# succinctlabs/snark-bn254-verifier

Measured on AMD Instinct MI355X. Metric: Groth16 verifies/sec (2 pub-inputs) at batch=2^20, 1/2/4/8 MI355X, higher is better.
Workload: dtype int64

## Files before the change

### snark-bn254-verifier_amd/csrc/bn254_fp.h

```cpp
#pragma once
#include <stdint.h>
#include <utility>
#include "bn254_constants.h"

#if defined(__HIPCC__)
#include <hip/hip_runtime.h>
#if defined(__HIP_DEVICE_COMPILE__)
#define BN_HD __host__ __device__ __forceinline__
#else
#define BN_HD __host__ __device__ inline
#endif
#if defined(BN_INLINE_ALL)
#define BN_HD_NOINLINE __host__ __device__ __forceinline__
#else
#define BN_HD_NOINLINE __host__ __device__ inline __attribute__((noinline))
#endif
#if defined(__HIP_DEVICE_COMPILE__)
#define BN_HD_DEVINLINE __host__ __device__ __forceinline__
#else
#define BN_HD_DEVINLINE __host__ __device__ inline __attribute__((noinline))
#endif
#else
#if defined(BN_TRACK_BOUNDS) || defined(BN_HOST_PLAIN_INLINE)
#define BN_HD inline
#else
#define BN_HD inline __attribute__((always_inline))
#endif
#define BN_HD_NOINLINE inline __attribute__((noinline))
#define BN_HD_DEVINLINE inline __attribute__((noinline))
#endif

#if defined(__HIP_DEVICE_COMPILE__) && !defined(BN_NO_SCHED_FENCE)
#define BN_SCHED_FENCE() __builtin_amdgcn_sched_barrier(0)
#else
#define BN_SCHED_FENCE() do { } while (0)
#endif

#if defined(BN_TRACK_BOUNDS) && !defined(__HIP_DEVICE_COMPILE__)
#include <cmath>
#include <cstdio>
#include <cstdlib>
#include <execinfo.h>
#define BN_TRACKING 1
#else
#define BN_TRACKING 0
#endif

namespace bn254 {

#define BN_HALF (1 << (BN_LB - 1))

struct Fp {
  int32_t v[BN_NL];
#if BN_TRACKING
  double vb;
  double lb;
#endif
};

#if BN_TRACKING
static const long double BN_P_LD = 21888242871839275222246405745257275088696311157297823662689037894645226208583.0L;
inline long double fp_dbg_value(const Fp& a) {
  long double s = 0;
  for (int i = BN_NL - 1; i >= 0; i--) s = s * 536870912.0L + (long double)a.v[i];
  return s;
}
inline void fp_dbg_fail(const char* what, double x) {
  fprintf(stderr, "bn254 bound violation: %s (%g)\n", what, x);
  void* bt[32]; int n = backtrace(bt, 32); backtrace_symbols_fd(bt, n, 2);
  abort();
}
inline void fp_dbg_check(const Fp& a, const char* where) {
  long double val = fabsl(fp_dbg_value(a)) / BN_P_LD;
  if (val > (long double)a.vb * (1 + 1e-12L) + 1e-9L) fp_dbg_fail(where, (double)val);
  if (a.vb > 80.0) fp_dbg_fail("value bound exceeds representable range (|v| < 2^260)", a.vb);
  for (int i = 0; i < BN_NL; i++)
    if (fabs((double)a.v[i]) > a.lb * 536870912.0 + 0.5) fp_dbg_fail("digit bound wrong", (double)a.v[i]);
}
#define BN_SETB(x, VB, LB) do { (x).vb = (VB); (x).lb = (LB); fp_dbg_check((x), __func__); } while (0)
#define BN_VB(x) ((x).vb)
#define BN_LBD(x) ((x).lb)
#else
#define BN_SETB(x, VB, LB) do { } while (0)
#define BN_VB(x) 0.0
#define BN_LBD(x) 0.0
#endif

BN_HD int32_t bn_p_limb(int i) {
  switch (i) {
    case 0: return BN_P0; case 1: return BN_P1; case 2: return BN_P2; case 3: return BN_P3; case 4: return BN_P4;
    case 5: return BN_P5; case 6: return BN_P6; case 7: return BN_P7; default: return BN_P8;
  }
}
BN_HD int32_t bn_sext29(uint32_t x) { return (int32_t)(x << 3) >> 3; }

BN_HD Fp fp_from_limbs(const int32_t* c) {
  Fp r;
#pragma unroll
  for (int i = 0; i < BN_NL; i++) r.v[i] = c[i];
  BN_SETB(r, 1.0, 0.5);
  return r;
}
BN_HD Fp fp_zero() {
  Fp r;
#pragma unroll
  for (int i = 0; i < BN_NL; i++) r.v[i] = 0;
  BN_SETB(r, 0.0, 0.5);
  return r;
}
BN_HD Fp fp_one() { return fp_from_limbs(BN_ONE); }

BN_HD Fp fp_norm(const Fp& a) {
  Fp r;
  int32_t c = 0;
#pragma unroll
  for (int i = 0; i < BN_NL - 1; i++) {
    int32_t t = a.v[i] + c + BN_HALF;
    r.v[i] = (t & (int32_t)BN_MASK) - BN_HALF;
    c = t >> BN_LB;
  }
  r.v[BN_NL - 1] = a.v[BN_NL - 1] + c;
#if BN_TRACKING
  if (a.lb > 3.4) fp_dbg_fail("fp_norm: digit overflow", a.lb);
  BN_SETB(r, a.vb, 0.5);
#endif
  return r;
}

BN_HD Fp fp_add_lazy(const Fp& a, const Fp& b) {
  Fp r;
#pragma unroll
  for (int i = 0; i < BN_NL; i++) r.v[i] = a.v[i] + b.v[i];
  BN_SETB(r, BN_VB(a) + BN_VB(b), BN_LBD(a) + BN_LBD(b));
  return r;
}
BN_HD Fp fp_sub_lazy(const Fp& a, const Fp& b) {
  Fp r;
#pragma unroll
  for (int i = 0; i < BN_NL; i++) r.v[i] = a.v[i] - b.v[i];
  BN_SETB(r, BN_VB(a) + BN_VB(b), BN_LBD(a) + BN_LBD(b));
  return r;
}
BN_HD Fp fp_neg(const Fp& a) {
  Fp r;
#pragma unroll
  for (int i = 0; i < BN_NL; i++) r.v[i] = -a.v[i];
  BN_SETB(r, BN_VB(a), BN_LBD(a) + 1e-9);
  return r;
}
BN_HD Fp fp_add(const Fp& a, const Fp& b) { return fp_norm(fp_add_lazy(a, b)); }
BN_HD Fp fp_sub(const Fp& a, const Fp& b) { return fp_norm(fp_sub_lazy(a, b)); }
BN_HD Fp fp_dbl(const Fp& a) { return fp_add(a, a); }
BN_HD Fp fp_dbl_lazy(const Fp& a) { return fp_add_lazy(a, a); }

BN_HD Fp fp_lincomb(int32_t k1, const Fp& a, int32_t k2, const Fp& b) {
  Fp r;
  int64_t acc = 0;
#pragma unroll
  for (int i = 0; i < BN_NL - 1; i++) {
    acc += (int64_t)k1 * (int64_t)a.v[i] + (int64_t)k2 * (int64_t)b.v[i] + BN_HALF;
    r.v[i] = (int32_t)((uint32_t)acc & BN_MASK) - BN_HALF;
    acc >>= BN_LB;
  }
  acc += (int64_t)k1 * (int64_t)a.v[BN_NL - 1] + (int64_t)k2 * (int64_t)b.v[BN_NL - 1];
  r.v[BN_NL - 1] = (int32_t)acc;
#if BN_TRACKING
  BN_SETB(r, a.vb * (k1 < 0 ? -k1 : k1) + b.vb * (k2 < 0 ? -k2 : k2), 0.5);
#endif
  return r;
}
BN_HD Fp fp_lincomb_reduce(int32_t k1, const Fp& a, int32_t k2, const Fp& b) {
  const int64_t C = 1420063842;
  int64_t top = (int64_t)k1 * (int64_t)a.v[BN_NL - 1] + (int64_t)k2 * (int64_t)b.v[BN_NL - 1];
  int32_t q = (int32_t)((top * C) >> 52);
  Fp r;
  int64_t acc = 0;
#pragma unroll
  for (int i = 0; i < BN_NL - 1; i++) {
    acc += (int64_t)k1 * (int64_t)a.v[i] + (int64_t)k2 * (int64_t)b.v[i] - (int64_t)q * (int64_t)bn_p_limb(i) + BN_HALF;
    r.v[i] = (int32_t)((uint32_t)acc & BN_MASK) - BN_HALF;
    acc >>= BN_LB;
  }
  acc += top - (int64_t)q * (int64_t)bn_p_limb(BN_NL - 1);
  r.v[BN_NL - 1] = (int32_t)acc;
#if BN_TRACKING
  if (a.vb * (k1 < 0 ? -k1 : k1) + b.vb * (k2 < 0 ? -k2 : k2) > 1e5) fp_dbg_fail("fp_lincomb_reduce: out of range", a.vb + b.vb);
  if (a.lb > 1.01 || b.lb > 1.01) fp_dbg_fail("fp_lincomb_reduce: digits too large", a.lb + b.lb);
  BN_SETB(r, 1.0 + 3e-5, 0.5);
#endif
  return r;
}
BN_HD Fp fp_reduce(const Fp& a) { return fp_lincomb_reduce(1, a, 0, a); }

template <int SIGN>
struct DotTerm {
  const Fp& a;
  const Fp& b;
};
BN_HD DotTerm<1> dplus(const Fp& a, const Fp& b) { return DotTerm<1>{a, b}; }
BN_HD DotTerm<-1> dminus(const Fp& a, const Fp& b) { return DotTerm<-1>{a, b}; }
template <int S> BN_HD DotTerm<S> dterm(const Fp& a, const Fp& b) { return DotTerm<S>{a, b}; }

struct DotAcc { int64_t p1, m1, p2, m2; };
template <int SIGN, int K>
BN_HD void dot_col(DotAcc& c, const DotTerm<SIGN>& t) {
  constexpr int LO = K < BN_NL ? 0 : K - (BN_NL - 1);
  constexpr int HI = K < BN_NL ? K : BN_NL - 1;
#pragma unroll
  for (int i = LO; i <= HI; i++) {
    int64_t pr = (int64_t)t.a.v[i] * (int64_t)t.b.v[K - i];
    if (SIGN == 1) c.p1 += pr; else if (SIGN == -1) c.m1 += pr; else if (SIGN == 2) c.p2 += pr; else c.m2 += pr;
  }
}
constexpr int bn_iabs(int x) { return x < 0 ? -x : x; }
template <int K, int... SIGNS>
BN_HD void dot_step(int64_t& acc, int32_t (&m)[BN_NL], Fp& r, const DotTerm<SIGNS>&... terms) {
  constexpr bool has_m1 = ((SIGNS == -1) || ...), has_p2 = ((SIGNS == 2) || ...), has_m2 = ((SIGNS == -2) || ...);
  DotAcc c; c.p1 = acc; c.m1 = 0; c.p2 = 0; c.m2 = 0;
  (dot_col<SIGNS, K>(c, terms), ...);
  acc = c.p1;
  if (has_m1) acc -= c.m1;
  if (has_p2 && has_m2) acc += 2 * (c.p2 - c.m2);
  else if (has_p2) acc += 2 * c.p2;
  else if (has_m2) acc -= 2 * c.m2;
  if constexpr (K < BN_NL) {
#pragma unroll
    for (int i = 0; i < K; i++) acc += (int64_t)m[i] * (int64_t)bn_p_limb(K - i);
    m[K] = bn_sext29((uint32_t)acc * BN_PINV);
    acc += (int64_t)m[K] * (int64_t)bn_p_limb(0);
    acc >>= BN_LB;
  } else {
#pragma unroll
    for (int i = K - (BN_NL - 1); i < BN_NL; i++) acc += (int64_t)m[i] * (int64_t)bn_p_limb(K - i);
    acc += BN_HALF;
    r.v[K - BN_NL] = (int32_t)((uint32_t)acc & BN_MASK) - BN_HALF;
    acc >>= BN_LB;
  }
}
template <int... KS, int... SIGNS>
BN_HD void dot_all(std::integer_sequence<int, KS...>, int64_t& acc, int32_t (&m)[BN_NL], Fp& r, const DotTerm<SIGNS>&... terms) {
  (dot_step<KS, SIGNS...>(acc, m, r, terms...), ...);
}
template <int... SIGNS>
BN_HD Fp fp_dot(const DotTerm<SIGNS>&... terms) {
  BN_SCHED_FENCE();
  int64_t acc = 0;
  int32_t m[BN_NL];
  Fp r;
  dot_all(std::make_integer_sequence<int, 2 * BN_NL - 1>{}, acc, m, r, terms...);
  r.v[BN_NL - 1] = (int32_t)acc;
  BN_SCHED_FENCE();
#if BN_TRACKING
  double cap = ((9.0 * bn_iabs(SIGNS) * terms.a.lb * terms.b.lb) + ...);
  if (cap + 9.0 * 0.25 + 0.01 > 32.0) fp_dbg_fail("fp_dot: accumulator may overflow", cap);
  double s = ((bn_iabs(SIGNS) * terms.a.vb * terms.b.vb) + ...);
  BN_SETB(r, 1.0 + s / 169.0 + 1e-6, 0.5);
#endif
  return r;
}
BN_HD Fp fp_mul(const Fp& a, const Fp& b) { return fp_dot(dplus(a, b)); }
BN_HD Fp fp_sqr(const Fp& a) {
  BN_SCHED_FENCE();
  int64_t acc = 0;
  int32_t m[BN_NL];
  int32_t a2[BN_NL];
  Fp r;
#pragma unroll
  for (int i = 0; i < BN_NL; i++) a2[i] = a.v[i] * 2;
#pragma unroll
  for (int k = 0; k < 2 * BN_NL - 1; k++) {
#pragma unroll
    for (int i = 0; i < BN_NL; i++) {
      int j = k - i;
      if (j >= 0 && j < BN_NL && i < j) acc += (int64_t)a2[i] * (int64_t)a.v[j];
    }
    if ((k & 1) == 0) acc += (int64_t)a.v[k / 2] * (int64_t)a.v[k / 2];
    if (k < BN_NL) {
#pragma unroll
      for (int i = 0; i < k; i++) acc += (int64_t)m[i] * (int64_t)bn_p_limb(k - i);
      m[k] = bn_sext29((uint32_t)acc * BN_PINV);
      acc += (int64_t)m[k] * (int64_t)bn_p_limb(0);
      acc >>= BN_LB;
    } else {
#pragma unroll
      for (int i = k - (BN_NL - 1); i < BN_NL; i++) acc += (int64_t)m[i] * (int64_t)bn_p_limb(k - i);
      acc += BN_HALF;
      r.v[k - BN_NL] = (int32_t)((uint32_t)acc & BN_MASK) - BN_HALF;
      acc >>= BN_LB;
    }
  }
  r.v[BN_NL - 1] = (int32_t)acc;
  BN_SCHED_FENCE();
#if BN_TRACKING
  if (9.0 * a.lb * a.lb + 2.26 > 32.0) fp_dbg_fail("fp_sqr: accumulator may overflow", a.lb);
  BN_SETB(r, 1.0 + a.vb * a.vb / 169.0 + 1e-6, 0.5);
#endif
  return r;
}

BN_HD bool fp_is_negative(const Fp& a) {
  int32_t s = a.v[BN_NL - 1];
#pragma unroll
  for (int i = BN_NL - 2; i >= 0; i--) s = (s != 0) ? s : a.v[i];
  return s < 0;
}
BN_HD Fp fp_select(bool c, const Fp& a, const Fp& b) {
  Fp r;
#pragma unroll
  for (int i = 0; i < BN_NL; i++) r.v[i] = c ? a.v[i] : b.v[i];
#if BN_TRACKING
  BN_SETB(r, a.vb > b.vb ? a.vb : b.vb, a.lb > b.lb ? a.lb : b.lb);
#endif
  return r;
}
BN_HD Fp fp_canon(const Fp& a) {
  Fp r = fp_reduce(fp_norm(a));
  Fp pl = fp_from_limbs(BN_P);
  r = fp_select(fp_is_negative(r), fp_norm(fp_add_lazy(r, pl)), r);
  Fp dn = fp_norm(fp_sub_lazy(r, pl));
  r = fp_select(!fp_is_negative(dn), dn, r);
  BN_SETB(r, 1.0, 0.5);
  return r;
}
BN_HD bool fp_is_zero(const Fp& a) {
  Fp c = fp_canon(a);
  int32_t d = 0;
#pragma unroll
  for (int i = 0; i < BN_NL; i++) d |= c.v[i];
  return d == 0;
}
BN_HD bool fp_eq(const Fp& a, const Fp& b) { return fp_is_zero(fp_sub(a, b)); }

BN_HD Fp fp_from_words_raw(const uint32_t w[8]) {
  Fp r;
#pragma unroll
  for (int i = 0; i < BN_NL; i++) {
    int bit = BN_LB * i, wi = bit >> 5, sh = bit & 31;
    uint64_t lo = w[wi];
    uint64_t hi = (wi + 1 < 8) ? w[wi + 1] : 0;
    r.v[i] = (int32_t)((uint32_t)(((hi << 32) | lo) >> sh) & BN_MASK);
  }
  BN_SETB(r, 5.3, 1.0);
  return fp_norm(r);
}
BN_HD Fp fp_from_words(const uint32_t w[8]) {
  return fp_mul(fp_from_words_raw(w), fp_from_limbs(BN_R2));
}
BN_HD void fp_to_words(uint32_t w[8], const Fp& a) {
  Fp one_plain = fp_zero();
  one_plain.v[0] = 1;
  Fp c = fp_canon(fp_mul(a, one_plain));
  uint32_t u[BN_NL];
  int32_t cy = 0;
#pragma unroll
  for (int i = 0; i < BN_NL; i++) {
    int32_t t = c.v[i] + cy;
    u[i] = (uint32_t)t & BN_MASK;
    cy = t >> BN_LB;
  }
#pragma unroll
  for (int i = 0; i < 8; i++) w[i] = 0;
#pragma unroll
  for (int i = 0; i < BN_NL; i++) {
    int bit = BN_LB * i, wi = bit >> 5, sh = bit & 31;
    uint64_t v = (uint64_t)u[i] << sh;
    if (wi < 8) w[wi] |= (uint32_t)v;
    if (wi + 1 < 8) w[wi + 1] |= (uint32_t)(v >> 32);
  }
}
BN_HD bool words_ge(const uint32_t a[8], const uint32_t b[8]) {
  bool ge = true;
#pragma unroll
  for (int i = 0; i < 8; i++) ge = (a[i] > b[i]) || (a[i] == b[i] && ge);
  return ge;
}
BN_HD void words_from_be(uint32_t w[8], const uint8_t* be32) {
#pragma unroll
  for (int i = 0; i < 8; i++) {
    const uint8_t* p = be32 + 4 * (7 - i);
    w[i] = (uint32_t)p[0] << 24 | (uint32_t)p[1] << 16 | (uint32_t)p[2] << 8 | (uint32_t)p[3];
  }
}
BN_HD void words_to_be(uint8_t* be32, const uint32_t w[8]) {
#pragma unroll
  for (int i = 0; i < 8; i++) {
    uint8_t* p = be32 + 4 * (7 - i);
    p[0] = (uint8_t)(w[i] >> 24); p[1] = (uint8_t)(w[i] >> 16); p[2] = (uint8_t)(w[i] >> 8); p[3] = (uint8_t)w[i];
  }
}

BN_HD_DEVINLINE Fp fp_mul_nl(const Fp& a, const Fp& b) { return fp_mul(a, b); }
BN_HD_DEVINLINE Fp fp_sqr_nl(const Fp& a) { return fp_sqr(a); }
BN_HD Fp fp_pow_bits(const Fp& a, const uint8_t* bits, int nbits) {
  Fp acc = a;
  for (int i = 1; i < nbits; i++) {
    acc = fp_sqr_nl(acc);
    if (bits[i]) acc = fp_mul_nl(acc, a);
  }
  return acc;
}
BN_HD Fp fp_inv_fermat(const Fp& a) { return fp_pow_bits(fp_reduce(fp_norm(a)), BN_EXP_PM2_BITS, BN_EXP_PM2_NBITS); }

BN_HD int bn_clz64(uint64_t x) {
#if defined(__HIP_DEVICE_COMPILE__)
  return __clzll((long long)x);
#else
  return __builtin_clzll(x);
#endif
}
BN_HD void fp_unsigned_digits(int32_t d[BN_NL], const int32_t* balanced) {
  int32_t cy = 0;
#pragma unroll
  for (int i = 0; i < BN_NL; i++) { int32_t t = balanced[i] + cy; d[i] = t & (int32_t)BN_MASK; cy = t >> BN_LB; }
}
BN_HD Fp fp_inv(const Fp& x) {
  const Fp y = fp_canon(x);
  int32_t a[BN_NL], b[BN_NL], u[BN_NL], v[BN_NL];
  fp_unsigned_digits(a, y.v);
  {
    int32_t pl[BN_NL];
#pragma unroll
    for (int i = 0; i < BN_NL; i++) pl[i] = bn_p_limb(i);
    fp_unsigned_digits(b, pl);
  }
  {
    const Fp c = fp_from_limbs(BN_R2);
#pragma unroll
    for (int i = 0; i < BN_NL; i++) { u[i] = c.v[i]; v[i] = 0; }
  }
#pragma unroll 1
  for (int round = 0; round < 18; round++) {
    int32_t ah = 0, am = 0, al = 0, bh = 0, bm = 0, bl = 0, low = 0;
    bool found = false;
#pragma unroll
    for (int i = BN_NL - 1; i >= 2; i--) {
      const bool take = !found && ((a[i] | b[i]) != 0);
      ah = take ? a[i] : ah; am = take ? a[i - 1] : am; al = take ? a[i - 2] : al;
      bh = take ? b[i] : bh; bm = take ? b[i - 1] : bm; bl = take ? b[i - 2] : bl;
// ... 74 lines not shown
```

### snark-bn254-verifier_amd/csrc/bn254_k_g16_load.hip

```cpp
#include <hip/hip_runtime.h>
#include "bn254_launch_ops.h"
#include "bn254_g16_loader.h"
#include "bn254_g16_plan.h"
#include "bn254_codec.h"
#include "bn254_sha256.h"

namespace bn254 {

__global__ void __launch_bounds__(256, 2)
k_g16_classify(const uint8_t* __restrict__ proofs, size_t stride, uint32_t n, uint8_t* __restrict__ status, uint32_t* __restrict__ block_count) {
  __shared__ uint32_t lds[4 * 64 * PREP_LDS_ROW];
  __shared__ uint32_t wave_pending[4];
  const int wave = threadIdx.x >> 6, lane = threadIdx.x & 63;
  const uint32_t first = blockIdx.x * 256u + (uint32_t)wave * 64u;
  uint32_t* wl = lds + wave * 64 * PREP_LDS_ROW;
  const uint32_t i = first + lane;
  const bool live = i < n;
  g16_stage_records(wl, proofs, stride, n, lane, i);
  __syncthreads();
  G1Aff A; G2Aff B;
  int err = g16_parse_a(wl + lane * PREP_LDS_ROW, A);
  err = g16_parse_b(wl + lane * PREP_LDS_ROW, B, err);
  if (live) status[i] = err ? (uint8_t)err : (uint8_t)BN254_ST_PENDING;
  const uint64_t pend = __builtin_amdgcn_ballot_w64(live && err == 0);
  if (lane == 0) wave_pending[wave] = (uint32_t)__builtin_popcountll(pend);
  __syncthreads();
  if (threadIdx.x == 0) block_count[blockIdx.x] = wave_pending[0] + wave_pending[1] + wave_pending[2] + wave_pending[3];
}
__global__ void __launch_bounds__(256)
k_g16_compact_write(const uint8_t* __restrict__ status, uint32_t n, const uint32_t* __restrict__ block_count, uint32_t* __restrict__ slot_proof, uint8_t* __restrict__ slot_status) {
  __shared__ uint32_t s_before[G16_COMPACT_BLOCK], s_total[G16_COMPACT_BLOCK], wave_pending[4];
  const uint32_t t = threadIdx.x, wave = t >> 6, lane = t & 63u;
  uint32_t before, total;
  g16_compact_partial(block_count, gridDim.x, blockIdx.x, t, &before, &total);
  s_before[t] = before; s_total[t] = total;
  const uint32_t i = blockIdx.x * 256u + t;
  const bool pend = i < n && status[i] == BN254_ST_PENDING;
  const uint64_t mask = __builtin_amdgcn_ballot_w64(pend);
  if (lane == 0) wave_pending[wave] = (uint32_t)__builtin_popcountll(mask);
  __syncthreads();
  for (uint32_t d = G16_COMPACT_BLOCK / 2; d > 0; d >>= 1) {
    if (t < d) { s_before[t] += s_before[t + d]; s_total[t] += s_total[t + d]; }
    __syncthreads();
  }
  const uint32_t n_pending = s_total[0];
  uint32_t j = s_before[0] + (uint32_t)__builtin_popcountll(mask & ((1ull << lane) - 1ull));
  for (uint32_t k = 0; k < wave; k++) j += wave_pending[k];
  if (pend && j < n) { slot_proof[j] = i; slot_status[j] = BN254_ST_PENDING; }
  if (i < n && i >= n_pending) { slot_proof[i] = G16_COMPACT_NO_PROOF; slot_status[i] = 0; }
}

__global__ void __launch_bounds__(256, 2)
k_g16_prepare(const uint8_t* __restrict__ proofs, size_t stride, const uint8_t* __restrict__ inputs, int n_public, uint32_t n,
              int32_t* ws, uint8_t* __restrict__ status, const int32_t* __restrict__ msm_tab, const int32_t* __restrict__ k0,
              int inputs_match_key, int wide_msm, const uint32_t* __restrict__ slot_proof, uint8_t* __restrict__ slot_status) {
  __shared__ uint32_t lds[4 * 64 * PREP_LDS_ROW];
  const int wave = threadIdx.x >> 6, lane = threadIdx.x & 63;
  const uint32_t first = blockIdx.x * 256u + (uint32_t)wave * 64u;
  uint32_t* wl = lds + wave * 64 * PREP_LDS_ROW;
  uint32_t pi = first + (uint32_t)lane;
  bool wave_live = true;
  if (slot_proof) {
    const bool slot_live = pi < n && (slot_status[pi] & BN254_ST_PENDING) != 0;
    pi = slot_live ? slot_proof[pi] : G16_COMPACT_NO_PROOF;
    wave_live = __builtin_amdgcn_ballot_w64(slot_live) != 0;
  }
  if (wave_live) g16_stage_records(wl, proofs, stride, n, lane, pi);
  __syncthreads();
  if (!wave_live) return;
  uint8_t* const st_out = slot_proof ? slot_status : status;
  const uint32_t i = first + lane;
  const bool live = pi < n;
  const uint32_t ii = live ? pi : n - 1;
  DevWs w(ws, n, live ? i : DEAD_LANE);
  const uint32_t* my = wl + lane * PREP_LDS_ROW;

  G1Aff A;
  int err = g16_parse_a(my, A);
  w.st(VE_AX, A.x); w.st(VE_AY, A.y);
  G2Aff B;
  err = g16_parse_b(my, B, err);
  vst2(w, VE_B, B.x); vst2(w, VE_B + 2, B.y);

  G1Aff C;
  const int err_c = g16_parse_c(my, C);
  w.st(VE_CX, C.x); w.st(VE_CY, C.y);

  if (wide_msm) {
    if (live) st_out[i] = err ? (uint8_t)err : (uint8_t)(BN254_ST_PENDING | err_c);
    return;
  }
  G1Aff K0; K0.x = uni_ld(k0); K0.y = uni_ld(k0 + BN_NL);
  G1Proj L = g1_from_affine(K0);
  if (inputs_match_key) {
    for (int s = 0; s < n_public; s++) {
      const uint8_t* sp = inputs + ((size_t)ii * (size_t)n_public + s) * 32;
      uint32_t sw[8];
      if ((((uintptr_t)inputs) & 3) == 0) {
#pragma unroll
        for (int k = 0; k < 8; k++) sw[k] = ((const uint32_t*)sp)[k];
      } else {
#pragma unroll
        for (int k = 0; k < 8; k++) sw[k] = (uint32_t)sp[4 * k] | (uint32_t)sp[4 * k + 1] << 8 | (uint32_t)sp[4 * k + 2] << 16 | (uint32_t)sp[4 * k + 3] << 24;
      }
      uint32_t kw[8];
#pragma unroll
      for (int k = 0; k < 8; k++) kw[k] = __builtin_bswap32(sw[7 - k]);
      auto next_digit = [&]() -> uint32_t {
        const uint32_t dg = kw[0] & MSM_FW_ENTRIES;
#pragma unroll
        for (int k = 0; k < 7; k++) kw[k] = (kw[k] >> MSM_FW_BITS) | (kw[k + 1] << (32 - MSM_FW_BITS));
        kw[7] >>= MSM_FW_BITS;
        return dg;
      };
      uint32_t dig = next_digit();
      G1Aff q = msm_entry(msm_tab, (size_t)(s * MSM_FW_WINDOWS) * MSM_FW_ENTRIES + (dig ? dig - 1 : 0));
      for (int j = 0; j < MSM_FW_WINDOWS; j++) {
        uint32_t dn = 0; G1Aff qn = q;
        if (j + 1 < MSM_FW_WINDOWS) { dn = next_digit(); qn = msm_entry(msm_tab, (size_t)(s * MSM_FW_WINDOWS + j + 1) * MSM_FW_ENTRIES + (dn ? dn - 1 : 0)); }
        if (dig != 0) L = g1_add_mixed(L, q);
        dig = dn; q = qn;
      }
    }
  }
  bool l_inf = g1_is_identity(L);
  G1Aff La = g1_to_affine(L);
  La.y = fp_select(l_inf, fp_one(), La.y);
  w.st(VE_LX, La.x); w.st(VE_LY, La.y);
  if (live) st_out[i] = err ? (uint8_t)err : (uint8_t)(BN254_ST_PENDING | (l_inf ? BN254_ST_LINF : 0) | err_c);
}

__global__ void __launch_bounds__(256, 2)
k_g16_check_scalars(const uint8_t* __restrict__ inputs, int n_public, uint32_t n, uint8_t* __restrict__ status) {
  const uint32_t i = blockIdx.x * 256u + threadIdx.x;
  if (i >= n) return;
  bool bad = false;
  for (int s = 0; s < n_public; s++) {
    const uint8_t* sp = inputs + ((size_t)i * (size_t)n_public + s) * 32;
    uint32_t w[8];
    words_from_be(w, sp);
    bad |= words_ge(w, BN_R_WORDS);
  }
  if (bad) status[i] = BN254_ST_NOT_MEMBER;
}

__global__ void __launch_bounds__(256, 2)
k_g16_msm_partial(const uint8_t* __restrict__ inputs, int n_public, uint32_t n, int per, int chunks, const uint8_t* __restrict__ status,
                  const int32_t* __restrict__ msm_tab, int32_t* __restrict__ part) {
  const uint32_t g = blockIdx.x * 256u + threadIdx.x;
  if (g >= n * (uint32_t)chunks) return;
  const uint32_t c = g / n, i = g - c * n;
  G1Proj acc = g1_identity();
  if (status[i] & BN254_ST_PENDING) {
    const int s_end = (int)min((uint32_t)n_public, (c + 1) * (uint32_t)per);
    for (int s = (int)(c * per); s < s_end; s++) {
      const uint8_t* sp = inputs + ((size_t)i * (size_t)n_public + s) * 32;
      uint32_t sw[8];
      if ((((uintptr_t)inputs) & 3) == 0) {
#pragma unroll
        for (int k = 0; k < 8; k++) sw[k] = ((const uint32_t*)sp)[k];
      } else {
#pragma unroll
        for (int k = 0; k < 8; k++) sw[k] = (uint32_t)sp[4 * k] | (uint32_t)sp[4 * k + 1] << 8 | (uint32_t)sp[4 * k + 2] << 16 | (uint32_t)sp[4 * k + 3] << 24;
      }
      for (int j = 0; j < 32; j++) {
        const int wi = 31 - j;
        uint32_t dig = sw[0] & 0xff;
#pragma unroll
        for (int k = 0; k < 7; k++) sw[k] = (sw[k] >> 8) | (sw[k + 1] << 24);
        sw[7] >>= 8;
        if (dig != 0) acc = g1_add_mixed(acc, msm_entry(msm_tab, (size_t)(s * 32 + wi) * 255 + (dig - 1)));
      }
    }
  }
  int32_t* o = part + (size_t)c * 27 * n + i;
#pragma unroll
  for (int l = 0; l < BN_NL; l++) { o[(size_t)l * n] = acc.x.v[l]; o[(size_t)(9 + l) * n] = acc.y.v[l]; o[(size_t)(18 + l) * n] = acc.z.v[l]; }
}
__global__ void __launch_bounds__(256)
k_g16_comb_digits(const uint8_t* __restrict__ inputs, int n_public, uint32_t n, uint16_t* __restrict__ digits) {
  const size_t g = (size_t)blockIdx.x * 256u + threadIdx.x;
  if (g >= (size_t)n * (size_t)n_public) return;
  const uint32_t s = (uint32_t)(g / n), i = (uint32_t)(g - (size_t)s * n);
  const uint8_t* sp = inputs + ((size_t)i * (size_t)n_public + s) * 32;
  uint32_t w[8];
#pragma unroll
  for (int k = 0; k < 8; k++) { const uint8_t* q = sp + 28 - 4 * k; w[k] = (uint32_t)q[0] << 24 | (uint32_t)q[1] << 16 | (uint32_t)q[2] << 8 | (uint32_t)q[3]; }
  for (int col = 0; col < G16_COMB_COLS; col++) {
    const uint32_t idx = g16_comb_digit(w, col);
    digits[((size_t)col * (size_t)n_public + s) * n + i] = (uint16_t)idx;
  }
}
__global__ void __launch_bounds__(256, 2)
k_g16_msm_partial_comb(const uint16_t* __restrict__ digits, int n_public, uint32_t n, int per, int chunks, const uint8_t* __restrict__ status,
                       const int32_t* __restrict__ msm_tab, int32_t* __restrict__ part) {
  const uint32_t g = blockIdx.x * 256u + threadIdx.x;
  if (g >= n * (uint32_t)chunks) return;
  const uint32_t c = g / n, i = g - c * n;
  G1Proj acc = g1_identity();
  if (status[i] & BN254_ST_PENDING) {
    const int s_begin = (int)(c * per), s_end = (int)min((uint32_t)n_public, (c + 1) * (uint32_t)per);
    auto digit_at = [&](int col, int s) -> uint32_t { return digits[((size_t)col * (size_t)n_public + (size_t)s) * n + i]; };
    auto entry_at = [&](int s, uint32_t idx) -> G1Aff { return msm_entry(msm_tab, ((size_t)s << G16_COMB_TEETH) + idx); };
    auto advance = [&](int& col, int& s) { if (++s == s_end) { s = s_begin; col--; } };
    if (s_begin < s_end) {
      int col1 = G16_COMB_COLS - 1, s1 = s_begin;
      uint32_t d_cur = digit_at(col1, s1);
      G1Aff e_cur = entry_at(s1, d_cur);
      int col0 = col1, s0 = s1;
      advance(col1, s1);
      uint32_t d_nxt = col1 >= 0 ? digit_at(col1, s1) : 0u;
      int col2 = col1, s2 = s1;
      if (col2 >= 0) advance(col2, s2);
      while (col0 >= 0) {
        G1Aff e_nxt = e_cur;
        uint32_t d_nn = 0u;
        if (col1 >= 0) e_nxt = entry_at(s1, d_nxt);
        if (col2 >= 0) d_nn = digit_at(col2, s2);
        if (s0 == s_begin && col0 != G16_COMB_COLS - 1) acc = g1_dbl(acc);
        if (d_cur != 0) acc = g1_add_mixed(acc, e_cur);
        col0 = col1; s0 = s1; d_cur = d_nxt; e_cur = e_nxt;
        col1 = col2; s1 = s2; d_nxt = d_nn;
        if (col2 >= 0) advance(col2, s2);
      }
    }
  }
  int32_t* o = part + (size_t)c * 27 * n + i;
#pragma unroll
  for (int l = 0; l < BN_NL; l++) { o[(size_t)l * n] = acc.x.v[l]; o[(size_t)(9 + l) * n] = acc.y.v[l]; o[(size_t)(18 + l) * n] = acc.z.v[l]; }
}
__global__ void __launch_bounds__(256, 2)
k_g16_msm_reduce(const int32_t* __restrict__ part, int chunks, uint32_t n, int32_t* ws, uint8_t* __restrict__ status, const int32_t* __restrict__ k0) {
  VM_KERNEL_PROLOGUE();
  const uint32_t ii = i < n ? i : n - 1;
  G1Aff K0; K0.x = uni_ld(k0); K0.y = uni_ld(k0 + BN_NL);
  G1Proj L = g1_from_affine(K0);
  for (int c = 0; c < chunks; c++) {
    const int32_t* o = part + (size_t)c * 27 * n + ii;
    G1Proj q;
#pragma unroll
    for (int l = 0; l < BN_NL; l++) { q.x.v[l] = o[(size_t)l * n]; q.y.v[l] = o[(size_t)(9 + l) * n]; q.z.v[l] = o[(size_t)(18 + l) * n]; }
    BN_SETB(q.x, 3.0, 0.5); BN_SETB(q.y, 3.0, 0.5); BN_SETB(q.z, 3.0, 0.5);
    L = g1_add(L, q);
  }
  bool l_inf = g1_is_identity(L);
  G1Aff La = g1_to_affine(L);
  La.y = fp_select(l_inf, fp_one(), La.y);
  w.st(VE_LX, La.x); w.st(VE_LY, La.y);
  if (i < n && (st & BN254_ST_PENDING) && l_inf) status[i] = st | BN254_ST_LINF;
}

__global__ void __launch_bounds__(256, 2)
k_g16_msm_reduce8(const int32_t* __restrict__ part, int chunks, uint32_t n, int32_t* ws, uint8_t* __restrict__ status, const int32_t* __restrict__ k0) {
  __shared__ int32_t sums[32 * 8 * 27];
  const uint32_t p = blockIdx.x * 32u + (threadIdx.x >> 3), sub = threadIdx.x & 7u;
  const uint32_t pp = p < n ? p : n - 1;
  G1Proj L = g1_identity();
  for (int c = (int)sub; c < chunks; c += 8) {
    const int32_t* o = part + (size_t)c * 27 * n + pp;
    G1Proj q;
#pragma unroll
    for (int l = 0; l < BN_NL; l++) { q.x.v[l] = o[(size_t)l * n]; q.y.v[l] = o[(size_t)(9 + l) * n]; q.z.v[l] = o[(size_t)(18 + l) * n]; }
    BN_SETB(q.x, 3.0, 0.5); BN_SETB(q.y, 3.0, 0.5); BN_SETB(q.z, 3.0, 0.5);
    L = g1_add(L, q);
  }
  {
    int32_t* o = sums + threadIdx.x * 27;
    const Fp x = fp_reduce(L.x), y = fp_reduce(L.y), z = fp_reduce(L.z);
#pragma unroll
    for (int l = 0; l < BN_NL; l++) { o[l] = x.v[l]; o[9 + l] = y.v[l]; o[18 + l] = z.v[l]; }
  }
  __syncthreads();
  const bool lead = sub == 0 && p < n;
  const uint8_t st = status[pp];
  G1Aff K0; K0.x = uni_ld(k0); K0.y = uni_ld(k0 + BN_NL);
  G1Proj T = g1_from_affine(K0);
  for (int j = 0; j < 8; j++) {
    const int32_t* o = sums + ((threadIdx.x & ~7u) + j) * 27;
    G1Proj q;
#pragma unroll
    for (int l = 0; l < BN_NL; l++) { q.x.v[l] = o[l]; q.y.v[l] = o[9 + l]; q.z.v[l] = o[18 + l]; }
    BN_SETB(q.x, 1.01, 0.5); BN_SETB(q.y, 1.01, 0.5); BN_SETB(q.z, 1.01, 0.5);
    T = g1_add(T, q);
  }
  const bool l_inf = g1_is_identity(T);
  G1Aff La = g1_to_affine(T);
  La.y = fp_select(l_inf, fp_one(), La.y);
  DevWs w(ws, n, lead ? p : DEAD_LANE);
  w.st(VE_LX, La.x); w.st(VE_LY, La.y);
  if (lead && (st & BN254_ST_PENDING) && l_inf) status[p] = st | BN254_ST_LINF;
}

__global__ void k_gather_rows(uint8_t* __restrict__ dst, const uint8_t* __restrict__ src, size_t src_stride, uint32_t row_bytes, const uint32_t* __restrict__ idx, uint32_t m) {
  const size_t t = (size_t)blockIdx.x * 256 + threadIdx.x;
  const uint32_t per = row_bytes / 4;
  if (t >= (size_t)m * per) return;
  const uint32_t k = (uint32_t)(t / per), c = (uint32_t)(t % per);
  const uint8_t* p = src + (size_t)idx[k] * src_stride + 4 * (size_t)c;
  uint32_t v;
  if ((((uintptr_t)src) | src_stride) & 3) v = (uint32_t)p[0] | (uint32_t)p[1] << 8 | (uint32_t)p[2] << 16 | (uint32_t)p[3] << 24;
  else v = *(const uint32_t*)p;
  ((uint32_t*)dst)[t] = v;
}
__global__ void k_scatter_status(uint8_t* __restrict__ status, const uint8_t* __restrict__ fb_status, const uint32_t* __restrict__ idx, uint32_t m) {
  const uint32_t k = blockIdx.x * 256u + threadIdx.x;
  if (k < m) status[idx[k]] = fb_status[k];
}
__global__ void __launch_bounds__(256, 2) k_g16_decompress(const uint8_t* __restrict__ src, size_t stride, uint32_t n, uint8_t* __restrict__ raw, uint8_t* __restrict__ pre) {
  const uint32_t i = blockIdx.x * 256u + threadIdx.x;
  if (i >= n) return;
  const uint8_t* p = src + (size_t)i * stride;
  uint32_t in[32], out[64];
  if (((((uintptr_t)src) | stride) & 15) == 0) {
#pragma unroll
    for (int k = 0; k < 8; k++) { const uint4 v = ((const uint4*)p)[k]; in[4 * k] = v.x; in[4 * k + 1] = v.y; in[4 * k + 2] = v.z; in[4 * k + 3] = v.w; }
  } else {
#pragma unroll
    for (int k = 0; k < 32; k++) in[k] = (uint32_t)p[4 * k] | (uint32_t)p[4 * k + 1] << 8 | (uint32_t)p[4 * k + 2] << 16 | (uint32_t)p[4 * k + 3] << 24;
  }
  const bool ok = g16_decompress_record(in, out);
  uint4* q = (uint4*)(raw + (size_t)i * 256);
#pragma unroll
  for (int k = 0; k < 16; k++) q[k] = make_uint4(out[4 * k], out[4 * k + 1], out[4 * k + 2], out[4 * k + 3]);
  pre[i] = ok ? 0 : 1;
}
__global__ void __launch_bounds__(256) k_g16_status_merge(uint8_t* __restrict__ status, const uint8_t* __restrict__ pre, uint32_t n) {
  const uint32_t i = blockIdx.x * 256u + threadIdx.x;
  if (i < n && pre[i]) status[i] = BN254_ST_MALFORMED;
}
__global__ void __launch_bounds__(256) k_sp1_public_inputs(const uint8_t* __restrict__ vkh, size_t vkh_stride, const uint8_t* __restrict__ pv, uint64_t pv_bytes,
                                                           uint64_t pv_base, const uint64_t* __restrict__ off, uint32_t n, uint8_t* __restrict__ rows,
                                                           uint8_t* __restrict__ pre) {
  const uint32_t i = blockIdx.x * 256u + threadIdx.x;
  const bool lane = i < n;
  uint64_t start = 0, len = 0;
  bool ok = false;
  if (lane) ok = sp1_range(off[i], off[i + 1], pv_base, pv_bytes, &start, &len);
  const uint64_t nb = lane ? sha256_blocks(len) : 0;
  uint32_t h[8];
  sha256_init(h);
  for (uint64_t b = 0; __ballot(b < nb) != 0; b++) sp1_sha256_block(h, pv, pv_bytes, start, len, b);
  if (!lane) return;
  uint32_t v[8], dg[8];
  sp1_load_vkey_hash(vkh + (size_t)i * vkh_stride, v);
  sp1_digest_words(h, dg);
  uint4* q = (uint4*)(rows + (size_t)i * 64);
  q[0] = make_uint4(v[0], v[1], v[2], v[3]); q[1] = make_uint4(v[4], v[5], v[6], v[7]);
  q[2] = make_uint4(dg[0], dg[1], dg[2], dg[3]); q[3] = make_uint4(dg[4], dg[5], dg[6], dg[7]);
  pre[i] = ok ? 0 : 1;
}

}

using namespace bn254;
hipError_t bn254_launch_gather_rows(uint8_t* dst, const uint8_t* src, size_t src_stride, uint32_t row_bytes, const uint32_t* idx, uint32_t m, hipStream_t s) {
  const size_t threads = (size_t)m * (row_bytes / 4);
  if (threads) hipLaunchKernelGGL(k_gather_rows, dim3((unsigned)((threads + 255) / 256)), dim3(256), 0, s, dst, src, src_stride, row_bytes, idx, m);
  return hipGetLastError();
}
hipError_t bn254_launch_scatter_status(uint8_t* status, const uint8_t* fb_status, const uint32_t* idx, uint32_t m, hipStream_t s) {
  if (m) hipLaunchKernelGGL(k_scatter_status, dim3(grid_for(m)), dim3(256), 0, s, status, fb_status, idx, m);
  return hipGetLastError();
}
hipError_t bn254_launch_g16_decompress(const uint8_t* src, size_t stride, uint32_t n, uint8_t* raw, uint8_t* pre, hipStream_t s) {
  if (n) hipLaunchKernelGGL(k_g16_decompress, dim3(grid_for(n)), dim3(256), 0, s, src, stride, n, raw, pre);
  return hipGetLastError();
}
hipError_t bn254_launch_g16_status_merge(uint8_t* status, const uint8_t* pre, uint32_t n, hipStream_t s) {
  if (n) hipLaunchKernelGGL(k_g16_status_merge, dim3(grid_for(n)), dim3(256), 0, s, status, pre, n);
  return hipGetLastError();
}
hipError_t bn254_launch_sp1_public_inputs(const uint8_t* vkh, size_t vkh_stride, const uint8_t* pv, uint64_t pv_bytes, uint64_t pv_base, const uint64_t* off, uint32_t n,
                                          uint8_t* rows, uint8_t* pre, hipStream_t s) {
  if (n) hipLaunchKernelGGL(k_sp1_public_inputs, dim3(grid_for(n)), dim3(256), 0, s, vkh, vkh_stride, pv, pv_bytes, pv_base, off, n, rows, pre);
  return hipGetLastError();
}
```

### snark-bn254-verifier_amd/csrc/bn254_k_probe.hip

```cpp
#include <hip/hip_runtime.h>
#include "bn254_launch_ops.h"

namespace bn254 {

#define VALU_PEAK_ITERS 16384
__global__ void __launch_bounds__(256) k_valu_peak(uint32_t* out, uint32_t seed, int iters) {
  const uint32_t tid = threadIdx.x + blockIdx.x * blockDim.x;
  const uint32_t a = seed * 2654435761u + tid, b = (seed ^ 0x9e3779b9u) + tid * 7u;
  uint64_t acc[16];
#pragma unroll
  for (int i = 0; i < 16; i++) acc[i] = (uint64_t)(a + i) << 7 | (uint32_t)i;
  for (int it = 0; it < iters; it++) {
#pragma unroll
    for (int i = 0; i < 16; i++) asm volatile("v_mad_u64_u32 %0, vcc, %1, %2, %0" : "+v"(acc[i]) : "v"(a), "v"(b) : "vcc");
  }
  uint32_t x = 0;
#pragma unroll
  for (int i = 0; i < 16; i++) x ^= (uint32_t)acc[i] ^ (uint32_t)(acc[i] >> 32);
  out[tid] = x;
}

__device__ __forceinline__ Fp probe_ld_fp(const uint8_t* p) {
  uint32_t w[8];
  words_from_be(w, p);
  return fp_from_words(w);
}
__device__ __forceinline__ void probe_st_fp(uint8_t* p, const Fp& a) {
  uint32_t w[8];
  fp_to_words(w, a);
  words_to_be(p, w);
}
__global__ void __launch_bounds__(256, 2) k_dbg_fp_mul(const uint8_t* a, const uint8_t* b, uint8_t* o, size_t n) {
  size_t i = (size_t)blockIdx.x * 256 + threadIdx.x;
  if (i >= n) return;
  probe_st_fp(o + 32 * i, fp_mul(probe_ld_fp(a + 32 * i), probe_ld_fp(b + 32 * i)));
}
__global__ void __launch_bounds__(256, 2) k_dbg_load(int32_t* ws, uint32_t n, uint8_t* status, int e, const uint8_t* src, int kind) {
  const uint32_t i = blockIdx.x * 256u + threadIdx.x;
  if (i >= n) return;
  DevWs w(ws, n, i);
  if (kind == 0) {
    const int korder[6] = {0, 2, 4, 1, 3, 5};
    const uint8_t* p = src + 384 * (size_t)i;
    for (int t = 0; t < 6; t++) { w.st(e + 2 * korder[t], probe_ld_fp(p + 64 * t)); w.st(e + 2 * korder[t] + 1, probe_ld_fp(p + 64 * t + 32)); }
  } else if (kind == 3) {
    const int korder[6] = {0, 2, 4, 1, 3, 5};
    const int32_t* p = (const int32_t*)src + 12 * BN_NL * (size_t)i;
    for (int t = 0; t < 12; t++) { Fp a; for (int l = 0; l < BN_NL; l++) a.v[l] = p[t * BN_NL + l]; w.st(e + 2 * korder[t >> 1] + (t & 1), a); }
  } else if (kind == 4) {
    w.st(e, probe_ld_fp(src + 64 * (size_t)i)); w.st(e + 1, probe_ld_fp(src + 64 * (size_t)i + 32));
  } else if (kind == 1) {
    w.st(VE_AX, probe_ld_fp(src + 64 * (size_t)i)); w.st(VE_AY, probe_ld_fp(src + 64 * (size_t)i + 32));
  } else {
    const uint8_t* q = src + 128 * (size_t)i;
    w.st(VE_B + 1, probe_ld_fp(q)); w.st(VE_B, probe_ld_fp(q + 32)); w.st(VE_B + 3, probe_ld_fp(q + 64)); w.st(VE_B + 2, probe_ld_fp(q + 96));
  }
  status[i] = BN254_ST_PENDING;
}
__global__ void __launch_bounds__(256, 2) k_dbg_store(int32_t* ws, uint32_t n, int e, uint8_t* dst) {
  const uint32_t i = blockIdx.x * 256u + threadIdx.x;
  if (i >= n) return;
  DevWs w(ws, n, i);
  const int korder[6] = {0, 2, 4, 1, 3, 5};
  uint8_t* p = dst + 384 * (size_t)i;
  for (int t = 0; t < 6; t++) { probe_st_fp(p + 64 * t, w.ld(e + 2 * korder[t])); probe_st_fp(p + 64 * t + 32, w.ld(e + 2 * korder[t] + 1)); }
}
__global__ void __launch_bounds__(256, 2) k_dbg_store_raw(int32_t* ws, uint32_t n, int e, int32_t* dst) {
  const uint32_t i = blockIdx.x * 256u + threadIdx.x;
  if (i >= n) return;
  DevWs w(ws, n, i);
  const int korder[6] = {0, 2, 4, 1, 3, 5};
  int32_t* p = dst + 12 * BN_NL * (size_t)i;
  for (int t = 0; t < 12; t++) { const Fp a = w.ld(e + 2 * korder[t >> 1] + (t & 1)); for (int l = 0; l < BN_NL; l++) p[t * BN_NL + l] = a.v[l]; }
}
__global__ void __launch_bounds__(256, 2) k_dbg_g2_subgroup(const uint8_t* g2, uint8_t* o, size_t n) {
  size_t i = (size_t)blockIdx.x * 256 + threadIdx.x;
  if (i >= n) return;
  G2Aff q; q.x.c1 = probe_ld_fp(g2 + 128 * i); q.x.c0 = probe_ld_fp(g2 + 128 * i + 32);
  q.y.c1 = probe_ld_fp(g2 + 128 * i + 64); q.y.c0 = probe_ld_fp(g2 + 128 * i + 96);
  o[i] = (g2_on_curve(q) && g2_in_subgroup(q)) ? 1 : 0;
}
__global__ void __launch_bounds__(256, 2) k_dbg_g2_ate(int32_t* ws, uint32_t n, const uint8_t* __restrict__ status, uint8_t* o) {
  VM_KERNEL_PROLOGUE();
  bool ok = vm_g2_ate_check(w, VE_T, VE_B);
  if (i < n) o[i] = ok ? 1 : 0;
}

}

using namespace bn254;
double bn254_measure_valu_peak(int reps) {
  hipDeviceProp_t p;
  int dev = 0;
  if (hipGetDevice(&dev) != hipSuccess || hipGetDeviceProperties(&p, dev) != hipSuccess) return 0.0;
  const int grid = p.multiProcessorCount * 4;
  uint32_t* out = nullptr;
  if (hipMalloc((void**)&out, (size_t)grid * 256 * 4) != hipSuccess) return 0.0;
  hipEvent_t e0, e1;
  (void)hipEventCreate(&e0); (void)hipEventCreate(&e1);
  hipLaunchKernelGGL(k_valu_peak, dim3(grid), dim3(256), 0, nullptr, out, 1u, VALU_PEAK_ITERS);
  float best = 1e30f;
  int since_best = 0;
  for (int r = 0; r < 200 && since_best < reps; r++) {
    (void)hipEventRecord(e0, nullptr);
    hipLaunchKernelGGL(k_valu_peak, dim3(grid), dim3(256), 0, nullptr, out, (uint32_t)(r + 2), VALU_PEAK_ITERS);
    (void)hipEventRecord(e1, nullptr);
    if (hipEventSynchronize(e1) != hipSuccess) { best = 1e30f; break; }
    float ms = 0.f;
    since_best++;
    if (hipEventElapsedTime(&ms, e0, e1) == hipSuccess && ms > 0.f && ms < best * 0.998f) { best = ms; since_best = 0; }
  }
  (void)hipEventDestroy(e0); (void)hipEventDestroy(e1); (void)hipFree(out);
  if (best > 1e29f) return 0.0;
  return (double)grid * 256.0 * (double)VALU_PEAK_ITERS * 16.0 / ((double)best * 1e-3);
}
double bn254_measure_valu_sustained(double ms_target) {
  hipDeviceProp_t p;
  int dev = 0;
  if (hipGetDevice(&dev) != hipSuccess || hipGetDeviceProperties(&p, dev) != hipSuccess) return 0.0;
  const int grid = p.multiProcessorCount * 4;
  uint32_t* out = nullptr;
  if (hipMalloc((void**)&out, (size_t)grid * 256 * 4) != hipSuccess) return 0.0;
  int launches = (int)(ms_target / 2.0);
  if (launches < 4) launches = 4;
  if (launches > 1000) launches = 1000;
  hipEvent_t e0, e1;
  (void)hipEventCreate(&e0); (void)hipEventCreate(&e1);
  (void)hipEventRecord(e0, nullptr);
  for (int r = 0; r < launches; r++) hipLaunchKernelGGL(k_valu_peak, dim3(grid), dim3(256), 0, nullptr, out, (uint32_t)(r + 1), VALU_PEAK_ITERS);
  (void)hipEventRecord(e1, nullptr);
  float ms = 0.f;
  const bool ok = hipEventSynchronize(e1) == hipSuccess && hipEventElapsedTime(&ms, e0, e1) == hipSuccess && ms > 0.f;
  (void)hipEventDestroy(e0); (void)hipEventDestroy(e1); (void)hipFree(out);
  return ok ? (double)launches * grid * 256.0 * (double)VALU_PEAK_ITERS * 16.0 / ((double)ms * 1e-3) : 0.0;
}
hipError_t bn254_launch_dbg_fp_mul(const uint8_t* a, const uint8_t* b, uint8_t* o, size_t n, hipStream_t s) {
  hipLaunchKernelGGL(k_dbg_fp_mul, dim3(grid_for(n)), dim3(256), 0, s, a, b, o, n);
  return hipGetLastError();
}
hipError_t bn254_launch_dbg_load(int32_t* ws, size_t n, uint8_t* status, int e, const void* src, int kind, hipStream_t s) {
  hipLaunchKernelGGL(k_dbg_load, dim3(grid_for(n)), dim3(256), 0, s, ws, (uint32_t)n, status, e, (const uint8_t*)src, kind);
  return hipGetLastError();
}
hipError_t bn254_launch_dbg_store(int32_t* ws, size_t n, int e, void* dst, int format, hipStream_t s) {
  if (format) hipLaunchKernelGGL(k_dbg_store_raw, dim3(grid_for(n)), dim3(256), 0, s, ws, (uint32_t)n, e, (int32_t*)dst);
  else hipLaunchKernelGGL(k_dbg_store, dim3(grid_for(n)), dim3(256), 0, s, ws, (uint32_t)n, e, (uint8_t*)dst);
  return hipGetLastError();
}
hipError_t bn254_launch_dbg_fp12_op_fmt(int op, const uint8_t* a, const uint8_t* b, uint8_t* o, size_t n, int32_t* ws, uint8_t* status, int in_format, int out_format, hipStream_t s) {
  unsigned g = grid_for(n);
  uint32_t nn = (uint32_t)n;
  LaunchOps ops{ws, nn, status, g, s, {nullptr, nullptr, nullptr}, nullptr};
  const int kind = in_format ? 3 : 0;
  hipLaunchKernelGGL(k_dbg_load, dim3(g), dim3(256), 0, s, ws, nn, status, (int)VE_F, a, kind);
  if (op == 0 || op == 8 || op == 9) {
    hipLaunchKernelGGL(k_dbg_load, dim3(g), dim3(256), 0, s, ws, nn, status, (int)VE_S1, b, kind);
    ops.f12_mul(VE_S0, op == 9 ? (VE_F | VE_CONJ) : VE_F, VE_S1, op == 8);
  }
  else if (op == 1) { ops.f12_sqr(VE_F); ops.f12_conj(VE_S0, VE_F); ops.f12_conj(VE_S0, VE_S0); }
  else if (op == 2) ops.f12_inv(VE_S0, VE_F);
  else if (op == 3) {
    ops.f12_inv(VE_S0, VE_F); ops.f12_conj(VE_S1, VE_F); ops.f12_mul(VE_S0, VE_S1, VE_S0); ops.f12_frob(VE_S1, VE_S0, 2);
    ops.f12_mul(VE_S0, VE_S1, VE_S0); ops.f12_cyclo_sqr(VE_S0, VE_S0);
  }
  else if (op == 5) ops.f12_cyclo_sqr(VE_S0, VE_F);
  else ops.f12_frob(VE_S0, VE_F, op == 6 ? 2 : op == 7 ? 3 : 1);
  (void)bn254_launch_dbg_store(ws, n, (int)VE_S0, o, out_format, s);
  return hipGetLastError();
}
hipError_t bn254_launch_dbg_verdict(int form, int32_t* ws, size_t n, uint8_t* status, const int32_t* target, hipStream_t s) {
  unsigned grid = grid_for(n);
  uint32_t nn = (uint32_t)n;
  if (form == 0) hipLaunchKernelGGL(k_g16_compare, dim3(grid), dim3(256), 0, s, ws, nn, status, target, (int)BN254_ST_REJECT);
  else hipLaunchKernelGGL(k_f12_mul_verdict, dim3(grid), dim3(256), 0, s, ws, nn, status, (int)VE_S0, (int)VE_S2, (int)VE_S0, target, (int)BN254_ST_REJECT, (const uint32_t*)nullptr, status);
  return hipGetLastError();
}
hipError_t bn254_launch_dbg_coop12_g16(const G16LaunchArgs& a, hipStream_t s) {
  hipLaunchKernelGGL(k_g16_prepare, dim3(grid_for(a.n)), dim3(256), 0, s, a.proofs, a.stride, a.inputs, a.n_public, (uint32_t)a.n, a.ws, a.status, a.msm_tab, a.k0, a.inputs_match_key, 1,
                     (const uint32_t*)nullptr, (uint8_t*)nullptr);
  return bn254_coop12_miller_g16(a.ws, a.status, a.n, a.gtab, a.dtab, a.inputs, a.n_public, a.inputs_match_key, a.msm_tab, a.k0, 0, a.target, s);
}
hipError_t bn254_launch_dbg_pairing(const uint8_t* g1, const uint8_t* g2, uint8_t* o, size_t n, int32_t* ws, uint8_t* status, hipStream_t s) {
  unsigned g = grid_for(n);
  uint32_t nn = (uint32_t)n;
  LaunchOps ops{ws, nn, status, g, s, {nullptr, nullptr, nullptr}, nullptr};
  hipLaunchKernelGGL(k_dbg_load, dim3(g), dim3(256), 0, s, ws, nn, status, 0, g1, 1);
  hipLaunchKernelGGL(k_dbg_load, dim3(g), dim3(256), 0, s, ws, nn, status, 0, g2, 2);
  hipLaunchKernelGGL(k_vm_init, dim3(g), dim3(256), 0, s, ws, nn, (const uint8_t*)status);
  vm_miller_program(ops, miller_step_table().kind, false);
  vm_final_exp_program(ops);
  hipLaunchKernelGGL(k_dbg_store, dim3(g), dim3(256), 0, s, ws, nn, (int)VE_S0, o);
  return hipGetLastError();
}
hipError_t bn254_launch_dbg_g2_ate(const uint8_t* g1, const uint8_t* g2, uint8_t* o, size_t n, int32_t* ws, uint8_t* status, hipStream_t s) {
  unsigned g = grid_for(n);
  uint32_t nn = (uint32_t)n;
  LaunchOps ops{ws, nn, status, g, s, {nullptr, nullptr, nullptr}, nullptr};
  hipLaunchKernelGGL(k_dbg_load, dim3(g), dim3(256), 0, s, ws, nn, status, 0, g1, 1);
  hipLaunchKernelGGL(k_dbg_load, dim3(g), dim3(256), 0, s, ws, nn, status, 0, g2, 2);
  hipLaunchKernelGGL(k_vm_init, dim3(g), dim3(256), 0, s, ws, nn, (const uint8_t*)status);
  vm_miller_program(ops, miller_step_table().kind, false);
  hipLaunchKernelGGL(k_dbg_g2_ate, dim3(g), dim3(256), 0, s, ws, nn, (const uint8_t*)status, o);
  return hipGetLastError();
}
hipError_t bn254_launch_dbg_g2_subgroup(const uint8_t* g2, uint8_t* o, size_t n, hipStream_t s) {
  hipLaunchKernelGGL(k_dbg_g2_subgroup, dim3(grid_for(n)), dim3(256), 0, s, g2, o, n);
  return hipGetLastError();
}
```

### snark-bn254-verifier_amd/csrc/bn254_kernels.hip

```cpp
#include <hip/hip_runtime.h>
#include "bn254_launch_ops.h"
#include "bn254_g16_plan.h"

static_assert(G16_MILLER_STEPS == BN_ATE_STEPS, "bn254_g16_plan.h counts the Miller steps of bn254_constants.h");

namespace bn254 {

__global__ void __launch_bounds__(256, 2) k_vm_init(int32_t* ws, uint32_t n, const uint8_t* __restrict__ status) {
  VM_KERNEL_PROLOGUE();
  w.st(VE_F, fp_one());
  for (int e = 1; e < 12; e++) w.st(VE_F + e, fp_zero());
  for (int e = 0; e < 4; e++) w.st(VE_T + e, w.ld(VE_B + e));
  w.st(VE_T + 4, fp_one()); w.st(VE_T + 5, fp_zero());
}
__global__ void __launch_bounds__(256, 2) k_f12_sqr(int32_t* ws, uint32_t n, const uint8_t* __restrict__ status, int e) { VM_KERNEL_PROLOGUE(); vm_f12_sqr(w, e); }
__global__ void __launch_bounds__(256, 2) k_f12_mul_line_fixed(int32_t* ws, uint32_t n, const uint8_t* __restrict__ status, int e, const int32_t* __restrict__ entry, int e_px, int inf_mask) {
  VM_KERNEL_PROLOGUE();
  FixedLine l; l.m = uni_ld2(entry); l.c = uni_ld2(entry + 2 * BN_NL); l.xc = uni_ld2(entry + 4 * BN_NL);
  vm_f12_mul_line_fixed(w, e, l, e_px, (st & inf_mask) != 0);
}
__global__ void __launch_bounds__(256, 2) k_f12_mul_line_fixed2(int32_t* ws, uint32_t n, const uint8_t* __restrict__ status, int e, const int32_t* __restrict__ entry0,
                                                                int e_px0, int inf_mask0, const int32_t* __restrict__ entry1, int e_px1, int inf_mask1) {
  __shared__ int32_t park_lds[72 * 256];
  VM_KERNEL_PROLOGUE();
  w.lds = park_lds;
  FixedLine l0, l1;
  l0.m = uni_ld2(entry0); l0.c = uni_ld2(entry0 + 2 * BN_NL); l0.xc = uni_ld2(entry0 + 4 * BN_NL);
  l1.m = uni_ld2(entry1); l1.c = uni_ld2(entry1 + 2 * BN_NL); l1.xc = uni_ld2(entry1 + 4 * BN_NL);
  vm_f12_mul_line_fixed2(w, e, l0, e_px0, (st & inf_mask0) != 0, l1, e_px1, (st & inf_mask1) != 0);
}
__global__ void __launch_bounds__(256, 2) k_miller_dbl_var(int32_t* ws, uint32_t n, const uint8_t* __restrict__ status, int e_t, int e, int e_px) {
  VM_KERNEL_PROLOGUE(); vm_miller_dbl_var(w, e_t, e, e_px);
}
__global__ void __launch_bounds__(256, 2) k_miller_sqr_dbl_var(int32_t* ws, uint32_t n, const uint8_t* __restrict__ status, int e_t, int e, int e_px) {
  __shared__ int32_t park_lds[72 * 256];
  VM_KERNEL_PROLOGUE();
  w.lds = park_lds;
  vm_miller_sqr_dbl_var(w, e_t, e, e_px);
}
__global__ void __launch_bounds__(256, 2) k_miller_add_var(int32_t* ws, uint32_t n, const uint8_t* __restrict__ status, int e_t, int e_b, int which, int e, int e_px) {
  VM_KERNEL_PROLOGUE(); vm_miller_add_var(w, e_t, e_b, which, e, e_px);
}
__global__ void __launch_bounds__(256, 2) k_f12_mul(int32_t* ws, uint32_t n, const uint8_t* __restrict__ status, int d, int a, int b, int conj_b) {
  __shared__ int32_t park_lds[72 * 256];
  VM_KERNEL_PROLOGUE();
  w.lds = park_lds;
  vm_f12_mul(w, d, a, b, conj_b != 0);
}
__global__ void __launch_bounds__(256, 2) k_f12_mul_verdict(int32_t* ws, uint32_t n, uint8_t* status, int d, int a, int b, const int32_t* __restrict__ target, int reject_code,
                                                            const uint32_t* __restrict__ slot_proof, uint8_t* __restrict__ out_status) {
  __shared__ int32_t park_lds[72 * 256];
  const uint32_t i = blockIdx.x * 256u + threadIdx.x;
  const uint8_t st = status[i < n ? i : n - 1];
  uint8_t out = st;
  if (__builtin_amdgcn_ballot_w64((st & BN254_ST_PENDING) != 0) != 0) {
    DevWs w(ws, n, i < n ? i : DEAD_LANE);
    w.lds = park_lds;
    const bool acc = vm_f12_mul_eq_const(w, d, a, b, target);
    if (st & BN254_ST_PENDING) out = acc ? BN254_ST_ACCEPT : (uint8_t)reject_code;
    if (i < n && (st & BN254_ST_PENDING)) status[i] = out;
  }
  if (slot_proof && i < n && st != 0) out_status[slot_proof[i]] = out;
}
__global__ void __launch_bounds__(256, 2) k_f12_copy(int32_t* ws, uint32_t n, const uint8_t* __restrict__ status, int d, int a) { VM_KERNEL_PROLOGUE(); vm_f12_copy(w, d, a); }
__global__ void __launch_bounds__(256, 2) k_f12_cyclo_sqr(int32_t* ws, uint32_t n, const uint8_t* __restrict__ status, int d, int a) { VM_KERNEL_PROLOGUE(); vm_f12_cyclo_sqr(w, d, a); }
__global__ void __launch_bounds__(256, 2) k_f12_cyclo_sqr_n(int32_t* ws, uint32_t n, const uint8_t* __restrict__ status, int d, int a, int count) {
  VM_KERNEL_PROLOGUE(); vm_f12_cyclo_sqr_n(w, d, a, __builtin_amdgcn_readfirstlane(count));
}
__global__ void __launch_bounds__(256, 2) k_f12_conj(int32_t* ws, uint32_t n, const uint8_t* __restrict__ status, int d, int a) { VM_KERNEL_PROLOGUE(); vm_f12_conj(w, d, a); }
__global__ void __launch_bounds__(256, 2) k_f12_frob(int32_t* ws, uint32_t n, const uint8_t* __restrict__ status, int d, int a, int j) { VM_KERNEL_PROLOGUE(); vm_f12_frob(w, d, a, j); }
__global__ void __launch_bounds__(256, 2) k_f12_inv(int32_t* ws, uint32_t n, const uint8_t* __restrict__ status, int d, int a) { VM_KERNEL_PROLOGUE(); vm_f12_inv(w, d, a); }
__global__ void __launch_bounds__(256, 2) k_g16_compare(int32_t* ws, uint32_t n, uint8_t* __restrict__ status, const int32_t* __restrict__ target, int reject_code) {
  VM_KERNEL_PROLOGUE();
  bool acc = vm_f12_eq_const(w, VE_S0, target);
  if (i < n && (st & BN254_ST_PENDING)) status[i] = acc ? BN254_ST_ACCEPT : (uint8_t)reject_code;
}

__global__ void __launch_bounds__(256, 2)
k_g16_subgroup(uint32_t n, int32_t* ws, uint8_t* __restrict__ status, int inputs_match_key, int e_t) {
  VM_KERNEL_PROLOGUE();
  bool ok = vm_g2_ate_check(w, e_t, VE_B);
  if (i < n && (st & BN254_ST_PENDING)) status[i] = g16_subgroup_status(st, ok, inputs_match_key);
}

}

using namespace bn254;
const char* const bn254_kernel_kind_names[KID_COUNT] = {
  "k_g16_prepare", "k_g16_subgroup", "k_vm_init", "k_f12_sqr", "k_f12_mul_line_fixed",
  "k_f12_mul", "k_f12_cyclo_sqr", "k_f12_conj", "k_f12_frob", "k_f12_inv", "k_g16_compare", "k_f12_copy", "k_f12_cyclo_sqr_n", "k_miller_dbl_var", "k_miller_add_var", "k_g16_msm_partial", "k_g16_msm_reduce", "k_f12_mul_line_fixed2", "k_miller_sqr_dbl_var", "k_miller_step_dbl", "k_miller_step_add", "k_coop12_miller_g16", "k_miller_run"};

hipError_t bn254_launch_g16(const G16LaunchArgs& a, hipStream_t s, hipEvent_t* ev , G16Prof* prof) {
  unsigned grid = grid_for(a.n);
  uint32_t n = (uint32_t)a.n;
  if (ev) (void)hipEventRecord(ev[0], s);
  const G16Form form = g16_launch_form(a.n, (size_t)a.n_public, a.inputs_match_key != 0, a.msm_part != nullptr, a.part_of_larger != 0,
                                       a.split_streams[0] && a.split_streams[1], knob_coop_on(), knob_run_steps_g16());
  const bool wide = form.wide, coop = form.form == G16_FORM_COOP;
  const bool compact = a.slot_proof && a.slot_status && a.block_count && g16_compacts(form, a.key_inputs, a.strict_scalars != 0, a.rlc != 0);
  uint8_t* const lane_status = compact ? a.slot_status : a.status;
  const uint32_t* const slot_proof = compact ? a.slot_proof : nullptr;
  {
    ProfScope ps_(prof, KID_PREPARE, s);
    if (compact) {
      hipLaunchKernelGGL(k_g16_classify, dim3(grid), dim3(256), 0, s, a.proofs, a.stride, n, a.status, a.block_count);
      hipLaunchKernelGGL(k_g16_compact_write, dim3(grid), dim3(256), 0, s, (const uint8_t*)a.status, n, (const uint32_t*)a.block_count, a.slot_proof, a.slot_status);
    }
    hipLaunchKernelGGL(k_g16_prepare, dim3(grid), dim3(256), 0, s, a.proofs, a.stride, a.inputs, a.n_public, n, a.ws, a.status, a.msm_tab, a.k0, a.inputs_match_key, (wide || coop) ? 1 : 0,
                       slot_proof, a.slot_status);
  }
  if (a.strict_scalars && a.n_public > 0) hipLaunchKernelGGL(k_g16_check_scalars, dim3(grid), dim3(256), 0, s, a.inputs, a.n_public, n, a.status);
  if (wide) {
    const int per = knob_wide_per() ? knob_wide_per() : G16_WIDE_MSM_INPUTS_PER_LANE, chunks = (a.n_public + per - 1) / per;
    unsigned pg = (unsigned)(((size_t)n * chunks + 255) / 256);
    {
      ProfScope ps_(prof, KID_MSM_PARTIAL, s);
      if (a.msm_comb) {
        const size_t scalars = (size_t)n * (size_t)a.n_public;
        hipLaunchKernelGGL(k_g16_comb_digits, dim3((unsigned)((scalars + 255) / 256)), dim3(256), 0, s, a.inputs, a.n_public, n, a.msm_digits);
        hipLaunchKernelGGL(k_g16_msm_partial_comb, dim3(pg), dim3(256), 0, s, (const uint16_t*)a.msm_digits, a.n_public, n, per, chunks, (const uint8_t*)a.status, a.msm_tab, a.msm_part);
      }
      else hipLaunchKernelGGL(k_g16_msm_partial, dim3(pg), dim3(256), 0, s, a.inputs, a.n_public, n, per, chunks, (const uint8_t*)a.status, a.msm_tab, a.msm_part);
    }
    if (chunks >= 16 && a.n <= 65536) {
      ProfScope ps_(prof, KID_MSM_REDUCE, s);
      hipLaunchKernelGGL(k_g16_msm_reduce8, dim3((unsigned)((a.n + 31) / 32)), dim3(256), 0, s, (const int32_t*)a.msm_part, chunks, n, a.ws, a.status, a.k0);
    } else {
      BN_LAUNCH(KID_MSM_REDUCE, k_g16_msm_reduce, (const int32_t*)a.msm_part, chunks, n, a.ws, a.status, a.k0);
    }
  }
  if (ev) (void)hipEventRecord(ev[1], s);
  if (coop) {
    hipError_t e;
    { ProfScope ps_(prof, KID_COOP_G16, s); e = bn254_coop12_miller_g16(a.ws, a.status, a.n, a.gtab, a.dtab, a.inputs, a.n_public, a.inputs_match_key, a.msm_tab, a.k0, wide ? 1 : 0, a.target, s); }
    if (e != hipSuccess) return e;
    if (ev) { (void)hipEventRecord(ev[2], s); (void)hipEventRecord(ev[3], s); (void)hipEventRecord(ev[4], s); }
    return hipGetLastError();
  }
  LaunchOps ops{a.ws, n, lane_status, grid, s, {a.gtab, a.dtab, nullptr}, prof};
  const bool folded = form.form == G16_FORM_LANES && form.run_steps > 0;
  if (folded) { ops.run_fold = MR_FOLD_INIT | MR_FOLD_ATE; ops.inputs_match_key = a.inputs_match_key; }
  else BN_LAUNCH(KID_VM_INIT, k_vm_init, a.ws, n, (const uint8_t*)a.status);
  if (form.form == G16_FORM_LATENCY) {
    ops.f12_copy(VE_S1, VE_F); ops.f12_copy(VE_S2, VE_F);
    (void)hipEventRecord(a.split_ev[0], s);
    LaunchOps ob{a.ws, n, a.status, grid, a.split_streams[0], {a.gtab, a.dtab, nullptr}, nullptr};
    LaunchOps oc{a.ws, n, a.status, grid, a.split_streams[1], {a.gtab, a.dtab, nullptr}, nullptr};
    (void)hipStreamWaitEvent(ob.s, a.split_ev[0], 0); (void)hipStreamWaitEvent(oc.s, a.split_ev[0], 0);
    const uint8_t* kinds = miller_step_table().kind;
    for (int st_ = 0; st_ < BN_ATE_STEPS; st_++) {
      const int kind = kinds[st_];
      if (kind == 0) { if (st_ != 0) ops.miller_sqr_dbl_var(VE_T, VE_F, VE_AX); else ops.miller_dbl_var(VE_T, VE_F, VE_AX); }
      else ops.miller_add_var(VE_T, VE_B, kind - 1, VE_F, VE_AX);
      if (kind == 0 && st_ != 0) { ob.f12_sqr(VE_S1); oc.f12_sqr(VE_S2); }
      ob.f12_mul_line_fixed(VE_S1, 0, st_, VE_LX);
      oc.f12_mul_line_fixed(VE_S2, 1, st_, VE_CX);
    }
    (void)hipEventRecord(a.split_ev[1], ob.s); (void)hipEventRecord(a.split_ev[2], oc.s);
    (void)hipStreamWaitEvent(s, a.split_ev[1], 0); (void)hipStreamWaitEvent(s, a.split_ev[2], 0);
    ops.f12_mul(VE_F, VE_F, VE_S1); ops.f12_mul(VE_F, VE_F, VE_S2);
  } else {
    const int run_steps = form.run_steps;
    if (run_steps) vm_miller_program_runs(ops, run_steps);
    else vm_miller_program(ops, miller_step_table().kind, true);
  }
  if (ev) (void)hipEventRecord(ev[2], s);
  if (!folded) BN_LAUNCH(KID_SUBGROUP, k_g16_subgroup, n, a.ws, a.status, a.inputs_match_key, (int)VE_T);
  if (ev) (void)hipEventRecord(ev[3], s);
  if (folded) {
    vm_final_exp_program_head(ops);
    BN_LAUNCH(KID_F12_MUL, k_f12_mul_verdict, a.ws, n, lane_status, (int)VE_S0, (int)VE_S2, (int)VE_S0, a.target, BN254_ST_REJECT, slot_proof, a.status);
  } else {
    vm_final_exp_program(ops);
    BN_LAUNCH(KID_COMPARE, k_g16_compare, a.ws, n, a.status, a.target, BN254_ST_REJECT);
  }
  if (ev) (void)hipEventRecord(ev[4], s);
  return hipGetLastError();
}

hipError_t bn254_launch_g16_keys(const G16KeysLaunchArgs& a, hipStream_t s) {
  unsigned grid = grid_for(a.m);
  const uint32_t n = (uint32_t)a.m;
  G16Prof* prof = nullptr;
  bn254_launch_g16_prepare_keys(a, grid, s);
  LaunchOps ops{a.ws, n, a.slot_status, grid, s, {nullptr, nullptr, nullptr}, prof};
  ops.key_desc = a.desc; ops.n_keys = a.n_keys; ops.granule_key = a.granule_key;
  ops.run_fold = MR_FOLD_INIT | MR_FOLD_ATE;
  vm_miller_program_runs(ops, g16_launch_form(a.m, 0, true, false, a.part_of_larger != 0, false, false, knob_run_steps_g16_keys()).run_steps);
  vm_final_exp_program_head(ops);
  bn254_launch_f12_mul_verdict_keys(a, grid, s, (int)VE_S0, (int)VE_S2, (int)VE_S0);
  return hipGetLastError();
}

hipError_t bn254_launch_g16_keys_direct(const G16KeysDirectArgs& a, hipStream_t s) {
  const uint32_t n = (uint32_t)a.n;
  hipLaunchKernelGGL(k_g16_prepare, dim3(grid_for(a.n)), dim3(256), 0, s, a.proofs, a.stride, a.inputs, 0, n, a.ws, a.status, (const int32_t*)nullptr, (const int32_t*)nullptr, 1, 1,
                     (const uint32_t*)nullptr, (uint8_t*)nullptr);
  return bn254_coop12_miller_g16_keys(a.ws, a.status, a.n, a.key_index, a.desc, a.n_keys, a.inputs, a.input_stride, a.strict_scalars, s);
}

hipError_t bn254_launch_pairing2_fixed(int32_t* ws, uint8_t* status, size_t n, const int32_t* tab0, const int32_t* tab1, const int32_t* target_one,
                                       int reject_code, hipStream_t s, hipStream_t aux, hipEvent_t ev_fork, hipEvent_t ev_join) {
  if (knob_coop_on() && n <= knob_coop_fixed_max()) {
    return bn254_coop12_miller_fixed(ws, status, n, 2, tab0, tab1, target_one, reject_code, s);
  }
  return bn254_launch_pairing2_fixed_lanes(ws, status, n, tab0, tab1, target_one, reject_code, s, aux, ev_fork, ev_join);
}
hipError_t bn254_launch_pairing2_fixed_lanes(int32_t* ws, uint8_t* status, size_t n, const int32_t* tab0, const int32_t* tab1, const int32_t* target_one,
                                             int reject_code, hipStream_t s, hipStream_t aux, hipEvent_t ev_fork, hipEvent_t ev_join) {
  unsigned grid = grid_for(n);
  uint32_t nn = (uint32_t)n;
  G16Prof* prof = nullptr;
  LaunchOps ops{ws, nn, status, grid, s, {tab0, tab1, nullptr}, nullptr};
  ops.inf_mask[0] = BN254_ST_LINF; ops.inf_mask[1] = BN254_ST_LINF2;
  BN_LAUNCH(KID_VM_INIT, k_vm_init, ws, nn, (const uint8_t*)status);
  const uint8_t* kinds = miller_step_table().kind;
  if (aux && n <= G16_SPLIT_MAX_PROOFS) {
    ops.f12_copy(VE_S1, VE_F);
    (void)hipEventRecord(ev_fork, s);
    LaunchOps ob = ops; ob.s = aux;
    (void)hipStreamWaitEvent(aux, ev_fork, 0);
    for (int st_ = 0; st_ < BN_ATE_STEPS; st_++) {
      if (kinds[st_] == 0 && st_ != 0) { ops.f12_sqr(VE_F); ob.f12_sqr(VE_S1); }
      ops.f12_mul_line_fixed(VE_F, 0, st_, VE_LX);
      ob.f12_mul_line_fixed(VE_S1, 1, st_, VE_CX);
    }
    (void)hipEventRecord(ev_join, aux);
    (void)hipStreamWaitEvent(s, ev_join, 0);
    ops.f12_mul(VE_F, VE_F, VE_S1);
  } else {
    const int run_steps = knob_run_steps_pairing2_lanes();
    if (run_steps > 0) {
      for (int s0 = 0; s0 < BN_ATE_STEPS; s0 += run_steps) ops.miller_run_fixed2(s0, s0 + run_steps < BN_ATE_STEPS ? s0 + run_steps : BN_ATE_STEPS, VE_F, VE_LX, VE_CX);
    } else {
      for (int st_ = 0; st_ < BN_ATE_STEPS; st_++) {
        if (kinds[st_] == 0 && st_ != 0) ops.f12_sqr(VE_F);
        ops.f12_mul_line_fixed2(VE_F, st_, VE_LX, VE_CX);
      }
    }
  }
  vm_final_exp_program(ops);
  BN_LAUNCH(KID_COMPARE, k_g16_compare, ws, nn, status, target_one, reject_code);
  return hipGetLastError();
}
hipError_t bn254_launch_pairing2_fixed_keys(int32_t* ws, uint8_t* status, size_t n, const PlonkKeyDesc* desc, uint32_t n_keys, const uint32_t* granule_key, const int32_t* target_one,
                                            int reject_code, hipStream_t s) {
  unsigned grid = grid_for(n);
  uint32_t nn = (uint32_t)n;
  G16Prof* prof = nullptr;
  LaunchOps ops{ws, nn, status, grid, s, {nullptr, nullptr, nullptr}, nullptr};
  ops.inf_mask[0] = BN254_ST_LINF; ops.inf_mask[1] = BN254_ST_LINF2;
  ops.plonk_desc = desc; ops.n_keys = n_keys; ops.granule_key = granule_key;
  if (plonk_keys_coop_form(n))
    return bn254_coop12_miller_fixed_keys(ws, status, n, granule_key, 6, desc, n_keys, target_one, reject_code, s);
  BN_LAUNCH(KID_VM_INIT, k_vm_init, ws, nn, (const uint8_t*)status);
  const int run_steps = knob_run_steps_pairing2_keys();
  for (int s0 = 0; s0 < BN_ATE_STEPS; s0 += run_steps) ops.miller_run_fixed2(s0, s0 + run_steps < BN_ATE_STEPS ? s0 + run_steps : BN_ATE_STEPS, VE_F, VE_LX, VE_CX);
  vm_final_exp_program(ops);
  BN_LAUNCH(KID_COMPARE, k_g16_compare, ws, nn, status, target_one, reject_code);
  return hipGetLastError();
}
hipError_t bn254_launch_pairing2_fixed_groups_keys(int32_t* grp_ws, uint8_t* grp_status, size_t groups, const PlonkKeyDesc* desc, uint32_t n_keys, const uint32_t* granule_key,
                                                   const int32_t* target_one, int reject_code, hipStream_t s) {
  if (groups > bn254_coop_max_proofs_fixed()) return hipErrorInvalidValue;
  return bn254_coop12_miller_fixed_keys(grp_ws, grp_status, groups, granule_key, 0, desc, n_keys, target_one, reject_code, s);
}
```

### snark-bn254-verifier_amd/csrc/bn254_rlc.h

```cpp
#pragma once
#include "bn254_vm.h"
#include "bn254_rlc_plan.h"
#include "bn254_fw.h"

namespace bn254 {

enum {
  RLC_C = VE_S1,
  RLC_T = VE_S1 + 3,
  RLC_MAX_PUBLIC = 8,
  RLC_W = RLC_T + 1,
  RLC_ACC = VE_S2,
  RLC_HI = 512
};

BN_HD uint32_t bn_rotl(uint32_t x, int n) { return (x << n) | (x >> (32 - n)); }
#define BN_CHACHA_QR(a, b, c, d) do { a += b; d ^= a; d = bn_rotl(d, 16); c += d; b ^= c; b = bn_rotl(b, 12); a += b; d ^= a; d = bn_rotl(d, 8); c += d; b ^= c; b = bn_rotl(b, 7); } while (0)
struct ChaChaKey { uint32_t k[8]; uint32_t nonce[3]; };
BN_HD void chacha20_block4(uint32_t out[4], const ChaChaKey& key, uint32_t counter) {
  uint32_t s0 = 0x61707865u, s1 = 0x3320646eu, s2 = 0x79622d32u, s3 = 0x6b206574u;
  uint32_t x0 = s0, x1 = s1, x2 = s2, x3 = s3, x4 = key.k[0], x5 = key.k[1], x6 = key.k[2], x7 = key.k[3], x8 = key.k[4], x9 = key.k[5],
           x10 = key.k[6], x11 = key.k[7], x12 = counter, x13 = key.nonce[0], x14 = key.nonce[1], x15 = key.nonce[2];
  for (int i = 0; i < 10; i++) {
    BN_CHACHA_QR(x0, x4, x8, x12); BN_CHACHA_QR(x1, x5, x9, x13); BN_CHACHA_QR(x2, x6, x10, x14); BN_CHACHA_QR(x3, x7, x11, x15);
    BN_CHACHA_QR(x0, x5, x10, x15); BN_CHACHA_QR(x1, x6, x11, x12); BN_CHACHA_QR(x2, x7, x8, x13); BN_CHACHA_QR(x3, x4, x9, x14);
  }
  out[0] = x0 + s0; out[1] = x1 + s1; out[2] = x2 + s2; out[3] = x3 + s3;
}

struct Fr8 { uint32_t w[8]; };
BN_HD uint32_t bn_r_word(int i) {
  switch (i) {
    case 0: return 0xf0000001u; case 1: return 0x43e1f593u; case 2: return 0x79b97091u; case 3: return 0x2833e848u;
    case 4: return 0x8181585du; case 5: return 0xb85045b6u; case 6: return 0xe131a029u; default: return 0x30644e72u;
  }
}
#define BN_R_NINV32 0xefffffffu
BN_HD uint32_t bn_r2_word(int i) {
  switch (i) {
    case 0: return 0xae216da7u; case 1: return 0x1bb8e645u; case 2: return 0xe35c59e3u; case 3: return 0x53fe3ab1u;
    case 4: return 0x53bb8085u; case 5: return 0x8c49833du; case 6: return 0x7f4e44a5u; default: return 0x0216d0b1u;
  }
}
BN_HD Fr8 fr8_cond_sub_r(const uint32_t t[9]) {
  uint32_t d[8]; uint64_t br = 0;
#pragma unroll
  for (int i = 0; i < 8; i++) { uint64_t x = (uint64_t)t[i] - bn_r_word(i) - br; d[i] = (uint32_t)x; br = (x >> 32) & 1; }
  const bool ge = t[8] != 0 || br == 0;
  Fr8 r;
#pragma unroll
  for (int i = 0; i < 8; i++) r.w[i] = ge ? d[i] : t[i];
  return r;
}
BN_HD Fr8 fr8_mont_mul(const Fr8& a, const Fr8& b) {
  uint32_t t[10];
#pragma unroll
  for (int i = 0; i < 10; i++) t[i] = 0;
#pragma unroll
  for (int i = 0; i < 8; i++) {
    uint64_t c = 0;
#pragma unroll
    for (int j = 0; j < 8; j++) { uint64_t s = (uint64_t)a.w[j] * b.w[i] + t[j] + c; t[j] = (uint32_t)s; c = s >> 32; }
    uint64_t s8 = (uint64_t)t[8] + c; t[8] = (uint32_t)s8; t[9] = (uint32_t)(s8 >> 32);
    const uint32_t m = t[0] * BN_R_NINV32;
    c = ((uint64_t)m * bn_r_word(0) + t[0]) >> 32;
#pragma unroll
    for (int j = 1; j < 8; j++) { uint64_t s = (uint64_t)m * bn_r_word(j) + t[j] + c; t[j - 1] = (uint32_t)s; c = s >> 32; }
    uint64_t s = (uint64_t)t[8] + c; t[7] = (uint32_t)s; t[8] = t[9] + (uint32_t)(s >> 32);
  }
  return fr8_cond_sub_r(t);
}
BN_HD Fr8 fr8_add(const Fr8& a, const Fr8& b) {
  uint32_t t[9]; uint64_t c = 0;
#pragma unroll
  for (int i = 0; i < 8; i++) { c += (uint64_t)a.w[i] + b.w[i]; t[i] = (uint32_t)c; c >>= 32; }
  t[8] = (uint32_t)c;
  return fr8_cond_sub_r(t);
}
BN_HD Fr8 fr8_zero() { Fr8 r; for (int i = 0; i < 8; i++) r.w[i] = 0; return r; }
BN_HD Fr8 fr8_mul_plain(const Fr8& x, const Fr8& k) {
  Fr8 r2;
#pragma unroll
  for (int i = 0; i < 8; i++) r2.w[i] = bn_r2_word(i);
  return fr8_mont_mul(fr8_mont_mul(x, r2), k);
}
BN_HD Fp fr8_to_slot(const Fr8& a) {
  Fp r;
#pragma unroll
  for (int i = 0; i < 8; i++) r.v[i] = (int32_t)a.w[i];
  r.v[8] = 0;
#if BN_TRACKING
  r.vb = 0; r.lb = 0;
#endif
  return r;
}
BN_HD Fr8 fr8_from_slot(const Fp& a) {
  Fr8 r;
#pragma unroll
  for (int i = 0; i < 8; i++) r.w[i] = (uint32_t)a.v[i];
  return r;
}

BN_FP_CONST(BN_GLV_BETA, {171145621, -175301341, -123954279, -218476986, -127948067, 24572270, 250450874, -198635200, 789247});
BN_HD uint32_t bn_glv_lambda_word(int i) {
  switch (i) {
    case 0: return 0xb99c90ddu; case 1: return 0x8b17ea66u; case 2: return 0x8d8daaa7u; case 3: return 0x5bfc4108u;
    case 4: return 0x41a91758u; case 5: return 0xb3c4d79du; default: return 0u;
  }
}
BN_HD Fr8 rlc_weight(const uint32_t k[4]) {
  Fr8 k2 = fr8_zero(), lam, k1 = fr8_zero();
  k1.w[0] = k[0]; k1.w[1] = k[1]; k2.w[0] = k[2]; k2.w[1] = k[3];
#pragma unroll
  for (int i = 0; i < 8; i++) lam.w[i] = bn_glv_lambda_word(i);
  return fr8_add(fr8_mul_plain(k2, lam), k1);
}
template <int W>
BN_HD G1Proj g1_mul_glv_w(const G1Aff& P, const uint32_t* k1, bool neg1, const uint32_t* k2, bool neg2) {
  G1Aff P1 = P, P2;
  P1.y = fp_select(neg1, fp_neg(P.y), P.y);
  P2.x = fp_mul(P.x, fp_from_limbs(BN_GLV_BETA)); P2.y = fp_select(neg2, fp_neg(P.y), P.y);
  const G1Proj T1 = g1_from_affine(P1), T2 = g1_from_affine(P2), T3 = g1_add_mixed(T1, P2);
  G1Proj acc = g1_identity();
  uint32_t a[W], b[W];
#pragma unroll
  for (int i = 0; i < W; i++) { a[i] = k1[i]; b[i] = k2[i]; }
  for (int bit = 0; bit < 32 * W; bit++) {
    const uint32_t d1 = a[W - 1] >> 31, d2 = b[W - 1] >> 31;
#pragma unroll
    for (int i = W - 1; i > 0; i--) { a[i] = (a[i] << 1) | (a[i - 1] >> 31); b[i] = (b[i] << 1) | (b[i - 1] >> 31); }
    a[0] <<= 1; b[0] <<= 1;
    acc = g1_dbl(acc);
    G1Proj q;
    q.x = fp_select(d2 != 0, fp_select(d1 != 0, T3.x, T2.x), T1.x);
    q.y = fp_select(d2 != 0, fp_select(d1 != 0, T3.y, T2.y), T1.y);
    q.z = fp_select(d2 != 0, fp_select(d1 != 0, T3.z, T2.z), T1.z);
    G1Proj c = g1_add(acc, q);
    const bool take = (d1 | d2) != 0;
    acc.x = fp_select(take, c.x, acc.x); acc.y = fp_select(take, c.y, acc.y); acc.z = fp_select(take, c.z, acc.z);
  }
  return acc;
}
BN_HD G1Proj g1_mul_glv(const G1Aff& P, const uint32_t k[4]) { return g1_mul_glv_w<2>(P, k, false, k + 2, false); }
template <class W, class LX>
BN_HD void vm_rlc_scale(W& w, const uint32_t r[4], int n_public, const LX& load_input) {
  {
    G1Aff A; A.x = w.ld(VE_AX); A.y = w.ld(VE_AY);
    G1Aff Ar = g1_to_affine(g1_mul_glv(A, r));
    w.st(VE_AX, Ar.x); w.st(VE_AY, Ar.y);
  }
  {
    G1Aff Cc; Cc.x = w.ld(VE_CX); Cc.y = w.ld(VE_CY);
    G1Proj Cr = g1_mul_glv(Cc, r);
    w.st(RLC_C, fp_reduce(Cr.x)); w.st(RLC_C + 1, fp_reduce(Cr.y)); w.st(RLC_C + 2, fp_reduce(Cr.z));
  }
  const Fr8 rr = rlc_weight(r);
  w.st(RLC_T, fr8_to_slot(rr));
  for (int j = 0; j < n_public; j++) {
    Fr8 x; load_input(j, x.w);
    w.st(RLC_T + 1 + j, fr8_to_slot(fr8_mul_plain(x, rr)));
  }
}
template <bool DO_SQR, class W>
BN_HD void vm_miller_var_multi(W& w, int kind, int G, uint32_t deadmask) {
  Fp2 f4, f5;
  {
    Fp2 k0, k1, k2, k3, k4, k5;
    k0.c0 = w.ld0(VE_F); k0.c1 = w.ld0(VE_F + 1); k1.c0 = w.ld0(VE_F + 2); k1.c1 = w.ld0(VE_F + 3); k2.c0 = w.ld0(VE_F + 4); k2.c1 = w.ld0(VE_F + 5);
    k3.c0 = w.ld0(VE_F + 6); k3.c1 = w.ld0(VE_F + 7); k4.c0 = w.ld0(VE_F + 8); k4.c1 = w.ld0(VE_F + 9); k5.c0 = w.ld0(VE_F + 10); k5.c1 = w.ld0(VE_F + 11);
    if constexpr (DO_SQR) {
      Fp2 x3 = fp2_mul_xi(k3), x4 = fp2_mul_xi(k4), x5 = fp2_mul_xi(k5);
      w.park(0, fp2_dotp(pp(k0, k0), pp2(k1, x5), pp2(k2, x4), pp(k3, x3)));
      w.park(1, fp2_dotp(pp2(k0, k1), pp2(k2, x5), pp2(k3, x4)));
      w.park(2, fp2_dotp(pp2(k0, k2), pp(k1, k1), pp2(k3, x5), pp(k4, x4)));
      w.park(3, fp2_dotp(pp2(k0, k3), pp2(k1, k2), pp2(k4, x5)));
      f4 = fp2_dotp(pp2(k0, k4), pp2(k1, k3), pp(k2, k2), pp(k5, x5));
      f5 = fp2_dotp(pp2(k0, k5), pp2(k1, k4), pp2(k2, k3));
    } else {
      w.park(0, k0); w.park(1, k1); w.park(2, k2); w.park(3, k3); f4 = k4; f5 = k5;
    }
  }
  for (int q = 0; q < G; q++) {
    w.sel(q);
    const bool dead = ((deadmask >> q) & 1u) != 0;
    G2Line l;
    {
      G2Proj t; t.x = vld2(w, VE_T); t.y = vld2(w, VE_T + 2); t.z = vld2(w, VE_T + 4);
      if (kind == 0) {
        l = g2_double_step(t);
      } else {
        G2Aff b; b.x = vld2(w, VE_B); b.y = vld2(w, VE_B + 2);
        if (kind == 2) b = g2_neg(b);
        else if (kind == 3) b = g2_psi_affine(b);
        else if (kind == 4) b = g2_neg(g2_psi2_affine(b));
        l = g2_add_step(t, b);
      }
      vst2(w, VE_T, t.x); vst2(w, VE_T + 2, t.y); vst2(w, VE_T + 4, t.z);
    }
    BN_SCHED_FENCE();
    Fp px = w.ld(VE_AX), py = w.ld(VE_AY);
    Fp2 d0 = fp2_mul_fp(l.r0, py), d3 = fp2_mul_fp(l.r1, px), d4 = l.r2;
    Fp2 x3 = fp2_mul_xi(d3), x4 = fp2_mul_xi(d4);
    BN_SCHED_FENCE();
    Fp2 k0 = w.unpark(0), k1 = w.unpark(1), k2 = w.unpark(2), k3 = w.unpark(3), k4 = f4, k5 = f5;
    w.park(0, fp2_select(dead, k0, fp2_dotp(pp(d0, k0), pp(x3, k5), pp(x4, k3))));
    w.park(1, fp2_select(dead, k1, fp2_dotp(pp(d0, k1), pp(d3, k0), pp(x4, k4))));
    w.park(2, fp2_select(dead, k2, fp2_dotp(pp(d0, k2), pp(d3, k1), pp(x4, k5))));
    w.park(3, fp2_select(dead, k3, fp2_dotp(pp(d0, k3), pp(d3, k2), pp(d4, k0))));
    Fp2 n4 = fp2_select(dead, k4, fp2_dotp(pp(d0, k4), pp(d3, k3), pp(d4, k1)));
    f5 = fp2_select(dead, k5, fp2_dotp(pp(d0, k5), pp(d3, k4), pp(d4, k2)));
    f4 = n4;
  }
  {
    Fp2 k0 = w.unpark(0), k1 = w.unpark(1), k2 = w.unpark(2), k3 = w.unpark(3);
    w.st0(VE_F, k0.c0); w.st0(VE_F + 1, k0.c1); w.st0(VE_F + 2, k1.c0); w.st0(VE_F + 3, k1.c1); w.st0(VE_F + 4, k2.c0); w.st0(VE_F + 5, k2.c1);
    w.st0(VE_F + 6, k3.c0); w.st0(VE_F + 7, k3.c1); w.st0(VE_F + 8, f4.c0); w.st0(VE_F + 9, f4.c1); w.st0(VE_F + 10, f5.c0); w.st0(VE_F + 11, f5.c1);
  }
}

template <bool DO_SQR, class W>
BN_HD void vm_miller_step_fixed3(W& w, int e, const FixedLine& l0, int e_p0, bool inf0, const FixedLine& l1, int e_p1, bool inf1,
                                 const FixedLine& l2, int e_p2, bool inf2) {
  Fp2 f4, f5;
  {
    Fp2 k0 = vld2(w, e), k1 = vld2(w, e + 2), k2 = vld2(w, e + 4), k3 = vld2(w, e + 6), k4 = vld2(w, e + 8), k5 = vld2(w, e + 10);
    if constexpr (DO_SQR) {
      Fp2 x3 = fp2_mul_xi(k3), x4 = fp2_mul_xi(k4), x5 = fp2_mul_xi(k5);
      w.park(0, fp2_dotp(pp(k0, k0), pp2(k1, x5), pp2(k2, x4), pp(k3, x3)));
      w.park(1, fp2_dotp(pp2(k0, k1), pp2(k2, x5), pp2(k3, x4)));
      w.park(2, fp2_dotp(pp2(k0, k2), pp(k1, k1), pp2(k3, x5), pp(k4, x4)));
      w.park(3, fp2_dotp(pp2(k0, k3), pp2(k1, k2), pp2(k4, x5)));
      f4 = fp2_dotp(pp2(k0, k4), pp2(k1, k3), pp(k2, k2), pp(k5, x5));
      f5 = fp2_dotp(pp2(k0, k5), pp2(k1, k4), pp2(k2, k3));
    } else {
      w.park(0, k0); w.park(1, k1); w.park(2, k2); w.park(3, k3); f4 = k4; f5 = k5;
    }
  }
  for (int t = 0; t < 2; t++) {
    const FixedLine& l = t == 0 ? l0 : l1;
    const bool inf = t == 0 ? inf0 : inf1;
    const int e_p = t == 0 ? e_p0 : e_p1;
    BN_SCHED_FENCE();
    Fp px = w.ld(e_p), d0 = w.ld(e_p + 1);
    Fp2 d3 = fp2_mul_fp(l.m, px);
    Fp2 x3 = fp2_mul_xi(d3);
    const Fp2 &d4 = l.c, &x4 = l.xc;
    Fp2 k0 = w.unpark(0), k1 = w.unpark(1), k2 = w.unpark(2), k3 = w.unpark(3), k4 = f4, k5 = f5;
    w.park(0, fp2_select(inf, k0, fp2_dot_line(d0, k0, x3, k5, x4, k3)));
    w.park(1, fp2_select(inf, k1, fp2_dot_line(d0, k1, d3, k0, x4, k4)));
    w.park(2, fp2_select(inf, k2, fp2_dot_line(d0, k2, d3, k1, x4, k5)));
    w.park(3, fp2_select(inf, k3, fp2_dot_line(d0, k3, d3, k2, d4, k0)));
    f4 = fp2_select(inf, k4, fp2_dot_line(d0, k4, d3, k3, d4, k1));
    f5 = fp2_select(inf, k5, fp2_dot_line(d0, k5, d3, k4, d4, k2));
  }
  {
    BN_SCHED_FENCE();
    Fp px = w.ld(e_p2), d0 = w.ld(e_p2 + 1);
    Fp2 d3 = fp2_mul_fp(l2.m, px);
    Fp2 x3 = fp2_mul_xi(d3);
    const Fp2 &d4 = l2.c, &x4 = l2.xc;
    Fp2 k0 = w.unpark(0), k1 = w.unpark(1), k2 = w.unpark(2), k3 = w.unpark(3);
    const Fp2 &k4 = f4, &k5 = f5;
    vst2(w, e, fp2_select(inf2, k0, fp2_dotk(kfp(k0, d0), kp(x3, k5), kp(x4, k3))));
    vst2(w, e + 2, fp2_select(inf2, k1, fp2_dotk(kfp(k1, d0), kp(d3, k0), kp(x4, k4))));
    vst2(w, e + 4, fp2_select(inf2, k2, fp2_dotk(kfp(k2, d0), kp(d3, k1), kp(x4, k5))));
    vst2(w, e + 6, fp2_select(inf2, k3, fp2_dotk(kfp(k3, d0), kp(d3, k2), kp(d4, k0))));
    vst2(w, e + 8, fp2_select(inf2, k4, fp2_dotk(kfp(k4, d0), kp(d3, k3), kp(d4, k1))));
    vst2(w, e + 10, fp2_select(inf2, k5, fp2_dotk(kfp(k5, d0), kp(d3, k4), kp(d4, k2))));
  }
}

template <class W>
BN_HD void vm_rlc_neutral(W& w, int n_public, bool with_f = true) {
  if (with_f) {
    w.st(VE_F, fp_one());
    for (int e = 1; e < 12; e++) w.st(VE_F + e, fp_zero());
  }
  w.st(RLC_C, fp_zero()); w.st(RLC_C + 1, fp_one()); w.st(RLC_C + 2, fp_zero());
  for (int j = 0; j <= n_public; j++) w.st(RLC_T + j, fr8_to_slot(fr8_zero()));
}
template <class W>
BN_HD void vm_rlc_fold(W& w, int n_public, bool with_f = true) {
  if (with_f) vm_f12_mul(w, VE_F, VE_F, RLC_HI + VE_F, false);
  {
    G1Proj a, b;
    a.x = w.ld(RLC_C); a.y = w.ld(RLC_C + 1); a.z = w.ld(RLC_C + 2);
    b.x = w.ld(RLC_HI + RLC_C); b.y = w.ld(RLC_HI + RLC_C + 1); b.z = w.ld(RLC_HI + RLC_C + 2);
    BN_SETB(a.x, 1.01, 0.5); BN_SETB(a.y, 1.01, 0.5); BN_SETB(a.z, 1.01, 0.5); BN_SETB(b.x, 1.01, 0.5); BN_SETB(b.y, 1.01, 0.5); BN_SETB(b.z, 1.01, 0.5);
    G1Proj s = g1_add(a, b);
    w.st(RLC_C, fp_reduce(s.x)); w.st(RLC_C + 1, fp_reduce(s.y)); w.st(RLC_C + 2, fp_reduce(s.z));
  }
  for (int j = 0; j <= n_public; j++)
    w.st(RLC_T + j, fr8_to_slot(fr8_add(fr8_from_slot(w.ld(RLC_T + j)), fr8_from_slot(w.ld(RLC_HI + RLC_T + j)))));
}
template <class TL>
BN_HD G1Proj g1_window_sum(G1Proj acc, const Fr8& k, const TL& entry) {
  uint32_t sw[8];
#pragma unroll
  for (int i = 0; i < 8; i++) sw[i] = k.w[i];
  for (int wi = 0; wi < MSM_FW_WINDOWS; wi++) {
    const uint32_t dig = sw[0] & MSM_FW_ENTRIES;
#pragma unroll
    for (int i = 0; i < 7; i++) sw[i] = (sw[i] >> MSM_FW_BITS) | (sw[i + 1] << (32 - MSM_FW_BITS));
    sw[7] >>= MSM_FW_BITS;
    if (dig != 0) acc = g1_add_mixed(acc, entry(wi, (int)dig - 1));
  }
  return acc;
}
template <class W>
BN_HD int vm_rlc_group_store(W& w, const G1Proj& Pa, const G1Proj& L) {
  G1Proj Cg; Cg.x = w.ld(RLC_C); Cg.y = w.ld(RLC_C + 1); Cg.z = w.ld(RLC_C + 2);
  BN_SETB(Cg.x, 1.01, 0.5); BN_SETB(Cg.y, 1.01, 0.5); BN_SETB(Cg.z, 1.01, 0.5);
  const bool ia = g1_is_identity(Pa), il = g1_is_identity(L), ic = g1_is_identity(Cg);
  Fp za = fp_select(ia, fp_one(), fp_reduce(fp_norm(Pa.z))), zl = fp_select(il, fp_one(), fp_reduce(fp_norm(L.z))), zc = fp_select(ic, fp_one(), fp_reduce(fp_norm(Cg.z)));
  Fp zal = fp_mul(za, zl);
  Fp inv = fp_inv(fp_mul(zal, zc));
  Fp izc = fp_mul(inv, zal);
  Fp izal = fp_mul(inv, zc);
  Fp iza = fp_mul(izal, zl), izl = fp_mul(izal, za);
  w.st(VE_AX, fp_mul(Pa.x, iza)); w.st(VE_AY, fp_select(ia, fp_one(), fp_mul(Pa.y, iza)));
  w.st(VE_LX, fp_mul(L.x, izl)); w.st(VE_LY, fp_select(il, fp_one(), fp_mul(L.y, izl)));
  w.st(VE_CX, fp_mul(Cg.x, izc)); w.st(VE_CY, fp_select(ic, fp_one(), fp_mul(Cg.y, izc)));
  w.st(RLC_ACC, fp_one());
  for (int e = 1; e < 12; e++) w.st(RLC_ACC + e, fp_zero());
  return (il ? 1 : 0) | (ic ? 2 : 0) | (ia ? 4 : 0);
}
template <class W, class TAB>
BN_HD int vm_rlc_group_points(W& w, int n_public, const TAB& tab) {
  const Fr8 t0 = fr8_from_slot(w.ld(RLC_T));
  G1Proj Pa = g1_window_sum(g1_identity(), t0, [&](int wi, int d) { return tab(0, wi, d); });
  G1Proj L = g1_window_sum(g1_identity(), t0, [&](int wi, int d) { return tab(1, wi, d); });
  for (int j = 1; j <= n_public; j++) {
    const Fr8 tj = fr8_from_slot(w.ld(RLC_T + j));
    L = g1_window_sum(L, tj, [&](int wi, int d) { return tab(1 + j, wi, d); });
  }
  return vm_rlc_group_store(w, Pa, L);
}
BN_HD void fr_acc_mul64(uint32_t acc[11], const uint32_t x[8], uint32_t k_lo, uint32_t k_hi) {
  uint32_t p[10];
  uint64_t c = 0;
#pragma unroll
  for (int j = 0; j < 8; j++) { uint64_t s = (uint64_t)x[j] * k_lo + c; p[j] = (uint32_t)s; c = s >> 32; }
  p[8] = (uint32_t)c; p[9] = 0; c = 0;
#pragma unroll
  for (int j = 0; j < 8; j++) { uint64_t s = (uint64_t)x[j] * k_hi + p[j + 1] + c; p[j + 1] = (uint32_t)s; c = s >> 32; }
  p[9] = (uint32_t)c;
  c = 0;
#pragma unroll
  for (int j = 0; j < 10; j++) { c += (uint64_t)acc[j] + p[j]; acc[j] = (uint32_t)c; c >>= 32; }
  acc[10] += (uint32_t)c;
}
BN_HD Fr8 fr_acc_redc128(const uint32_t acc[11]) {
  uint32_t t[13];
#pragma unroll
  for (int i = 0; i < 11; i++) t[i] = acc[i];
  t[11] = 0; t[12] = 0;
#pragma unroll
  for (int s = 0; s < 4; s++) {
    const uint32_t m = t[s] * BN_R_NINV32;
    uint64_t c = 0;
#pragma unroll
    for (int j = 0; j < 8; j++) { uint64_t v = (uint64_t)m * bn_r_word(j) + t[s + j] + c; t[s + j] = (uint32_t)v; c = v >> 32; }
#pragma unroll
    for (int j = s + 8; j < 13; j++) { c += t[j]; t[j] = (uint32_t)c; c >>= 32; }
  }
  uint32_t u[9];
#pragma unroll
  for (int i = 0; i < 9; i++) u[i] = t[4 + i];
  return fr8_cond_sub_r(u);
}
template <class LX, class LW>
BN_HD Fr8 rlc_group_scalar(uint32_t g, int j, uint32_t n, const RlcPlan& p, const LX& load_input, const LW& load_weight) {
  uint32_t a1[11], a2[11];
#pragma unroll
  for (int i = 0; i < 11; i++) { a1[i] = 0; a2[i] = 0; }
  rlc_for_each_member(g, n, p, [&](uint32_t i) {
    uint32_t k[4];
    if (!load_weight(i, k)) return;
    uint32_t x[8];
    load_input(i, j, x);
    fr_acc_mul64(a1, x, k[0], k[1]);
    fr_acc_mul64(a2, x, k[2], k[3]);
  });
  Fr8 r2, t128 = fr8_zero(), lam;
#pragma unroll
// ... 15 lines not shown
```

### snark-bn254-verifier_amd/csrc/bn254_tower.h

```cpp
#pragma once
#include "bn254_fp.h"

namespace bn254 {

struct Fp2 { Fp c0, c1; };
struct Fp6 { Fp2 c0, c1, c2; };
struct Fp12 { Fp6 c0, c1; };

BN_HD Fp2 fp2_zero() { Fp2 r; r.c0 = fp_zero(); r.c1 = fp_zero(); return r; }
BN_HD Fp2 fp2_one() { Fp2 r; r.c0 = fp_one(); r.c1 = fp_zero(); return r; }
BN_HD Fp2 fp2_add(const Fp2& a, const Fp2& b) { Fp2 r; r.c0 = fp_add(a.c0, b.c0); r.c1 = fp_add(a.c1, b.c1); return r; }
BN_HD Fp2 fp2_sub(const Fp2& a, const Fp2& b) { Fp2 r; r.c0 = fp_sub(a.c0, b.c0); r.c1 = fp_sub(a.c1, b.c1); return r; }
BN_HD Fp2 fp2_add_lazy(const Fp2& a, const Fp2& b) { Fp2 r; r.c0 = fp_add_lazy(a.c0, b.c0); r.c1 = fp_add_lazy(a.c1, b.c1); return r; }
BN_HD Fp2 fp2_sub_lazy(const Fp2& a, const Fp2& b) { Fp2 r; r.c0 = fp_sub_lazy(a.c0, b.c0); r.c1 = fp_sub_lazy(a.c1, b.c1); return r; }
BN_HD Fp2 fp2_neg(const Fp2& a) { Fp2 r; r.c0 = fp_neg(a.c0); r.c1 = fp_neg(a.c1); return r; }
BN_HD Fp2 fp2_dbl(const Fp2& a) { Fp2 r; r.c0 = fp_dbl(a.c0); r.c1 = fp_dbl(a.c1); return r; }
BN_HD Fp2 fp2_conj(const Fp2& a) { Fp2 r; r.c0 = a.c0; r.c1 = fp_neg(a.c1); return r; }
BN_HD Fp2 fp2_reduce(const Fp2& a) { Fp2 r; r.c0 = fp_reduce(a.c0); r.c1 = fp_reduce(a.c1); return r; }
BN_HD Fp2 fp2_norm(const Fp2& a) { Fp2 r; r.c0 = fp_norm(a.c0); r.c1 = fp_norm(a.c1); return r; }
BN_HD Fp2 fp2_select(bool c, const Fp2& a, const Fp2& b) { Fp2 r; r.c0 = fp_select(c, a.c0, b.c0); r.c1 = fp_select(c, a.c1, b.c1); return r; }
BN_HD Fp2 fp2_sub2(const Fp2& a, const Fp2& b, const Fp2& c) {
  Fp2 r; r.c0 = fp_norm(fp_sub_lazy(fp_sub_lazy(a.c0, b.c0), c.c0)); r.c1 = fp_norm(fp_sub_lazy(fp_sub_lazy(a.c1, b.c1), c.c1)); return r;
}

template <int W>
struct P2 {
  const Fp2& x;
  const Fp2& y;
};
BN_HD P2<1> pp(const Fp2& x, const Fp2& y) { return P2<1>{x, y}; }
BN_HD P2<-1> pm(const Fp2& x, const Fp2& y) { return P2<-1>{x, y}; }
BN_HD P2<2> pp2(const Fp2& x, const Fp2& y) { return P2<2>{x, y}; }
BN_HD P2<-2> pm2(const Fp2& x, const Fp2& y) { return P2<-2>{x, y}; }
template <int... W>
BN_HD Fp2 fp2_dotp(const P2<W>&... t) {
  Fp2 r;
  r.c0 = fp_dot(dterm<W>(t.x.c0, t.y.c0)..., dterm<-W>(t.x.c1, t.y.c1)...);
  r.c1 = fp_dot(dterm<W>(t.x.c0, t.y.c1)..., dterm<W>(t.x.c1, t.y.c0)...);
  return r;
}

struct KAcc { uint64_t re, im, a[2][2]; };
#define BN_KCOL_RANGE constexpr int LO = K < BN_NL ? 0 : K - (BN_NL - 1); constexpr int HI = K < BN_NL ? K : BN_NL - 1
BN_HD uint64_t bn_dmul(int32_t a, int32_t b) { return (uint64_t)((int64_t)a * (int64_t)b); }
template <int AW>
struct KProd {
  Fp x0, nx1, y0, y1, sxw, sy;
  static constexpr int cls = AW;
  template <int K> BN_HD void col(KAcc& c) const {
    BN_KCOL_RANGE;
#pragma unroll
    for (int i = LO; i <= HI; i++) {
      c.a[AW - 1][0] += bn_dmul(x0.v[i], y0.v[K - i]);
      c.a[AW - 1][1] += bn_dmul(nx1.v[i], y1.v[K - i]);
      c.im += bn_dmul(sxw.v[i], sy.v[K - i]);
    }
  }
#if BN_TRACKING
  double cap_re() const { return 9.0 * AW * (x0.lb * y0.lb + nx1.lb * y1.lb); }
  double cap_im() const { return 9.0 * AW * (x0.lb * y1.lb + nx1.lb * y0.lb); }
  double val_re() const { return AW * (x0.vb * y0.vb + nx1.vb * y1.vb); }
  double val_im() const { return AW * (x0.vb * y1.vb + nx1.vb * y0.vb); }
  void check() const { if (sxw.lb > 3.99 || sy.lb > 3.99) fp_dbg_fail("fp2_dotk: operand sum overflows a digit", sxw.lb + sy.lb); }
#endif
};
struct KDirect {
  Fp ure, vre, uim, vim;
  static constexpr int cls = 0;
  template <int K> BN_HD void col(KAcc& c) const {
    BN_KCOL_RANGE;
#pragma unroll
    for (int i = LO; i <= HI; i++) {
      c.re += bn_dmul(ure.v[i], vre.v[K - i]);
      c.im += bn_dmul(uim.v[i], vim.v[K - i]);
    }
  }
#if BN_TRACKING
  double cap_re() const { return 9.0 * ure.lb * vre.lb; }
  double cap_im() const { return 9.0 * uim.lb * vim.lb; }
  double val_re() const { return ure.vb * vre.vb; }
  double val_im() const { return uim.vb * vim.vb; }
  void check() const { if (ure.lb > 3.99 || vre.lb > 3.99 || uim.lb > 3.99 || vim.lb > 3.99) fp_dbg_fail("fp2_dotk: direct operand overflows a digit", ure.lb); }
#endif
};
template <int AW, bool NEG> BN_HD KProd<AW> kprod(const Fp2& x, const Fp2& y) {
  KProd<AW> t;
  t.x0 = NEG ? fp_neg(x.c0) : x.c0; t.nx1 = NEG ? x.c1 : fp_neg(x.c1); t.y0 = y.c0; t.y1 = y.c1;
  t.sy = fp_add_lazy(y.c0, y.c1);
#pragma unroll
  for (int i = 0; i < BN_NL; i++) t.sxw.v[i] = (NEG ? -AW : AW) * (x.c0.v[i] + x.c1.v[i]);
  BN_SETB(t.sxw, AW * (BN_VB(x.c0) + BN_VB(x.c1)), AW * (BN_LBD(x.c0) + BN_LBD(x.c1)));
  return t;
}
BN_HD KProd<1> kp(const Fp2& x, const Fp2& y) { return kprod<1, false>(x, y); }
BN_HD KProd<1> km(const Fp2& x, const Fp2& y) { return kprod<1, true>(x, y); }
BN_HD KProd<2> kp2(const Fp2& x, const Fp2& y) { return kprod<2, false>(x, y); }
BN_HD KProd<2> km2(const Fp2& x, const Fp2& y) { return kprod<2, true>(x, y); }
BN_HD KDirect ksq(const Fp2& x) {
  KDirect t; t.ure = fp_add_lazy(x.c0, x.c1); t.vre = fp_sub_lazy(x.c0, x.c1); t.uim = fp_dbl_lazy(x.c0); t.vim = x.c1; return t;
}
BN_HD KDirect kfp(const Fp2& x, const Fp& f) { KDirect t; t.ure = x.c0; t.vre = f; t.uim = x.c1; t.vim = f; return t; }

template <int K, class... T>
BN_HD void dotk_step(int64_t& cre, int64_t& cim, int32_t (&mre)[BN_NL], int32_t (&mim)[BN_NL], Fp2& r, const T&... t) {
  constexpr bool has1 = ((T::cls == 1) || ...), has2 = ((T::cls == 2) || ...);
  KAcc c; c.re = (uint64_t)cre; c.im = (uint64_t)cim;
  c.a[0][0] = c.a[0][1] = c.a[1][0] = c.a[1][1] = 0;
  (t.template col<K>(c), ...);
  if constexpr (K < BN_NL) {
#pragma unroll
    for (int i = 0; i < K; i++) { c.re += bn_dmul(mre[i], bn_p_limb(K - i)); c.im += bn_dmul(mim[i], bn_p_limb(K - i)); }
  } else {
#pragma unroll
    for (int i = K - (BN_NL - 1); i < BN_NL; i++) { c.re += bn_dmul(mre[i], bn_p_limb(K - i)); c.im += bn_dmul(mim[i], bn_p_limb(K - i)); }
  }
  if (has1) { c.re += c.a[0][0] + c.a[0][1]; c.im += c.a[0][1] - c.a[0][0]; }
  if (has2) { c.re += (c.a[1][0] + c.a[1][1]) << 1; c.im += (c.a[1][1] - c.a[1][0]) << 1; }
  if constexpr (K < BN_NL) {
    mre[K] = bn_sext29((uint32_t)c.re * BN_PINV);
    mim[K] = bn_sext29((uint32_t)c.im * BN_PINV);
    c.re += bn_dmul(mre[K], bn_p_limb(0));
    c.im += bn_dmul(mim[K], bn_p_limb(0));
    cre = (int64_t)c.re >> BN_LB;
    cim = (int64_t)c.im >> BN_LB;
  } else {
    c.re += BN_HALF; c.im += BN_HALF;
    r.c0.v[K - BN_NL] = (int32_t)((uint32_t)c.re & BN_MASK) - BN_HALF;
    r.c1.v[K - BN_NL] = (int32_t)((uint32_t)c.im & BN_MASK) - BN_HALF;
    cre = (int64_t)c.re >> BN_LB;
    cim = (int64_t)c.im >> BN_LB;
  }
}
template <int... KS, class... T>
BN_HD void dotk_all(std::integer_sequence<int, KS...>, int64_t& cre, int64_t& cim, int32_t (&mre)[BN_NL], int32_t (&mim)[BN_NL], Fp2& r, const T&... t) {
  (dotk_step<KS, T...>(cre, cim, mre, mim, r, t...), ...);
}
template <class... T>
BN_HD Fp2 fp2_dotk(const T&... t) {
  BN_SCHED_FENCE();
  int64_t cre = 0, cim = 0;
  int32_t mre[BN_NL], mim[BN_NL];
  Fp2 r;
  dotk_all(std::make_integer_sequence<int, 2 * BN_NL - 1>{}, cre, cim, mre, mim, r, t...);
  r.c0.v[BN_NL - 1] = (int32_t)cre;
  r.c1.v[BN_NL - 1] = (int32_t)cim;
  BN_SCHED_FENCE();
#if BN_TRACKING
  (t.check(), ...);
  double cr = (t.cap_re() + ...), ci = (t.cap_im() + ...);
  if (cr + 9.0 * 0.25 + 0.01 > 32.0 || ci + 9.0 * 0.25 + 0.01 > 32.0) fp_dbg_fail("fp2_dotk: accumulator may overflow", cr > ci ? cr : ci);
  BN_SETB(r.c0, 1.0 + (t.val_re() + ...) / 169.0 + 1e-6, 0.5);
  BN_SETB(r.c1, 1.0 + (t.val_im() + ...) / 169.0 + 1e-6, 0.5);
#endif
  return r;
}
BN_HD Fp2 fp2_mul(const Fp2& a, const Fp2& b) { return fp2_dotp(pp(a, b)); }
BN_HD Fp2 fp2_sqr(const Fp2& a) {
  Fp2 r;
  r.c0 = fp_mul(fp_add(a.c0, a.c1), fp_sub_lazy(a.c0, a.c1));
  r.c1 = fp_mul(fp_add_lazy(a.c0, a.c0), a.c1);
  return r;
}
BN_HD Fp2 fp2_mul_fp(const Fp2& a, const Fp& f) { Fp2 r; r.c0 = fp_mul(a.c0, f); r.c1 = fp_mul(a.c1, f); return r; }
BN_HD Fp2 fp2_mul_xi(const Fp2& a) {
  Fp2 r;
  r.c0 = fp_lincomb_reduce(9, a.c0, -1, a.c1);
  r.c1 = fp_lincomb_reduce(1, a.c0, 9, a.c1);
  return r;
}
BN_HD Fp2 fp2_mul_small(const Fp2& a, int32_t k) {
  Fp2 r;
  r.c0 = fp_lincomb_reduce(k, a.c0, 0, a.c0);
  r.c1 = fp_lincomb_reduce(k, a.c1, 0, a.c1);
  return r;
}
BN_HD Fp2 fp2_lincomb_reduce(int32_t k1, const Fp2& a, int32_t k2, const Fp2& b) {
  Fp2 r;
  r.c0 = fp_lincomb_reduce(k1, a.c0, k2, b.c0);
  r.c1 = fp_lincomb_reduce(k1, a.c1, k2, b.c1);
  return r;
}
BN_HD Fp2 fp2_inv(const Fp2& a) {
  Fp n = fp_dot(dplus(a.c0, a.c0), dplus(a.c1, a.c1));
  Fp ni = fp_inv(n);
  Fp2 r;
  r.c0 = fp_mul(a.c0, ni);
  r.c1 = fp_neg(fp_mul(a.c1, ni));
  return r;
}
BN_HD bool fp2_is_zero(const Fp2& a) { return fp_is_zero(a.c0) & fp_is_zero(a.c1); }
BN_HD bool fp2_eq(const Fp2& a, const Fp2& b) { return fp_eq(a.c0, b.c0) & fp_eq(a.c1, b.c1); }
BN_HD Fp2 fp2_from_limbs(const int32_t* c0, const int32_t* c1) { Fp2 r; r.c0 = fp_from_limbs(c0); r.c1 = fp_from_limbs(c1); return r; }

BN_HD_NOINLINE Fp2 fp2_mul_nl(const Fp2& a, const Fp2& b) { return fp2_mul(a, b); }
BN_HD_NOINLINE Fp2 fp2_sqr_nl(const Fp2& a) { return fp2_sqr(a); }

BN_HD Fp6 fp6_zero() { Fp6 r; r.c0 = fp2_zero(); r.c1 = fp2_zero(); r.c2 = fp2_zero(); return r; }
BN_HD Fp6 fp6_one() { Fp6 r; r.c0 = fp2_one(); r.c1 = fp2_zero(); r.c2 = fp2_zero(); return r; }
BN_HD Fp6 fp6_add(const Fp6& a, const Fp6& b) { Fp6 r; r.c0 = fp2_add(a.c0, b.c0); r.c1 = fp2_add(a.c1, b.c1); r.c2 = fp2_add(a.c2, b.c2); return r; }
BN_HD Fp6 fp6_sub(const Fp6& a, const Fp6& b) { Fp6 r; r.c0 = fp2_sub(a.c0, b.c0); r.c1 = fp2_sub(a.c1, b.c1); r.c2 = fp2_sub(a.c2, b.c2); return r; }
BN_HD Fp6 fp6_neg(const Fp6& a) { Fp6 r; r.c0 = fp2_neg(a.c0); r.c1 = fp2_neg(a.c1); r.c2 = fp2_neg(a.c2); return r; }
BN_HD Fp6 fp6_reduce(const Fp6& a) { Fp6 r; r.c0 = fp2_reduce(a.c0); r.c1 = fp2_reduce(a.c1); r.c2 = fp2_reduce(a.c2); return r; }
BN_HD Fp6 fp6_select(bool c, const Fp6& a, const Fp6& b) { Fp6 r; r.c0 = fp2_select(c, a.c0, b.c0); r.c1 = fp2_select(c, a.c1, b.c1); r.c2 = fp2_select(c, a.c2, b.c2); return r; }
BN_HD Fp6 fp6_mul_v(const Fp6& a) { Fp6 r; r.c0 = fp2_mul_xi(a.c2); r.c1 = a.c0; r.c2 = a.c1; return r; }
BN_HD Fp6 fp6_mul(const Fp6& x, const Fp6& y) {
  Fp2 Y1 = fp2_mul_xi(y.c1), Y2 = fp2_mul_xi(y.c2);
  Fp6 r;
  r.c0 = fp2_dotk(kp(x.c0, y.c0), kp(x.c1, Y2), kp(x.c2, Y1));
  r.c1 = fp2_dotk(kp(x.c0, y.c1), kp(x.c1, y.c0), kp(x.c2, Y2));
  r.c2 = fp2_dotk(kp(x.c0, y.c2), kp(x.c1, y.c1), kp(x.c2, y.c0));
  return r;
}
BN_HD Fp6 fp6_mul_plain(const Fp6& x, const Fp6& y) {
  Fp2 Y1 = fp2_mul_xi(y.c1), Y2 = fp2_mul_xi(y.c2);
  Fp6 r;
  r.c0 = fp2_dotp(pp(x.c0, y.c0), pp(x.c1, Y2), pp(x.c2, Y1));
  r.c1 = fp2_dotp(pp(x.c0, y.c1), pp(x.c1, y.c0), pp(x.c2, Y2));
  r.c2 = fp2_dotp(pp(x.c0, y.c2), pp(x.c1, y.c1), pp(x.c2, y.c0));
  return r;
}
BN_HD Fp6 fp6_sqr(const Fp6& x) {
  Fp2 X2 = fp2_mul_xi(x.c2);
  Fp6 r;
  r.c0 = fp2_dotp(pp(x.c0, x.c0), pp2(x.c1, X2));
  r.c1 = fp2_dotp(pp2(x.c0, x.c1), pp(x.c2, X2));
  r.c2 = fp2_dotp(pp2(x.c0, x.c2), pp(x.c1, x.c1));
  return r;
}
BN_HD Fp6 fp6_mul_fp2(const Fp6& a, const Fp2& b) { Fp6 r; r.c0 = fp2_mul(a.c0, b); r.c1 = fp2_mul(a.c1, b); r.c2 = fp2_mul(a.c2, b); return r; }
BN_HD_NOINLINE Fp6 fp6_mul_nl(const Fp6& a, const Fp6& b) { return fp6_mul(a, b); }
BN_HD Fp6 fp6_inv(const Fp6& a) {
  Fp2 X1 = fp2_mul_xi(a.c1), X2 = fp2_mul_xi(a.c2);
  Fp2 A = fp2_dotp(pp(a.c0, a.c0), pm(X1, a.c2));
  Fp2 B = fp2_dotp(pp(X2, a.c2), pm(a.c0, a.c1));
  Fp2 C = fp2_dotp(pp(a.c1, a.c1), pm(a.c0, a.c2));
  Fp2 F = fp2_dotp(pp(a.c0, A), pp(X2, B), pp(X1, C));
  Fp2 Fi = fp2_inv(F);
  Fp6 r;
  r.c0 = fp2_mul(A, Fi); r.c1 = fp2_mul(B, Fi); r.c2 = fp2_mul(C, Fi);
  return r;
}

BN_HD Fp12 fp12_one() { Fp12 r; r.c0 = fp6_one(); r.c1 = fp6_zero(); return r; }
BN_HD Fp12 fp12_conj(const Fp12& a) { Fp12 r; r.c0 = a.c0; r.c1 = fp6_neg(a.c1); return r; }
BN_HD Fp12 fp12_reduce(const Fp12& a) { Fp12 r; r.c0 = fp6_reduce(a.c0); r.c1 = fp6_reduce(a.c1); return r; }
BN_HD Fp12 fp12_select(bool c, const Fp12& a, const Fp12& b) { Fp12 r; r.c0 = fp6_select(c, a.c0, b.c0); r.c1 = fp6_select(c, a.c1, b.c1); return r; }
#define K0(f) ((f).c0.c0)
#define K1(f) ((f).c1.c0)
#define K2(f) ((f).c0.c1)
#define K3(f) ((f).c1.c1)
#define K4(f) ((f).c0.c2)
#define K5(f) ((f).c1.c2)

BN_HD Fp12 fp12_mul(const Fp12& a, const Fp12& b) {
  Fp6 v0 = fp6_mul_nl(a.c0, b.c0);
  Fp6 v1 = fp6_mul_nl(a.c1, b.c1);
  Fp6 s = fp6_mul_nl(fp6_add(a.c0, a.c1), fp6_add(b.c0, b.c1));
  Fp12 r;
  Fp2 x = fp2_mul_xi(v1.c2);
  r.c0.c0 = fp2_add(v0.c0, x); r.c0.c1 = fp2_add(v0.c1, v1.c0); r.c0.c2 = fp2_add(v0.c2, v1.c1);
  r.c1.c0 = fp2_sub2(s.c0, v0.c0, v1.c0); r.c1.c1 = fp2_sub2(s.c1, v0.c1, v1.c1); r.c1.c2 = fp2_sub2(s.c2, v0.c2, v1.c2);
  return r;
}
BN_HD Fp12 fp12_sqr(const Fp12& f) {
  Fp2 x3 = fp2_mul_xi(K3(f)), x4 = fp2_mul_xi(K4(f)), x5 = fp2_mul_xi(K5(f));
  Fp12 r;
  K0(r) = fp2_dotp(pp(K0(f), K0(f)), pp2(K1(f), x5), pp2(K2(f), x4), pp(K3(f), x3));
  K1(r) = fp2_dotp(pp2(K0(f), K1(f)), pp2(K2(f), x5), pp2(K3(f), x4));
  K2(r) = fp2_dotp(pp2(K0(f), K2(f)), pp(K1(f), K1(f)), pp2(K3(f), x5), pp(K4(f), x4));
  K3(r) = fp2_dotp(pp2(K0(f), K3(f)), pp2(K1(f), K2(f)), pp2(K4(f), x5));
  K4(r) = fp2_dotp(pp2(K0(f), K4(f)), pp2(K1(f), K3(f)), pp(K2(f), K2(f)), pp(K5(f), x5));
  K5(r) = fp2_dotp(pp2(K0(f), K5(f)), pp2(K1(f), K4(f)), pp2(K2(f), K3(f)));
  return r;
}
BN_HD Fp12 fp12_mul_by_034(const Fp12& f, const Fp2& d0, const Fp2& d3, const Fp2& d4) {
  Fp2 x3 = fp2_mul_xi(d3), x4 = fp2_mul_xi(d4);
  Fp12 r;
  K0(r) = fp2_dotp(pp(d0, K0(f)), pp(x3, K5(f)), pp(x4, K3(f)));
  K1(r) = fp2_dotp(pp(d0, K1(f)), pp(d3, K0(f)), pp(x4, K4(f)));
  K2(r) = fp2_dotp(pp(d0, K2(f)), pp(d3, K1(f)), pp(x4, K5(f)));
  K3(r) = fp2_dotp(pp(d0, K3(f)), pp(d3, K2(f)), pp(d4, K0(f)));
  K4(r) = fp2_dotp(pp(d0, K4(f)), pp(d3, K3(f)), pp(d4, K1(f)));
  K5(r) = fp2_dotp(pp(d0, K5(f)), pp(d3, K4(f)), pp(d4, K2(f)));
  return r;
}
BN_HD Fp2 fp2_dot_line(const Fp& d0, const Fp2& k, const Fp2& da, const Fp2& ka, const Fp2& db, const Fp2& kb) {
  Fp2 r;
  r.c0 = fp_dot(dplus(d0, k.c0), dplus(da.c0, ka.c0), dminus(da.c1, ka.c1), dplus(db.c0, kb.c0), dminus(db.c1, kb.c1));
  r.c1 = fp_dot(dplus(d0, k.c1), dplus(da.c0, ka.c1), dplus(da.c1, ka.c0), dplus(db.c0, kb.c1), dplus(db.c1, kb.c0));
  return r;
}
BN_HD Fp12 fp12_mul_by_034_fp(const Fp12& f, const Fp& d0, const Fp2& d3, const Fp2& d4, const Fp2& x4) {
  Fp2 x3 = fp2_mul_xi(d3);
  Fp12 r;
  K0(r) = fp2_dot_line(d0, K0(f), x3, K5(f), x4, K3(f));
  K1(r) = fp2_dot_line(d0, K1(f), d3, K0(f), x4, K4(f));
  K2(r) = fp2_dot_line(d0, K2(f), d3, K1(f), x4, K5(f));
  K3(r) = fp2_dot_line(d0, K3(f), d3, K2(f), d4, K0(f));
  K4(r) = fp2_dot_line(d0, K4(f), d3, K3(f), d4, K1(f));
  K5(r) = fp2_dot_line(d0, K5(f), d3, K4(f), d4, K2(f));
  return r;
}
BN_HD Fp12 fp12_inv(const Fp12& a) {
  Fp6 s0 = fp6_sqr(a.c0), s1 = fp6_mul_v(fp6_sqr(a.c1));
  Fp6 di = fp6_inv(fp6_sub(s0, s1));
  Fp12 r;
  r.c0 = fp6_mul_nl(a.c0, di);
  r.c1 = fp6_neg(fp6_mul_nl(a.c1, di));
  return r;
}
BN_HD Fp2 frob_coeff(int j, int k) {
  const int32_t(*t)[2][BN_NL] = j == 1 ? BN_FROB_G1 : j == 2 ? BN_FROB_G2 : BN_FROB_G3;
  return fp2_from_limbs(t[k][0], t[k][1]);
}
BN_HD Fp12 fp12_frob(const Fp12& a, int j) {
  Fp12 r;
  const bool odd = (j & 1) != 0;
  Fp2 x1 = odd ? fp2_conj(K1(a)) : K1(a), x2 = odd ? fp2_conj(K2(a)) : K2(a), x3 = odd ? fp2_conj(K3(a)) : K3(a);
  Fp2 x4 = odd ? fp2_conj(K4(a)) : K4(a), x5 = odd ? fp2_conj(K5(a)) : K5(a);
  K0(r) = odd ? fp2_conj(K0(a)) : K0(a);
  if (j == 2) {
    K1(r) = fp2_mul_fp(x1, frob_coeff(2, 1).c0); K2(r) = fp2_mul_fp(x2, frob_coeff(2, 2).c0);
    K3(r) = fp2_mul_fp(x3, frob_coeff(2, 3).c0); K4(r) = fp2_mul_fp(x4, frob_coeff(2, 4).c0);
    K5(r) = fp2_mul_fp(x5, frob_coeff(2, 5).c0);
  } else {
    K1(r) = fp2_mul_nl(x1, frob_coeff(j, 1)); K2(r) = fp2_mul_nl(x2, frob_coeff(j, 2));
    K3(r) = fp2_mul_nl(x3, frob_coeff(j, 3)); K4(r) = fp2_mul_nl(x4, frob_coeff(j, 4));
    K5(r) = fp2_mul_nl(x5, frob_coeff(j, 5));
  }
  return r;
}
BN_HD void gs_pair(Fp2& za, Fp2& zb, const Fp2& a, const Fp2& b, const Fp2& sub, const Fp2& add, bool xi_on_cross) {
  Fp2 xb = fp2_mul_xi(b);
  Fp2 S = fp2_dotp(pp(xb, b), pp(a, a));
  Fp2 T = xi_on_cross ? fp2_dotp(pp2(a, xb)) : fp2_dotp(pp2(a, b));
  za = fp2_lincomb_reduce(3, S, -2, sub);
  zb = fp2_lincomb_reduce(3, T, 2, add);
}
BN_HD Fp12 fp12_cyclo_sqr(const Fp12& x) {
  Fp12 z;
  gs_pair(z.c0.c0, z.c1.c1, x.c0.c0, x.c1.c1, x.c0.c0, x.c1.c1, false);
  gs_pair(z.c0.c1, z.c1.c2, x.c1.c0, x.c0.c2, x.c0.c1, x.c1.c2, false);
  gs_pair(z.c0.c2, z.c1.c0, x.c0.c1, x.c1.c2, x.c0.c2, x.c1.c0, true);
  return z;
}
BN_HD bool fp6_eq(const Fp6& a, const Fp6& b) { return fp2_eq(a.c0, b.c0) & fp2_eq(a.c1, b.c1) & fp2_eq(a.c2, b.c2); }
BN_HD bool fp12_eq(const Fp12& a, const Fp12& b) { return fp6_eq(a.c0, b.c0) & fp6_eq(a.c1, b.c1); }

}
```

### snark-bn254-verifier_amd/csrc/bn254_vm.h

```cpp
#pragma once
#include "bn254_pairing.h"

namespace bn254 {

enum {
  VE_AX = 0, VE_AY = 1, VE_B = 2 , VE_CX = 6, VE_CY = 7, VE_LX = 8, VE_LY = 9,
  VE_F = 10,
  VE_T = 22,
  VE_S0 = 22, VE_S1 = 34, VE_S2 = 46, VE_S3 = 58, VE_S4 = 70,
  VE_UT0 = 82,
  VE_TMPA = 94, VE_TMPB = 100,
  VE_UT1 = 106, VE_UT2 = 118,
  VE_COUNT = 130,
  VE_CONJ = 0x100
};
enum { VP_MAX_PAIRS = 8, VP_PAIR_ELEMS = 12, VP_EXTRA = VE_S1, VP_IDENT = VE_CX };
static_assert(VP_EXTRA + (VP_MAX_PAIRS - 1) * VP_PAIR_ELEMS <= VE_COUNT, "the extra pairs fit the slots of the final exponentiation");
BN_HD int vp_p(int j) { return j == 0 ? (int)VE_AX : VP_EXTRA + VP_PAIR_ELEMS * (j - 1); }
BN_HD int vp_q(int j) { return j == 0 ? (int)VE_B : VP_EXTRA + VP_PAIR_ELEMS * (j - 1) + 2; }
BN_HD int vp_t(int j) { return j == 0 ? (int)VE_T : VP_EXTRA + VP_PAIR_ELEMS * (j - 1) + 6; }
BN_HD bool ve_conj(int e) { return (e & VE_CONJ) != 0; }
BN_HD int ve_elem(int e) { return e & ~VE_CONJ; }

template <class W> BN_HD Fp2 vld2(W& w, int e) { Fp2 r; r.c0 = w.ld(e); r.c1 = w.ld(e + 1); return r; }
template <class W> BN_HD void vst2(W& w, int e, const Fp2& a) { w.st(e, a.c0); w.st(e + 1, a.c1); }
template <class W> BN_HD Fp6 vld6(W& w, int e) { Fp6 r; r.c0 = vld2(w, e); r.c1 = vld2(w, e + 2); r.c2 = vld2(w, e + 4); return r; }
template <class W> BN_HD void vst6(W& w, int e, const Fp6& a) { vst2(w, e, a.c0); vst2(w, e + 2, a.c1); vst2(w, e + 4, a.c2); }

template <class W>
BN_HD void vm_f12_sqr(W& w, int e) {
  Fp2 k0 = vld2(w, e), k1 = vld2(w, e + 2), k2 = vld2(w, e + 4), k3 = vld2(w, e + 6), k4 = vld2(w, e + 8), k5 = vld2(w, e + 10);
  Fp2 x3 = fp2_mul_xi(k3), x4 = fp2_mul_xi(k4), x5 = fp2_mul_xi(k5);
  vst2(w, e, fp2_dotp(pp(k0, k0), pp2(k1, x5), pp2(k2, x4), pp(k3, x3)));
  vst2(w, e + 2, fp2_dotp(pp2(k0, k1), pp2(k2, x5), pp2(k3, x4)));
  vst2(w, e + 4, fp2_dotp(pp2(k0, k2), pp(k1, k1), pp2(k3, x5), pp(k4, x4)));
  vst2(w, e + 6, fp2_dotp(pp2(k0, k3), pp2(k1, k2), pp2(k4, x5)));
  vst2(w, e + 8, fp2_dotp(pp2(k0, k4), pp2(k1, k3), pp(k2, k2), pp(k5, x5)));
  vst2(w, e + 10, fp2_dotp(pp2(k0, k5), pp2(k1, k4), pp2(k2, k3)));
}
template <class W>
BN_HD void vm_f12_mul_line_fixed(W& w, int e, const FixedLine& l, int e_px, bool inf) {
  Fp px = w.ld(e_px), d0 = w.ld(e_px + 1);
  Fp2 d3 = fp2_mul_fp(l.m, px);
  Fp2 x3 = fp2_mul_xi(d3);
  const Fp2 &d4 = l.c, &x4 = l.xc;
  Fp2 k0 = vld2(w, e), k1 = vld2(w, e + 2), k2 = vld2(w, e + 4), k3 = vld2(w, e + 6), k4 = vld2(w, e + 8), k5 = vld2(w, e + 10);
  vst2(w, e, fp2_select(inf, k0, fp2_dotk(kfp(k0, d0), kp(x3, k5), kp(x4, k3))));
  vst2(w, e + 2, fp2_select(inf, k1, fp2_dotk(kfp(k1, d0), kp(d3, k0), kp(x4, k4))));
  vst2(w, e + 4, fp2_select(inf, k2, fp2_dotk(kfp(k2, d0), kp(d3, k1), kp(x4, k5))));
  vst2(w, e + 6, fp2_select(inf, k3, fp2_dotk(kfp(k3, d0), kp(d3, k2), kp(d4, k0))));
  vst2(w, e + 8, fp2_select(inf, k4, fp2_dotk(kfp(k4, d0), kp(d3, k3), kp(d4, k1))));
  vst2(w, e + 10, fp2_select(inf, k5, fp2_dotk(kfp(k5, d0), kp(d3, k4), kp(d4, k2))));
}
template <class W>
BN_HD void vm_f12_mul_line_fixed2(W& w, int e, const FixedLine& l1, int e_px1, bool inf1, const FixedLine& l2, int e_px2, bool inf2) {
  Fp2 r4, r5;
  {
    Fp px = w.ld(e_px1), d0 = w.ld(e_px1 + 1);
    Fp2 d3 = fp2_mul_fp(l1.m, px);
    Fp2 x3 = fp2_mul_xi(d3);
    const Fp2 &d4 = l1.c, &x4 = l1.xc;
    Fp2 k0 = vld2(w, e), k1 = vld2(w, e + 2), k2 = vld2(w, e + 4), k3 = vld2(w, e + 6), k4 = vld2(w, e + 8), k5 = vld2(w, e + 10);
    w.park(0, fp2_select(inf1, k0, fp2_dot_line(d0, k0, x3, k5, x4, k3)));
    w.park(1, fp2_select(inf1, k1, fp2_dot_line(d0, k1, d3, k0, x4, k4)));
    w.park(2, fp2_select(inf1, k2, fp2_dot_line(d0, k2, d3, k1, x4, k5)));
    w.park(3, fp2_select(inf1, k3, fp2_dot_line(d0, k3, d3, k2, d4, k0)));
    r4 = fp2_select(inf1, k4, fp2_dot_line(d0, k4, d3, k3, d4, k1));
    r5 = fp2_select(inf1, k5, fp2_dot_line(d0, k5, d3, k4, d4, k2));
  }
  {
    Fp px = w.ld(e_px2), d0 = w.ld(e_px2 + 1);
    Fp2 d3 = fp2_mul_fp(l2.m, px);
    Fp2 x3 = fp2_mul_xi(d3);
    const Fp2 &d4 = l2.c, &x4 = l2.xc;
    Fp2 k0 = w.unpark(0), k1 = w.unpark(1), k2 = w.unpark(2), k3 = w.unpark(3);
    const Fp2 &k4 = r4, &k5 = r5;
    vst2(w, e, fp2_select(inf2, k0, fp2_dotk(kfp(k0, d0), kp(x3, k5), kp(x4, k3))));
    vst2(w, e + 2, fp2_select(inf2, k1, fp2_dotk(kfp(k1, d0), kp(d3, k0), kp(x4, k4))));
    vst2(w, e + 4, fp2_select(inf2, k2, fp2_dotk(kfp(k2, d0), kp(d3, k1), kp(x4, k5))));
    vst2(w, e + 6, fp2_select(inf2, k3, fp2_dotk(kfp(k3, d0), kp(d3, k2), kp(d4, k0))));
    vst2(w, e + 8, fp2_select(inf2, k4, fp2_dotk(kfp(k4, d0), kp(d3, k3), kp(d4, k1))));
    vst2(w, e + 10, fp2_select(inf2, k5, fp2_dotk(kfp(k5, d0), kp(d3, k4), kp(d4, k2))));
  }
}
template <class W>
BN_HD void vm_f12_mul_line_regs(W& w, int e, const G2Line& l, int e_px) {
  Fp px = w.ld(e_px), py = w.ld(e_px + 1);
  Fp2 d0 = fp2_mul_fp(l.r0, py), d3 = fp2_mul_fp(l.r1, px), d4 = l.r2;
  Fp2 x3 = fp2_mul_xi(d3), x4 = fp2_mul_xi(d4);
  Fp2 k0 = vld2(w, e), k1 = vld2(w, e + 2), k2 = vld2(w, e + 4), k3 = vld2(w, e + 6), k4 = vld2(w, e + 8), k5 = vld2(w, e + 10);
  vst2(w, e, fp2_dotp(pp(d0, k0), pp(x3, k5), pp(x4, k3)));
  vst2(w, e + 2, fp2_dotp(pp(d0, k1), pp(d3, k0), pp(x4, k4)));
  vst2(w, e + 4, fp2_dotp(pp(d0, k2), pp(d3, k1), pp(x4, k5)));
  vst2(w, e + 6, fp2_dotp(pp(d0, k3), pp(d3, k2), pp(d4, k0)));
  vst2(w, e + 8, fp2_dotp(pp(d0, k4), pp(d3, k3), pp(d4, k1)));
  vst2(w, e + 10, fp2_dotp(pp(d0, k5), pp(d3, k4), pp(d4, k2)));
}
template <class W>
BN_HD void vm_miller_dbl_var(W& w, int e_t, int e, int e_px) {
  G2Proj t; t.x = vld2(w, e_t); t.y = vld2(w, e_t + 2); t.z = vld2(w, e_t + 4);
  G2Line l = g2_double_step(t);
  vst2(w, e_t, t.x); vst2(w, e_t + 2, t.y); vst2(w, e_t + 4, t.z);
  vm_f12_mul_line_regs(w, e, l, e_px);
}
template <class W>
BN_HD void vm_miller_add_var(W& w, int e_t, int e_b, int which, int e, int e_px) {
  G2Aff q; q.x = vld2(w, e_b); q.y = vld2(w, e_b + 2);
  if (which == 1) q = g2_neg(q);
  else if (which == 2) q = g2_psi_affine(q);
  else if (which == 3) q = g2_neg(g2_psi2_affine(q));
  G2Proj t; t.x = vld2(w, e_t); t.y = vld2(w, e_t + 2); t.z = vld2(w, e_t + 4);
  G2Line l = g2_add_step(t, q);
  vst2(w, e_t, t.x); vst2(w, e_t + 2, t.y); vst2(w, e_t + 4, t.z);
  vm_f12_mul_line_regs(w, e, l, e_px);
}

template <class W>
BN_HD void vm_miller_sqr_dbl_var(W& w, int e_t, int e, int e_px) {
  Fp2 r4, r5;
  {
    Fp2 k0 = vld2(w, e), k1 = vld2(w, e + 2), k2 = vld2(w, e + 4), k3 = vld2(w, e + 6), k4 = vld2(w, e + 8), k5 = vld2(w, e + 10);
    Fp2 x3 = fp2_mul_xi(k3), x4 = fp2_mul_xi(k4), x5 = fp2_mul_xi(k5);
    w.park(0, fp2_dotp(pp(k0, k0), pp2(k1, x5), pp2(k2, x4), pp(k3, x3)));
    w.park(1, fp2_dotp(pp2(k0, k1), pp2(k2, x5), pp2(k3, x4)));
    w.park(2, fp2_dotp(pp2(k0, k2), pp(k1, k1), pp2(k3, x5), pp(k4, x4)));
    w.park(3, fp2_dotp(pp2(k0, k3), pp2(k1, k2), pp2(k4, x5)));
    r4 = fp2_dotp(pp2(k0, k4), pp2(k1, k3), pp(k2, k2), pp(k5, x5));
    r5 = fp2_dotp(pp2(k0, k5), pp2(k1, k4), pp2(k2, k3));
  }
  G2Line l;
  {
    G2Proj t; t.x = vld2(w, e_t); t.y = vld2(w, e_t + 2); t.z = vld2(w, e_t + 4);
    l = g2_double_step(t);
    vst2(w, e_t, t.x); vst2(w, e_t + 2, t.y); vst2(w, e_t + 4, t.z);
  }
  BN_SCHED_FENCE();
  Fp px = w.ld(e_px), py = w.ld(e_px + 1);
  Fp2 d0 = fp2_mul_fp(l.r0, py), d3 = fp2_mul_fp(l.r1, px), d4 = l.r2;
  Fp2 x3 = fp2_mul_xi(d3), x4 = fp2_mul_xi(d4);
  BN_SCHED_FENCE();
  Fp2 k0 = w.unpark(0), k1 = w.unpark(1), k2 = w.unpark(2), k3 = w.unpark(3);
  const Fp2 &k4 = r4, &k5 = r5;
  vst2(w, e, fp2_dotp(pp(d0, k0), pp(x3, k5), pp(x4, k3)));
  vst2(w, e + 2, fp2_dotp(pp(d0, k1), pp(d3, k0), pp(x4, k4)));
  vst2(w, e + 4, fp2_dotp(pp(d0, k2), pp(d3, k1), pp(x4, k5)));
  vst2(w, e + 6, fp2_dotp(pp(d0, k3), pp(d3, k2), pp(d4, k0)));
  vst2(w, e + 8, fp2_dotp(pp(d0, k4), pp(d3, k3), pp(d4, k1)));
  vst2(w, e + 10, fp2_dotp(pp(d0, k5), pp(d3, k4), pp(d4, k2)));
}

template <bool DO_SQR, class W>
BN_HD void vm_miller_step(W& w, int kind, int e_t, int e_b, int e, int e_pa, const FixedLine& l0, int e_p0, bool inf0,
                          const FixedLine& l1, int e_p1, bool inf1) {
  Fp2 f4, f5;
  if constexpr (DO_SQR) {
    Fp2 k0 = vld2(w, e), k1 = vld2(w, e + 2), k2 = vld2(w, e + 4), k3 = vld2(w, e + 6), k4 = vld2(w, e + 8), k5 = vld2(w, e + 10);
    Fp2 x3 = fp2_mul_xi(k3), x4 = fp2_mul_xi(k4), x5 = fp2_mul_xi(k5);
    w.park(0, fp2_dotp(pp(k0, k0), pp2(k1, x5), pp2(k2, x4), pp(k3, x3)));
    w.park(1, fp2_dotp(pp2(k0, k1), pp2(k2, x5), pp2(k3, x4)));
    w.park(2, fp2_dotp(pp2(k0, k2), pp(k1, k1), pp2(k3, x5), pp(k4, x4)));
    w.park(3, fp2_dotp(pp2(k0, k3), pp2(k1, k2), pp2(k4, x5)));
    f4 = fp2_dotp(pp2(k0, k4), pp2(k1, k3), pp(k2, k2), pp(k5, x5));
    f5 = fp2_dotp(pp2(k0, k5), pp2(k1, k4), pp2(k2, k3));
  }
  G2Line l;
  {
    G2Proj t; t.x = vld2(w, e_t); t.y = vld2(w, e_t + 2); t.z = vld2(w, e_t + 4);
    if (kind == 0) {
      l = g2_double_step(t);
    } else {
      G2Aff q; q.x = vld2(w, e_b); q.y = vld2(w, e_b + 2);
      if (kind == 2) q = g2_neg(q);
      else if (kind == 3) q = g2_psi_affine(q);
      else if (kind == 4) q = g2_neg(g2_psi2_affine(q));
      l = g2_add_step(t, q);
    }
    vst2(w, e_t, t.x); vst2(w, e_t + 2, t.y); vst2(w, e_t + 4, t.z);
  }
  {
    Fp px = w.ld(e_pa), py = w.ld(e_pa + 1);
    Fp2 d0 = fp2_mul_fp(l.r0, py), d3 = fp2_mul_fp(l.r1, px), d4 = l.r2;
    Fp2 x3 = fp2_mul_xi(d3), x4 = fp2_mul_xi(d4);
    Fp2 k0, k1, k2, k3, k4, k5;
    if constexpr (DO_SQR) { k0 = w.unpark(0); k1 = w.unpark(1); k2 = w.unpark(2); k3 = w.unpark(3); k4 = f4; k5 = f5; }
    else { k0 = vld2(w, e); k1 = vld2(w, e + 2); k2 = vld2(w, e + 4); k3 = vld2(w, e + 6); k4 = vld2(w, e + 8); k5 = vld2(w, e + 10); }
    w.park(0, fp2_dotp(pp(d0, k0), pp(x3, k5), pp(x4, k3)));
    w.park(1, fp2_dotp(pp(d0, k1), pp(d3, k0), pp(x4, k4)));
    w.park(2, fp2_dotp(pp(d0, k2), pp(d3, k1), pp(x4, k5)));
    w.park(3, fp2_dotp(pp(d0, k3), pp(d3, k2), pp(d4, k0)));
    Fp2 n4 = fp2_dotp(pp(d0, k4), pp(d3, k3), pp(d4, k1));
    f5 = fp2_dotp(pp(d0, k5), pp(d3, k4), pp(d4, k2));
    f4 = n4;
  }
  {
    Fp px = w.ld(e_p0), d0 = w.ld(e_p0 + 1);
    Fp2 d3 = fp2_mul_fp(l0.m, px);
    Fp2 x3 = fp2_mul_xi(d3);
    const Fp2 &d4 = l0.c, &x4 = l0.xc;
    Fp2 k0 = w.unpark(0), k1 = w.unpark(1), k2 = w.unpark(2), k3 = w.unpark(3), k4 = f4, k5 = f5;
    w.park(0, fp2_select(inf0, k0, fp2_dot_line(d0, k0, x3, k5, x4, k3)));
    w.park(1, fp2_select(inf0, k1, fp2_dot_line(d0, k1, d3, k0, x4, k4)));
    w.park(2, fp2_select(inf0, k2, fp2_dot_line(d0, k2, d3, k1, x4, k5)));
    w.park(3, fp2_select(inf0, k3, fp2_dot_line(d0, k3, d3, k2, d4, k0)));
    f4 = fp2_select(inf0, k4, fp2_dot_line(d0, k4, d3, k3, d4, k1));
    f5 = fp2_select(inf0, k5, fp2_dot_line(d0, k5, d3, k4, d4, k2));
  }
  {
    Fp px = w.ld(e_p1), d0 = w.ld(e_p1 + 1);
    Fp2 d3 = fp2_mul_fp(l1.m, px);
    Fp2 x3 = fp2_mul_xi(d3);
    const Fp2 &d4 = l1.c, &x4 = l1.xc;
    Fp2 k0 = w.unpark(0), k1 = w.unpark(1), k2 = w.unpark(2), k3 = w.unpark(3);
    const Fp2 &k4 = f4, &k5 = f5;
    vst2(w, e, fp2_select(inf1, k0, fp2_dotk(kfp(k0, d0), kp(x3, k5), kp(x4, k3))));
    vst2(w, e + 2, fp2_select(inf1, k1, fp2_dotk(kfp(k1, d0), kp(d3, k0), kp(x4, k4))));
    vst2(w, e + 4, fp2_select(inf1, k2, fp2_dotk(kfp(k2, d0), kp(d3, k1), kp(x4, k5))));
    vst2(w, e + 6, fp2_select(inf1, k3, fp2_dotk(kfp(k3, d0), kp(d3, k2), kp(d4, k0))));
    vst2(w, e + 8, fp2_select(inf1, k4, fp2_dotk(kfp(k4, d0), kp(d3, k3), kp(d4, k1))));
    vst2(w, e + 10, fp2_select(inf1, k5, fp2_dotk(kfp(k5, d0), kp(d3, k4), kp(d4, k2))));
  }
}

template <class W> BN_HD void mf_load(W& w, int e, Fp2& f4, Fp2& f5) {
  w.park(0, vld2(w, e)); w.park(1, vld2(w, e + 2)); w.park(2, vld2(w, e + 4)); w.park(3, vld2(w, e + 6));
  f4 = vld2(w, e + 8); f5 = vld2(w, e + 10);
}
template <class W> BN_HD void mf_store(W& w, int e, const Fp2& f4, const Fp2& f5) {
  vst2(w, e, w.unpark(0)); vst2(w, e + 2, w.unpark(1)); vst2(w, e + 4, w.unpark(2)); vst2(w, e + 6, w.unpark(3));
  vst2(w, e + 8, f4); vst2(w, e + 10, f5);
}
template <class W> BN_HD void mf_sqr(W& w, Fp2& f4, Fp2& f5) {
  Fp2 k0 = w.unpark(0), k1 = w.unpark(1), k2 = w.unpark(2), k3 = w.unpark(3), k4 = f4, k5 = f5;
  Fp2 x3 = fp2_mul_xi(k3), x4 = fp2_mul_xi(k4), x5 = fp2_mul_xi(k5);
  w.park(0, fp2_dotp(pp(k0, k0), pp2(k1, x5), pp2(k2, x4), pp(k3, x3)));
  w.park(1, fp2_dotp(pp2(k0, k1), pp2(k2, x5), pp2(k3, x4)));
  w.park(2, fp2_dotp(pp2(k0, k2), pp(k1, k1), pp2(k3, x5), pp(k4, x4)));
  w.park(3, fp2_dotp(pp2(k0, k3), pp2(k1, k2), pp2(k4, x5)));
  Fp2 n4 = fp2_dotp(pp2(k0, k4), pp2(k1, k3), pp(k2, k2), pp(k5, x5));
  f5 = fp2_dotp(pp2(k0, k5), pp2(k1, k4), pp2(k2, k3));
  f4 = n4;
}
template <class W> BN_HD G2Line mf_g2(W& w, int kind, int e_t, int e_b) {
  G2Line l;
  G2Proj t; t.x = vld2(w, e_t); t.y = vld2(w, e_t + 2); t.z = vld2(w, e_t + 4);
  if (kind == 0) {
    l = g2_double_step(t);
  } else {
    G2Aff q; q.x = vld2(w, e_b); q.y = vld2(w, e_b + 2);
    if (kind == 2) q = g2_neg(q);
    else if (kind == 3) q = g2_psi_affine(q);
    else if (kind == 4) q = g2_neg(g2_psi2_affine(q));
    l = g2_add_step(t, q);
  }
  vst2(w, e_t, t.x); vst2(w, e_t + 2, t.y); vst2(w, e_t + 4, t.z);
  return l;
}
template <class W> BN_HD void mf_line_var(W& w, const G2Line& l, int e_pa, Fp2& f4, Fp2& f5) {
  Fp px = w.ld(e_pa), py = w.ld(e_pa + 1);
  Fp2 d0 = fp2_mul_fp(l.r0, py), d3 = fp2_mul_fp(l.r1, px), d4 = l.r2;
  Fp2 x3 = fp2_mul_xi(d3), x4 = fp2_mul_xi(d4);
  Fp2 k0 = w.unpark(0), k1 = w.unpark(1), k2 = w.unpark(2), k3 = w.unpark(3), k4 = f4, k5 = f5;
  w.park(0, fp2_dotp(pp(d0, k0), pp(x3, k5), pp(x4, k3)));
  w.park(1, fp2_dotp(pp(d0, k1), pp(d3, k0), pp(x4, k4)));
  w.park(2, fp2_dotp(pp(d0, k2), pp(d3, k1), pp(x4, k5)));
  w.park(3, fp2_dotp(pp(d0, k3), pp(d3, k2), pp(d4, k0)));
  Fp2 n4 = fp2_dotp(pp(d0, k4), pp(d3, k3), pp(d4, k1));
  f5 = fp2_dotp(pp(d0, k5), pp(d3, k4), pp(d4, k2));
  f4 = n4;
}
template <class W> BN_HD void mf_line_fixed(W& w, const FixedLine& l, int e_p, bool inf, Fp2& f4, Fp2& f5) {
  Fp px = w.ld(e_p), d0 = w.ld(e_p + 1);
  Fp2 d3 = fp2_mul_fp(l.m, px);
  Fp2 x3 = fp2_mul_xi(d3);
  const Fp2 &d4 = l.c, &x4 = l.xc;
  Fp2 k0 = w.unpark(0), k1 = w.unpark(1), k2 = w.unpark(2), k3 = w.unpark(3);
  const Fp2 k4 = f4, k5 = f5;
  w.park(0, fp2_select(inf, k0, fp2_dotk(kfp(k0, d0), kp(x3, k5), kp(x4, k3))));
  w.park(1, fp2_select(inf, k1, fp2_dotk(kfp(k1, d0), kp(d3, k0), kp(x4, k4))));
  w.park(2, fp2_select(inf, k2, fp2_dotk(kfp(k2, d0), kp(d3, k1), kp(x4, k5))));
  w.park(3, fp2_select(inf, k3, fp2_dotk(kfp(k3, d0), kp(d3, k2), kp(d4, k0))));
  f4 = fp2_select(inf, k4, fp2_dotk(kfp(k4, d0), kp(d3, k3), kp(d4, k1)));
  f5 = fp2_select(inf, k5, fp2_dotk(kfp(k5, d0), kp(d3, k4), kp(d4, k2)));
}
template <class W> BN_HD void mf_init(W& w, int e_t, int e_b, Fp2& f4, Fp2& f5) {
  w.park(0, fp2_one()); w.park(1, fp2_zero()); w.park(2, fp2_zero()); w.park(3, fp2_zero());
  f4 = fp2_zero(); f5 = fp2_zero();
  vst2(w, e_t, vld2(w, e_b)); vst2(w, e_t + 2, vld2(w, e_b + 2)); vst2(w, e_t + 4, fp2_one());
}
enum { MR_FOLD_INIT = 1, MR_FOLD_ATE = 2 };
template <class W> BN_HD bool vm_g2_ate_check(W& w, int e_t, int e_b);
template <class W, class LINES, class KINDS>
BN_HD bool vm_miller_run(W& w, const LINES& lines, const KINDS& kinds, int s_begin, int s_end, int e_t, int e_b, int e, int e_pa, int e_p0, bool inf0, int e_p1, bool inf1,
                         int fold = 0) {
  Fp2 f4, f5;
  if ((fold & MR_FOLD_INIT) && s_begin == 0) mf_init(w, e_t, e_b, f4, f5);
  else mf_load(w, e, f4, f5);
  for (int s = s_begin; s < s_end; s++) {
    const int kind = kinds.get(s);
    if (kind == 0) {
      if (s != 0) mf_sqr(w, f4, f5);
      BN_SCHED_FENCE();
      G2Line l = mf_g2(w, 0, e_t, e_b);
      mf_line_var(w, l, e_pa, f4, f5);
    } else {
      G2Line l = mf_g2(w, kind, e_t, e_b);
      mf_line_var(w, l, e_pa, f4, f5);
    }
    BN_SCHED_FENCE();
    mf_line_fixed(w, lines.get(0, s), e_p0, inf0, f4, f5);
    mf_line_fixed(w, lines.get(1, s), e_p1, inf1, f4, f5);
  }
  mf_store(w, e, f4, f5);
  if ((fold & MR_FOLD_ATE) && s_end == BN_ATE_STEPS) return vm_g2_ate_check(w, e_t, e_b);
  return true;
}

template <class W, class LINES, class KINDS>
BN_HD void vm_miller_run_fixed2(W& w, const LINES& lines, const KINDS& kinds, int s_begin, int s_end, int e, int e_p0, bool inf0, int e_p1, bool inf1) {
  Fp2 f4, f5;
  mf_load(w, e, f4, f5);
  for (int s = s_begin; s < s_end; s++) {
    if (kinds.get(s) == 0 && s != 0) mf_sqr(w, f4, f5);
    BN_SCHED_FENCE();
    mf_line_fixed(w, lines.get(0, s), e_p0, inf0, f4, f5);
    mf_line_fixed(w, lines.get(1, s), e_p1, inf1, f4, f5);
  }
  mf_store(w, e, f4, f5);
}

template <class W> BN_HD void mf_line_var_sel(W& w, const G2Line& l, int e_pa, bool skip, Fp2& f4, Fp2& f5) {
  Fp px = w.ld(e_pa), py = w.ld(e_pa + 1);
  Fp2 d0 = fp2_mul_fp(l.r0, py), d3 = fp2_mul_fp(l.r1, px), d4 = l.r2;
  Fp2 x3 = fp2_mul_xi(d3), x4 = fp2_mul_xi(d4);
  Fp2 k0 = w.unpark(0), k1 = w.unpark(1), k2 = w.unpark(2), k3 = w.unpark(3);
  const Fp2 k4 = f4, k5 = f5;
  w.park(0, fp2_select(skip, k0, fp2_dotp(pp(d0, k0), pp(x3, k5), pp(x4, k3))));
  w.park(1, fp2_select(skip, k1, fp2_dotp(pp(d0, k1), pp(d3, k0), pp(x4, k4))));
  w.park(2, fp2_select(skip, k2, fp2_dotp(pp(d0, k2), pp(d3, k1), pp(x4, k5))));
  w.park(3, fp2_select(skip, k3, fp2_dotp(pp(d0, k3), pp(d3, k2), pp(d4, k0))));
  f4 = fp2_select(skip, k4, fp2_dotp(pp(d0, k4), pp(d3, k3), pp(d4, k1)));
  f5 = fp2_select(skip, k5, fp2_dotp(pp(d0, k5), pp(d3, k4), pp(d4, k2)));
}
BN_HD bool vp_skips(uint32_t ident, int j) { return ((ident >> (2 * j)) & 3u) != 0; }
BN_HD bool vp_q_finite(uint32_t ident, int j) { return ((ident >> (2 * j + 1)) & 1u) == 0; }
template <class W, class KINDS>
BN_HD int vm_miller_run_var(W& w, const KINDS& kinds, int s_begin, int s_end, int np, uint32_t ident, int e, int fold = 0) {
  Fp2 f4, f5;
  if ((fold & MR_FOLD_INIT) && s_begin == 0) {
    mf_init(w, vp_t(0), vp_q(0), f4, f5);
    for (int j = 1; j < np; j++) { const int et = vp_t(j), eb = vp_q(j); vst2(w, et, vld2(w, eb)); vst2(w, et + 2, vld2(w, eb + 2)); vst2(w, et + 4, fp2_one()); }
  } else mf_load(w, e, f4, f5);
  for (int s = s_begin; s < s_end; s++) {
    const int kind = kinds.get(s);
    if (kind == 0) {
      if (s != 0) mf_sqr(w, f4, f5);
      for (int j = 0; j < np; j++) {
        BN_SCHED_FENCE();
        G2Line l = mf_g2(w, 0, vp_t(j), vp_q(j));
        mf_line_var_sel(w, l, vp_p(j), vp_skips(ident, j), f4, f5);
      }
    } else {
      for (int j = 0; j < np; j++) {
        BN_SCHED_FENCE();
        G2Line l = mf_g2(w, kind, vp_t(j), vp_q(j));
        mf_line_var_sel(w, l, vp_p(j), vp_skips(ident, j), f4, f5);
      }
    }
    BN_SCHED_FENCE();
  }
  mf_store(w, e, f4, f5);
  int failed = -1;
  if ((fold & MR_FOLD_ATE) && s_end == BN_ATE_STEPS)
    for (int j = 0; j < np; j++) {
      const bool ok = vm_g2_ate_check(w, vp_t(j), vp_q(j));
      if (failed < 0 && vp_q_finite(ident, j) && !ok) failed = j;
    }
  return failed;
}

BN_HD int vp_first(uint32_t m) { return __builtin_ctz(m); }
template <bool VAR, class W, class LINES, class KINDS>
BN_HD int vm_miller_run_mix(W& w, const LINES& lines, const KINDS& kinds, int s_begin, int s_end, uint32_t var_mask, uint32_t sh_mask, uint32_t ident, int e, int fold = 0) {
  Fp2 f4, f5;
  if ((fold & MR_FOLD_INIT) && s_begin == 0) {
    w.park(0, fp2_one()); w.park(1, fp2_zero()); w.park(2, fp2_zero()); w.park(3, fp2_zero());
    f4 = fp2_zero(); f5 = fp2_zero();
    if constexpr (VAR)
      for (uint32_t m = var_mask; m; m &= m - 1) { const int j = vp_first(m), et = vp_t(j), eb = vp_q(j); vst2(w, et, vld2(w, eb)); vst2(w, et + 2, vld2(w, eb + 2)); vst2(w, et + 4, fp2_one()); }
  } else mf_load(w, e, f4, f5);
  for (int s = s_begin; s < s_end; s++) {
    const int kind = kinds.get(s);
// ... 251 lines not shown
```

Measured before the change: 6.316 million.

## Chain multiply-accumulates through opaque accumulator and exploit squaring symmetry in dot products

Result: faster. 6.388 million, median of 6 (+1.1%).

```diff
diff --git a/snark-bn254-verifier_amd/csrc/bn254_fp.h b/snark-bn254-verifier_amd/csrc/bn254_fp.h
--- a/snark-bn254-verifier_amd/csrc/bn254_fp.h
+++ b/snark-bn254-verifier_amd/csrc/bn254_fp.h
@@ -34,6 +34,17 @@
 #define BN_SCHED_FENCE() __builtin_amdgcn_sched_barrier(0)
 #else
 #define BN_SCHED_FENCE() do { } while (0)
+#endif
+#if defined(__HIP_DEVICE_COMPILE__) && !defined(BN_NO_CARRY_RIDE)
+__device__ int64_t bn_opq_i64(int64_t) __asm("llvm.amdgcn.softwqm.i64");
+#define BN_OPQ(x) bn_opq_i64(x)
+#else
+#define BN_OPQ(x) (x)
+#endif
+#if defined(BN_NO_CARRY_RIDE)
+#define BN_RIDE_DEFAULT false
+#else
+#define BN_RIDE_DEFAULT true
 #endif
 
 #if defined(BN_TRACK_BOUNDS) && !defined(__HIP_DEVICE_COMPILE__)
@@ -92,6 +103,8 @@
     case 5: return BN_P5; case 6: return BN_P6; case 7: return BN_P7; default: return BN_P8;
   }
 }
+template <bool RIDE = BN_RIDE_DEFAULT> BN_HD void bn_ride(int64_t& acc, int32_t a, int32_t b) { acc = (RIDE ? BN_OPQ(acc) : acc) + (int64_t)a * (int64_t)b; }
+template <bool RIDE = BN_RIDE_DEFAULT> BN_HD void bn_ride(uint64_t& acc, int32_t a, int32_t b) { acc = (RIDE ? (uint64_t)BN_OPQ((int64_t)acc) : acc) + (uint64_t)((int64_t)a * (int64_t)b); }
 BN_HD int32_t bn_sext29(uint32_t x) { return (int32_t)(x << 3) >> 3; }
 
 BN_HD Fp fp_from_limbs(const int32_t* c) {
@@ -169,20 +182,37 @@
 #endif
   return r;
 }
+template <bool RIDE = BN_RIDE_DEFAULT>
 BN_HD Fp fp_lincomb_reduce(int32_t k1, const Fp& a, int32_t k2, const Fp& b) {
   const int64_t C = 1420063842;
   int64_t top = (int64_t)k1 * (int64_t)a.v[BN_NL - 1] + (int64_t)k2 * (int64_t)b.v[BN_NL - 1];
   int32_t q = (int32_t)((top * C) >> 52);
   Fp r;
-  int64_t acc = 0;
-#pragma unroll
-  for (int i = 0; i < BN_NL - 1; i++) {
-    acc += (int64_t)k1 * (int64_t)a.v[i] + (int64_t)k2 * (int64_t)b.v[i] - (int64_t)q * (int64_t)bn_p_limb(i) + BN_HALF;
-    r.v[i] = (int32_t)((uint32_t)acc & BN_MASK) - BN_HALF;
-    acc >>= BN_LB;
-  }
-  acc += top - (int64_t)q * (int64_t)bn_p_limb(BN_NL - 1);
-  r.v[BN_NL - 1] = (int32_t)acc;
+  if (RIDE) {
+    const int32_t nq = -q;
+    int64_t acc = (int64_t)k1 * (int64_t)a.v[0] + BN_HALF;
+#pragma unroll
+    for (int i = 0; i < BN_NL - 1; i++) {
+      if (i > 0) { acc += BN_HALF; bn_ride(acc, k1, a.v[i]); }
+      bn_ride(acc, k2, b.v[i]);
+      bn_ride(acc, nq, bn_p_limb(i));
+      r.v[i] = (int32_t)((uint32_t)acc & BN_MASK) - BN_HALF;
+      acc >>= BN_LB;
+    }
+    acc += top;
+    bn_ride(acc, nq, bn_p_limb(BN_NL - 1));
+    r.v[BN_NL - 1] = (int32_t)acc;
+  } else {
+    int64_t acc = 0;
+#pragma unroll
+    for (int i = 0; i < BN_NL - 1; i++) {
+      acc += (int64_t)k1 * (int64_t)a.v[i] + (int64_t)k2 * (int64_t)b.v[i] - (int64_t)q * (int64_t)bn_p_limb(i) + BN_HALF;
+      r.v[i] = (int32_t)((uint32_t)acc & BN_MASK) - BN_HALF;
+      acc >>= BN_LB;
+    }
+    acc += top - (int64_t)q * (int64_t)bn_p_limb(BN_NL - 1);
+    r.v[BN_NL - 1] = (int32_t)acc;
+  }
 #if BN_TRACKING
   if (a.vb * (k1 < 0 ? -k1 : k1) + b.vb * (k2 < 0 ? -k2 : k2) > 1e5) fp_dbg_fail("fp_lincomb_reduce: out of range", a.vb + b.vb);
   if (a.lb > 1.01 || b.lb > 1.01) fp_dbg_fail("fp_lincomb_reduce: digits too large", a.lb + b.lb);
@@ -190,74 +220,113 @@
 #endif
   return r;
 }
-BN_HD Fp fp_reduce(const Fp& a) { return fp_lincomb_reduce(1, a, 0, a); }
-
+BN_HD Fp fp_reduce(const Fp& a) { return fp_lincomb_reduce<false>(1, a, 0, a); }
+
+struct DotAcc { int64_t p1, m1, p2, m2; };
+#define BN_DCOL_RANGE constexpr int LO = K < BN_NL ? 0 : K - (BN_NL - 1); constexpr int HI = K < BN_NL ? K : BN_NL - 1
+template <int SIGN, int K, bool RIDE>
+BN_HD void dot_add(DotAcc& c, int32_t a, int32_t b) {
+  if (SIGN == 1 && K > 0) bn_ride<RIDE>(c.p1, a, b);
+  else if (SIGN == 1) c.p1 += (int64_t)a * (int64_t)b;
+  else if (SIGN == -1) c.m1 += (int64_t)a * (int64_t)b;
+  else if (SIGN == 2) c.p2 += (int64_t)a * (int64_t)b;
+  else c.m2 += (int64_t)a * (int64_t)b;
+}
 template <int SIGN>
 struct DotTerm {
   const Fp& a;
   const Fp& b;
+  static constexpr int cls = SIGN, cls_cross = SIGN;
+  template <int K, bool RIDE> BN_HD void col(DotAcc& c) const {
+    BN_DCOL_RANGE;
+#pragma unroll
+    for (int i = LO; i <= HI; i++) dot_add<SIGN, K, RIDE>(c, a.v[i], b.v[K - i]);
+  }
+#if BN_TRACKING
+  double cap() const { return 9.0 * (SIGN < 0 ? -SIGN : SIGN) * a.lb * b.lb; }
+  double val() const { return (SIGN < 0 ? -SIGN : SIGN) * a.vb * b.vb; }
+#endif
+};
+template <int SIGN>
+struct DotSq {
+  const Fp& a;
+  static constexpr int cls = SIGN, cls_cross = 2 * SIGN;
+  template <int K, bool RIDE> BN_HD void col(DotAcc& c) const {
+    BN_DCOL_RANGE;
+#pragma unroll
+    for (int i = LO; i <= HI; i++) {
+      if (!RIDE) dot_add<SIGN, K, RIDE>(c, a.v[i], a.v[K - i]);
+      else if (i < K - i) dot_add<2 * SIGN, K, RIDE>(c, a.v[i], a.v[K - i]);
+      else if (i == K - i) dot_add<SIGN, K, RIDE>(c, a.v[i], a.v[i]);
+    }
+  }
+#if BN_TRACKING
+  double cap() const { return 9.0 * a.lb * a.lb; }
+  double val() const { return a.vb * a.vb; }
+#endif
+};
+struct DotNone {
+  static constexpr int cls = 1, cls_cross = 1;
+  template <int K, bool RIDE> BN_HD void col(DotAcc&) const {}
+#if BN_TRACKING
+  double cap() const { return 0.0; }
+  double val() const { return 0.0; }
+#endif
 };
 BN_HD DotTerm<1> dplus(const Fp& a, const Fp& b) { return DotTerm<1>{a, b}; }
 BN_HD DotTerm<-1> dminus(const Fp& a, const Fp& b) { return DotTerm<-1>{a, b}; }
 template <int S> BN_HD DotTerm<S> dterm(const Fp& a, const Fp& b) { return DotTerm<S>{a, b}; }
-
-struct DotAcc { int64_t p1, m1, p2, m2; };
-template <int SIGN, int K>
-BN_HD void dot_col(DotAcc& c, const DotTerm<SIGN>& t) {
-  constexpr int LO = K < BN_NL ? 0 : K - (BN_NL - 1);
-  constexpr int HI = K < BN_NL ? K : BN_NL - 1;
-#pragma unroll
-  for (int i = LO; i <= HI; i++) {
-    int64_t pr = (int64_t)t.a.v[i] * (int64_t)t.b.v[K - i];
-    if (SIGN == 1) c.p1 += pr; else if (SIGN == -1) c.m1 += pr; else if (SIGN == 2) c.p2 += pr; else c.m2 += pr;
-  }
-}
-constexpr int bn_iabs(int x) { return x < 0 ? -x : x; }
-template <int K, int... SIGNS>
-BN_HD void dot_step(int64_t& acc, int32_t (&m)[BN_NL], Fp& r, const DotTerm<SIGNS>&... terms) {
-  constexpr bool has_m1 = ((SIGNS == -1) || ...), has_p2 = ((SIGNS == 2) || ...), has_m2 = ((SIGNS == -2) || ...);
+template <int S> BN_HD DotSq<S> dsq(const Fp& a) { return DotSq<S>{a}; }
+
+template <int K, bool RIDE, class... T>
+BN_HD void dot_step(int64_t& acc, int32_t (&m)[BN_NL], Fp& r, const T&... terms) {
+  constexpr bool has_m1 = ((T::cls == -1) || ...), has_p2 = ((T::cls == 2 || (RIDE && T::cls_cross == 2)) || ...), has_m2 = ((T::cls == -2 || (RIDE && T::cls_cross == -2)) || ...);
   DotAcc c; c.p1 = acc; c.m1 = 0; c.p2 = 0; c.m2 = 0;
-  (dot_col<SIGNS, K>(c, terms), ...);
+  (terms.template col<K, RIDE>(c), ...);
   acc = c.p1;
+  if constexpr (K < BN_NL) {
+#pragma unroll
+    for (int i = 0; i < K; i++) bn_ride<RIDE>(acc, m[i], bn_p_limb(K - i));
+  } else {
+#pragma unroll
+    for (int i = K - (BN_NL - 1); i < BN_NL; i++) bn_ride<RIDE>(acc, m[i], bn_p_limb(K - i));
+  }
   if (has_m1) acc -= c.m1;
   if (has_p2 && has_m2) acc += 2 * (c.p2 - c.m2);
   else if (has_p2) acc += 2 * c.p2;
   else if (has_m2) acc -= 2 * c.m2;
   if constexpr (K < BN_NL) {
-#pragma unroll
-    for (int i = 0; i < K; i++) acc += (int64_t)m[i] * (int64_t)bn_p_limb(K - i);
     m[K] = bn_sext29((uint32_t)acc * BN_PINV);
-    acc += (int64_t)m[K] * (int64_t)bn_p_limb(0);
+    bn_ride<RIDE>(acc, m[K], bn_p_limb(0));
     acc >>= BN_LB;
   } else {
-#pragma unroll
-    for (int i = K - (BN_NL - 1); i < BN_NL; i++) acc += (int64_t)m[i] * (int64_t)bn_p_limb(K - i);
     acc += BN_HALF;
     r.v[K - BN_NL] = (int32_t)((uint32_t)acc & BN_MASK) - BN_HALF;
     acc >>= BN_LB;
   }
 }
-template <int... KS, int... SIGNS>
-BN_HD void dot_all(std::integer_sequence<int, KS...>, int64_t& acc, int32_t (&m)[BN_NL], Fp& r, const DotTerm<SIGNS>&... terms) {
-  (dot_step<KS, SIGNS...>(acc, m, r, terms...), ...);
-}
-template <int... SIGNS>
-BN_HD Fp fp_dot(const DotTerm<SIGNS>&... terms) {
+template <bool RIDE, int... KS, class... T>
+BN_HD void dot_all(std::integer_sequence<int, KS...>, int64_t& acc, int32_t (&m)[BN_NL], Fp& r, const T&... terms) {
+  (dot_step<KS, RIDE, T...>(acc, m, r, terms...), ...);
+}
+template <bool RIDE, class... T>
+BN_HD Fp fp_dot_r(const T&... terms) {
   BN_SCHED_FENCE();
   int64_t acc = 0;
   int32_t m[BN_NL];
   Fp r;
-  dot_all(std::make_integer_sequence<int, 2 * BN_NL - 1>{}, acc, m, r, terms...);
+  dot_all<RIDE>(std::make_integer_sequence<int, 2 * BN_NL - 1>{}, acc, m, r, terms...);
   r.v[BN_NL - 1] = (int32_t)acc;
   BN_SCHED_FENCE();
 #if BN_TRACKING
-  double cap = ((9.0 * bn_iabs(SIGNS) * terms.a.lb * terms.b.lb) + ...);
+  double cap = (terms.cap() + ...);
   if (cap + 9.0 * 0.25 + 0.01 > 32.0) fp_dbg_fail("fp_dot: accumulator may overflow", cap);
-  double s = ((bn_iabs(SIGNS) * terms.a.vb * terms.b.vb) + ...);
+  double s = (terms.val() + ...);
   BN_SETB(r, 1.0 + s / 169.0 + 1e-6, 0.5);
 #endif
   return r;
 }
+template <class... T> BN_HD Fp fp_dot(const T&... terms) { return fp_dot_r<BN_RIDE_DEFAULT>(terms...); }
 BN_HD Fp fp_mul(const Fp& a, const Fp& b) { return fp_dot(dplus(a, b)); }
 BN_HD Fp fp_sqr(const Fp& a) {
   BN_SCHED_FENCE();
@@ -272,18 +341,19 @@
 #pragma unroll
     for (int i = 0; i < BN_NL; i++) {
       int j = k - i;
-      if (j >= 0 && j < BN_NL && i < j) acc += (int64_t)a2[i] * (int64_t)a.v[j];
-    }
-    if ((k & 1) == 0) acc += (int64_t)a.v[k / 2] * (int64_t)a.v[k / 2];
+      if (j >= 0 && j < BN_NL && i < j) bn_ride(acc, a2[i], a.v[j]);
+    }
+    if (k == 0) acc = (int64_t)a.v[0] * (int64_t)a.v[0];
+    else if ((k & 1) == 0) bn_ride(acc, a.v[k / 2], a.v[k / 2]);
     if (k < BN_NL) {
 #pragma unroll
-      for (int i = 0; i < k; i++) acc += (int64_t)m[i] * (int64_t)bn_p_limb(k - i);
+      for (int i = 0; i < k; i++) bn_ride(acc, m[i], bn_p_limb(k - i));
       m[k] = bn_sext29((uint32_t)acc * BN_PINV);
-      acc += (int64_t)m[k] * (int64_t)bn_p_limb(0);
+      bn_ride(acc, m[k], bn_p_limb(0));
       acc >>= BN_LB;
     } else {
 #pragma unroll
-      for (int i = k - (BN_NL - 1); i < BN_NL; i++) acc += (int64_t)m[i] * (int64_t)bn_p_limb(k - i);
+      for (int i = k - (BN_NL - 1); i < BN_NL; i++) bn_ride(acc, m[i], bn_p_limb(k - i));
       acc += BN_HALF;
       r.v[k - BN_NL] = (int32_t)((uint32_t)acc & BN_MASK) - BN_HALF;
       acc >>= BN_LB;
diff --git a/snark-bn254-verifier_amd/csrc/bn254_k_g16_load.hip b/snark-bn254-verifier_amd/csrc/bn254_k_g16_load.hip
--- a/snark-bn254-verifier_amd/csrc/bn254_k_g16_load.hip
+++ b/snark-bn254-verifier_amd/csrc/bn254_k_g16_load.hip
@@ -6,6 +6,7 @@
 #include "bn254_sha256.h"
 
 namespace bn254 {
+#ifndef BN_PLAIN_HALF
 
 __global__ void __launch_bounds__(256, 2)
 k_g16_classify(const uint8_t* __restrict__ proofs, size_t stride, uint32_t n, uint8_t* __restrict__ status, uint32_t* __restrict__ block_count) {
@@ -306,7 +307,10 @@
   const uint32_t k = blockIdx.x * 256u + threadIdx.x;
   if (k < m) status[idx[k]] = fb_status[k];
 }
-__global__ void __launch_bounds__(256, 2) k_g16_decompress(const uint8_t* __restrict__ src, size_t stride, uint32_t n, uint8_t* __restrict__ raw, uint8_t* __restrict__ pre) {
+#endif
+__global__ void __launch_bounds__(256, 2) k_g16_decompress(const uint8_t* __restrict__ src, size_t stride, uint32_t n, uint8_t* __restrict__ raw, uint8_t* __restrict__ pre)
+#ifdef BN_PLAIN_HALF
+{
   const uint32_t i = blockIdx.x * 256u + threadIdx.x;
   if (i >= n) return;
   const uint8_t* p = src + (size_t)i * stride;
@@ -324,6 +328,10 @@
   for (int k = 0; k < 16; k++) q[k] = make_uint4(out[4 * k], out[4 * k + 1], out[4 * k + 2], out[4 * k + 3]);
   pre[i] = ok ? 0 : 1;
 }
+#else
+;
+#endif
+#ifndef BN_PLAIN_HALF
 __global__ void __launch_bounds__(256) k_g16_status_merge(uint8_t* __restrict__ status, const uint8_t* __restrict__ pre, uint32_t n) {
   const uint32_t i = blockIdx.x * 256u + threadIdx.x;
   if (i < n && pre[i]) status[i] = BN254_ST_MALFORMED;
@@ -350,7 +358,9 @@
   pre[i] = ok ? 0 : 1;
 }
 
-}
+#endif
+}
+#ifndef BN_PLAIN_HALF
 
 using namespace bn254;
 hipError_t bn254_launch_gather_rows(uint8_t* dst, const uint8_t* src, size_t src_stride, uint32_t row_bytes, const uint32_t* idx, uint32_t m, hipStream_t s) {
@@ -375,3 +385,4 @@
   if (n) hipLaunchKernelGGL(k_sp1_public_inputs, dim3(grid_for(n)), dim3(256), 0, s, vkh, vkh_stride, pv, pv_bytes, pv_base, off, n, rows, pre);
   return hipGetLastError();
 }
+#endif
diff --git a/snark-bn254-verifier_amd/csrc/bn254_k_probe.hip b/snark-bn254-verifier_amd/csrc/bn254_k_probe.hip
--- a/snark-bn254-verifier_amd/csrc/bn254_k_probe.hip
+++ b/snark-bn254-verifier_amd/csrc/bn254_k_probe.hip
@@ -2,6 +2,7 @@
 #include "bn254_launch_ops.h"
 
 namespace bn254 {
+#ifndef BN_PLAIN_HALF
 
 #define VALU_PEAK_ITERS 16384
 __global__ void __launch_bounds__(256) k_valu_peak(uint32_t* out, uint32_t seed, int iters) {
@@ -20,6 +21,7 @@
   out[tid] = x;
 }
 
+#endif
 __device__ __forceinline__ Fp probe_ld_fp(const uint8_t* p) {
   uint32_t w[8];
   words_from_be(w, p);
@@ -30,6 +32,7 @@
   fp_to_words(w, a);
   words_to_be(p, w);
 }
+#ifndef BN_PLAIN_HALF
 __global__ void __launch_bounds__(256, 2) k_dbg_fp_mul(const uint8_t* a, const uint8_t* b, uint8_t* o, size_t n) {
   size_t i = (size_t)blockIdx.x * 256 + threadIdx.x;
   if (i >= n) return;
@@ -73,20 +76,29 @@
   int32_t* p = dst + 12 * BN_NL * (size_t)i;
   for (int t = 0; t < 12; t++) { const Fp a = w.ld(e + 2 * korder[t >> 1] + (t & 1)); for (int l = 0; l < BN_NL; l++) p[t * BN_NL + l] = a.v[l]; }
 }
-__global__ void __launch_bounds__(256, 2) k_dbg_g2_subgroup(const uint8_t* g2, uint8_t* o, size_t n) {
+#endif
+__global__ void __launch_bounds__(256, 2) k_dbg_g2_subgroup(const uint8_t* g2, uint8_t* o, size_t n)
+#ifdef BN_PLAIN_HALF
+{
   size_t i = (size_t)blockIdx.x * 256 + threadIdx.x;
   if (i >= n) return;
   G2Aff q; q.x.c1 = probe_ld_fp(g2 + 128 * i); q.x.c0 = probe_ld_fp(g2 + 128 * i + 32);
   q.y.c1 = probe_ld_fp(g2 + 128 * i + 64); q.y.c0 = probe_ld_fp(g2 + 128 * i + 96);
   o[i] = (g2_on_curve(q) && g2_in_subgroup(q)) ? 1 : 0;
 }
+#else
+;
+#endif
+#ifndef BN_PLAIN_HALF
 __global__ void __launch_bounds__(256, 2) k_dbg_g2_ate(int32_t* ws, uint32_t n, const uint8_t* __restrict__ status, uint8_t* o) {
   VM_KERNEL_PROLOGUE();
   bool ok = vm_g2_ate_check(w, VE_T, VE_B);
   if (i < n) o[i] = ok ? 1 : 0;
 }
 
-}
+#endif
+}
+#ifndef BN_PLAIN_HALF
 
 using namespace bn254;
 double bn254_measure_valu_peak(int reps) {
@@ -207,3 +219,4 @@
   hipLaunchKernelGGL(k_dbg_g2_subgroup, dim3(grid_for(n)), dim3(256), 0, s, g2, o, n);
   return hipGetLastError();
 }
+#endif
diff --git a/snark-bn254-verifier_amd/csrc/bn254_kernels.hip b/snark-bn254-verifier_amd/csrc/bn254_kernels.hip
--- a/snark-bn254-verifier_amd/csrc/bn254_kernels.hip
+++ b/snark-bn254-verifier_amd/csrc/bn254_kernels.hip
@@ -5,6 +5,7 @@
 static_assert(G16_MILLER_STEPS == BN_ATE_STEPS, "bn254_g16_plan.h counts the Miller steps of bn254_constants.h");
 
 namespace bn254 {
+#ifndef BN_PLAIN_HALF
 
 __global__ void __launch_bounds__(256, 2) k_vm_init(int32_t* ws, uint32_t n, const uint8_t* __restrict__ status) {
   VM_KERNEL_PROLOGUE();
@@ -47,8 +48,11 @@
   w.lds = park_lds;
   vm_f12_mul(w, d, a, b, conj_b != 0);
 }
+#endif
 __global__ void __launch_bounds__(256, 2) k_f12_mul_verdict(int32_t* ws, uint32_t n, uint8_t* status, int d, int a, int b, const int32_t* __restrict__ target, int reject_code,
-                                                            const uint32_t* __restrict__ slot_proof, uint8_t* __restrict__ out_status) {
+                                                            const uint32_t* __restrict__ slot_proof, uint8_t* __restrict__ out_status)
+#ifdef BN_PLAIN_HALF
+{
   __shared__ int32_t park_lds[72 * 256];
   const uint32_t i = blockIdx.x * 256u + threadIdx.x;
   const uint8_t st = status[i < n ? i : n - 1];
@@ -62,6 +66,10 @@
   }
   if (slot_proof && i < n && st != 0) out_status[slot_proof[i]] = out;
 }
+#else
+;
+#endif
+#ifndef BN_PLAIN_HALF
 __global__ void __launch_bounds__(256, 2) k_f12_copy(int32_t* ws, uint32_t n, const uint8_t* __restrict__ status, int d, int a) { VM_KERNEL_PROLOGUE(); vm_f12_copy(w, d, a); }
 __global__ void __launch_bounds__(256, 2) k_f12_cyclo_sqr(int32_t* ws, uint32_t n, const uint8_t* __restrict__ status, int d, int a) { VM_KERNEL_PROLOGUE(); vm_f12_cyclo_sqr(w, d, a); }
 __global__ void __launch_bounds__(256, 2) k_f12_cyclo_sqr_n(int32_t* ws, uint32_t n, const uint8_t* __restrict__ status, int d, int a, int count) {
@@ -83,7 +91,9 @@
   if (i < n && (st & BN254_ST_PENDING)) status[i] = g16_subgroup_status(st, ok, inputs_match_key);
 }
 
-}
+#endif
+}
+#ifndef BN_PLAIN_HALF
 
 using namespace bn254;
 const char* const bn254_kernel_kind_names[KID_COUNT] = {
@@ -265,3 +275,4 @@
   if (groups > bn254_coop_max_proofs_fixed()) return hipErrorInvalidValue;
   return bn254_coop12_miller_fixed_keys(grp_ws, grp_status, groups, granule_key, 0, desc, n_keys, target_one, reject_code, s);
 }
+#endif
diff --git a/snark-bn254-verifier_amd/csrc/bn254_rlc.h b/snark-bn254-verifier_amd/csrc/bn254_rlc.h
--- a/snark-bn254-verifier_amd/csrc/bn254_rlc.h
+++ b/snark-bn254-verifier_amd/csrc/bn254_rlc.h
@@ -170,11 +170,11 @@
     k3.c0 = w.ld0(VE_F + 6); k3.c1 = w.ld0(VE_F + 7); k4.c0 = w.ld0(VE_F + 8); k4.c1 = w.ld0(VE_F + 9); k5.c0 = w.ld0(VE_F + 10); k5.c1 = w.ld0(VE_F + 11);
     if constexpr (DO_SQR) {
       Fp2 x3 = fp2_mul_xi(k3), x4 = fp2_mul_xi(k4), x5 = fp2_mul_xi(k5);
-      w.park(0, fp2_dotp(pp(k0, k0), pp2(k1, x5), pp2(k2, x4), pp(k3, x3)));
+      w.park(0, fp2_dotp(psq(k0), pp2(k1, x5), pp2(k2, x4), pp(k3, x3)));
       w.park(1, fp2_dotp(pp2(k0, k1), pp2(k2, x5), pp2(k3, x4)));
-      w.park(2, fp2_dotp(pp2(k0, k2), pp(k1, k1), pp2(k3, x5), pp(k4, x4)));
+      w.park(2, fp2_dotp(pp2(k0, k2), psq(k1), pp2(k3, x5), pp(k4, x4)));
       w.park(3, fp2_dotp(pp2(k0, k3), pp2(k1, k2), pp2(k4, x5)));
-      f4 = fp2_dotp(pp2(k0, k4), pp2(k1, k3), pp(k2, k2), pp(k5, x5));
+      f4 = fp2_dotp(pp2(k0, k4), pp2(k1, k3), psq(k2), pp(k5, x5));
       f5 = fp2_dotp(pp2(k0, k5), pp2(k1, k4), pp2(k2, k3));
     } else {
       w.park(0, k0); w.park(1, k1); w.park(2, k2); w.park(3, k3); f4 = k4; f5 = k5;
@@ -226,11 +226,11 @@
     Fp2 k0 = vld2(w, e), k1 = vld2(w, e + 2), k2 = vld2(w, e + 4), k3 = vld2(w, e + 6), k4 = vld2(w, e + 8), k5 = vld2(w, e + 10);
     if constexpr (DO_SQR) {
       Fp2 x3 = fp2_mul_xi(k3), x4 = fp2_mul_xi(k4), x5 = fp2_mul_xi(k5);
-      w.park(0, fp2_dotp(pp(k0, k0), pp2(k1, x5), pp2(k2, x4), pp(k3, x3)));
+      w.park(0, fp2_dotp(psq(k0), pp2(k1, x5), pp2(k2, x4), pp(k3, x3)));
       w.park(1, fp2_dotp(pp2(k0, k1), pp2(k2, x5), pp2(k3, x4)));
-      w.park(2, fp2_dotp(pp2(k0, k2), pp(k1, k1), pp2(k3, x5), pp(k4, x4)));
+      w.park(2, fp2_dotp(pp2(k0, k2), psq(k1), pp2(k3, x5), pp(k4, x4)));
       w.park(3, fp2_dotp(pp2(k0, k3), pp2(k1, k2), pp2(k4, x5)));
-      f4 = fp2_dotp(pp2(k0, k4), pp2(k1, k3), pp(k2, k2), pp(k5, x5));
+      f4 = fp2_dotp(pp2(k0, k4), pp2(k1, k3), psq(k2), pp(k5, x5));
       f5 = fp2_dotp(pp2(k0, k5), pp2(k1, k4), pp2(k2, k3));
     } else {
       w.park(0, k0); w.park(1, k1); w.park(2, k2); w.park(3, k3); f4 = k4; f5 = k5;
diff --git a/snark-bn254-verifier_amd/csrc/bn254_tower.h b/snark-bn254-verifier_amd/csrc/bn254_tower.h
--- a/snark-bn254-verifier_amd/csrc/bn254_tower.h
+++ b/snark-bn254-verifier_amd/csrc/bn254_tower.h
@@ -32,13 +32,26 @@
 BN_HD P2<-1> pm(const Fp2& x, const Fp2& y) { return P2<-1>{x, y}; }
 BN_HD P2<2> pp2(const Fp2& x, const Fp2& y) { return P2<2>{x, y}; }
 BN_HD P2<-2> pm2(const Fp2& x, const Fp2& y) { return P2<-2>{x, y}; }
-template <int... W>
-BN_HD Fp2 fp2_dotp(const P2<W>&... t) {
-  Fp2 r;
-  r.c0 = fp_dot(dterm<W>(t.x.c0, t.y.c0)..., dterm<-W>(t.x.c1, t.y.c1)...);
-  r.c1 = fp_dot(dterm<W>(t.x.c0, t.y.c1)..., dterm<W>(t.x.c1, t.y.c0)...);
-  return r;
-}
+struct P2Sq {
+  const Fp2& x;
+};
+BN_HD P2Sq psq(const Fp2& x) { return P2Sq{x}; }
+template <int W> BN_HD DotTerm<W> p2_re0(const P2<W>& t) { return dterm<W>(t.x.c0, t.y.c0); }
+template <int W> BN_HD DotTerm<-W> p2_re1(const P2<W>& t) { return dterm<-W>(t.x.c1, t.y.c1); }
+template <bool RIDE, int W> BN_HD DotTerm<W> p2_im0(const P2<W>& t) { return dterm<W>(t.x.c0, t.y.c1); }
+template <bool RIDE, int W> BN_HD DotTerm<W> p2_im1(const P2<W>& t) { return dterm<W>(t.x.c1, t.y.c0); }
+BN_HD DotSq<1> p2_re0(const P2Sq& t) { return dsq<1>(t.x.c0); }
+BN_HD DotSq<-1> p2_re1(const P2Sq& t) { return dsq<-1>(t.x.c1); }
+template <bool RIDE> BN_HD auto p2_im0(const P2Sq& t) { if constexpr (RIDE) return dterm<2>(t.x.c0, t.x.c1); else return dterm<1>(t.x.c0, t.x.c1); }
+template <bool RIDE> BN_HD auto p2_im1(const P2Sq& t) { if constexpr (RIDE) return DotNone{}; else return dterm<1>(t.x.c1, t.x.c0); }
+template <bool RIDE, class... T>
+BN_HD Fp2 fp2_dotp_r(const T&... t) {
+  Fp2 r;
+  r.c0 = fp_dot_r<RIDE>(p2_re0(t)..., p2_re1(t)...);
+  r.c1 = fp_dot_r<RIDE>(p2_im0<RIDE>(t)..., p2_im1<RIDE>(t)...);
+  return r;
+}
+template <class... T> BN_HD Fp2 fp2_dotp(const T&... t) { return fp2_dotp_r<BN_RIDE_DEFAULT>(t...); }
 
 struct KAcc { uint64_t re, im, a[2][2]; };
 #define BN_KCOL_RANGE constexpr int LO = K < BN_NL ? 0 : K - (BN_NL - 1); constexpr int HI = K < BN_NL ? K : BN_NL - 1
@@ -53,7 +66,7 @@
     for (int i = LO; i <= HI; i++) {
       c.a[AW - 1][0] += bn_dmul(x0.v[i], y0.v[K - i]);
       c.a[AW - 1][1] += bn_dmul(nx1.v[i], y1.v[K - i]);
-      c.im += bn_dmul(sxw.v[i], sy.v[K - i]);
+      if (K > 0) bn_ride(c.im, sxw.v[i], sy.v[K - i]); else c.im += bn_dmul(sxw.v[i], sy.v[K - i]);
     }
   }
 #if BN_TRACKING
@@ -71,8 +84,8 @@
     BN_KCOL_RANGE;
 #pragma unroll
     for (int i = LO; i <= HI; i++) {
-      c.re += bn_dmul(ure.v[i], vre.v[K - i]);
-      c.im += bn_dmul(uim.v[i], vim.v[K - i]);
+      if (K > 0) { bn_ride(c.re, ure.v[i], vre.v[K - i]); bn_ride(c.im, uim.v[i], vim.v[K - i]); }
+      else { c.re += bn_dmul(ure.v[i], vre.v[K - i]); c.im += bn_dmul(uim.v[i], vim.v[K - i]); }
     }
   }
 #if BN_TRACKING
@@ -109,18 +122,18 @@
   (t.template col<K>(c), ...);
   if constexpr (K < BN_NL) {
 #pragma unroll
-    for (int i = 0; i < K; i++) { c.re += bn_dmul(mre[i], bn_p_limb(K - i)); c.im += bn_dmul(mim[i], bn_p_limb(K - i)); }
+    for (int i = 0; i < K; i++) { bn_ride(c.re, mre[i], bn_p_limb(K - i)); bn_ride(c.im, mim[i], bn_p_limb(K - i)); }
   } else {
 #pragma unroll
-    for (int i = K - (BN_NL - 1); i < BN_NL; i++) { c.re += bn_dmul(mre[i], bn_p_limb(K - i)); c.im += bn_dmul(mim[i], bn_p_limb(K - i)); }
+    for (int i = K - (BN_NL - 1); i < BN_NL; i++) { bn_ride(c.re, mre[i], bn_p_limb(K - i)); bn_ride(c.im, mim[i], bn_p_limb(K - i)); }
   }
   if (has1) { c.re += c.a[0][0] + c.a[0][1]; c.im += c.a[0][1] - c.a[0][0]; }
   if (has2) { c.re += (c.a[1][0] + c.a[1][1]) << 1; c.im += (c.a[1][1] - c.a[1][0]) << 1; }
   if constexpr (K < BN_NL) {
     mre[K] = bn_sext29((uint32_t)c.re * BN_PINV);
     mim[K] = bn_sext29((uint32_t)c.im * BN_PINV);
-    c.re += bn_dmul(mre[K], bn_p_limb(0));
-    c.im += bn_dmul(mim[K], bn_p_limb(0));
+    bn_ride(c.re, mre[K], bn_p_limb(0));
+    bn_ride(c.im, mim[K], bn_p_limb(0));
     cre = (int64_t)c.re >> BN_LB;
     cim = (int64_t)c.im >> BN_LB;
   } else {
@@ -162,10 +175,11 @@
   return r;
 }
 BN_HD Fp2 fp2_mul_fp(const Fp2& a, const Fp& f) { Fp2 r; r.c0 = fp_mul(a.c0, f); r.c1 = fp_mul(a.c1, f); return r; }
+template <bool RIDE = BN_RIDE_DEFAULT>
 BN_HD Fp2 fp2_mul_xi(const Fp2& a) {
   Fp2 r;
-  r.c0 = fp_lincomb_reduce(9, a.c0, -1, a.c1);
-  r.c1 = fp_lincomb_reduce(1, a.c0, 9, a.c1);
+  r.c0 = fp_lincomb_reduce<RIDE>(9, a.c0, -1, a.c1);
+  r.c1 = fp_lincomb_reduce<RIDE>(1, a.c0, 9, a.c1);
   return r;
 }
 BN_HD Fp2 fp2_mul_small(const Fp2& a, int32_t k) {
@@ -174,14 +188,15 @@
   r.c1 = fp_lincomb_reduce(k, a.c1, 0, a.c1);
   return r;
 }
+template <bool RIDE = BN_RIDE_DEFAULT>
 BN_HD Fp2 fp2_lincomb_reduce(int32_t k1, const Fp2& a, int32_t k2, const Fp2& b) {
   Fp2 r;
-  r.c0 = fp_lincomb_reduce(k1, a.c0, k2, b.c0);
-  r.c1 = fp_lincomb_reduce(k1, a.c1, k2, b.c1);
+  r.c0 = fp_lincomb_reduce<RIDE>(k1, a.c0, k2, b.c0);
+  r.c1 = fp_lincomb_reduce<RIDE>(k1, a.c1, k2, b.c1);
   return r;
 }
 BN_HD Fp2 fp2_inv(const Fp2& a) {
-  Fp n = fp_dot(dplus(a.c0, a.c0), dplus(a.c1, a.c1));
+  Fp n = fp_dot(dsq<1>(a.c0), dsq<1>(a.c1));
   Fp ni = fp_inv(n);
   Fp2 r;
   r.c0 = fp_mul(a.c0, ni);
@@ -222,18 +237,18 @@
 BN_HD Fp6 fp6_sqr(const Fp6& x) {
   Fp2 X2 = fp2_mul_xi(x.c2);
   Fp6 r;
-  r.c0 = fp2_dotp(pp(x.c0, x.c0), pp2(x.c1, X2));
+  r.c0 = fp2_dotp(psq(x.c0), pp2(x.c1, X2));
   r.c1 = fp2_dotp(pp2(x.c0, x.c1), pp(x.c2, X2));
-  r.c2 = fp2_dotp(pp2(x.c0, x.c2), pp(x.c1, x.c1));
+  r.c2 = fp2_dotp(pp2(x.c0, x.c2), psq(x.c1));
   return r;
 }
 BN_HD Fp6 fp6_mul_fp2(const Fp6& a, const Fp2& b) { Fp6 r; r.c0 = fp2_mul(a.c0, b); r.c1 = fp2_mul(a.c1, b); r.c2 = fp2_mul(a.c2, b); return r; }
 BN_HD_NOINLINE Fp6 fp6_mul_nl(const Fp6& a, const Fp6& b) { return fp6_mul(a, b); }
 BN_HD Fp6 fp6_inv(const Fp6& a) {
   Fp2 X1 = fp2_mul_xi(a.c1), X2 = fp2_mul_xi(a.c2);
-  Fp2 A = fp2_dotp(pp(a.c0, a.c0), pm(X1, a.c2));
+  Fp2 A = fp2_dotp(psq(a.c0), pm(X1, a.c2));
   Fp2 B = fp2_dotp(pp(X2, a.c2), pm(a.c0, a.c1));
-  Fp2 C = fp2_dotp(pp(a.c1, a.c1), pm(a.c0, a.c2));
+  Fp2 C = fp2_dotp(psq(a.c1), pm(a.c0, a.c2));
   Fp2 F = fp2_dotp(pp(a.c0, A), pp(X2, B), pp(X1, C));
   Fp2 Fi = fp2_inv(F);
   Fp6 r;
@@ -265,11 +280,11 @@
 BN_HD Fp12 fp12_sqr(const Fp12& f) {
   Fp2 x3 = fp2_mul_xi(K3(f)), x4 = fp2_mul_xi(K4(f)), x5 = fp2_mul_xi(K5(f));
   Fp12 r;
-  K0(r) = fp2_dotp(pp(K0(f), K0(f)), pp2(K1(f), x5), pp2(K2(f), x4), pp(K3(f), x3));
+  K0(r) = fp2_dotp(psq(K0(f)), pp2(K1(f), x5), pp2(K2(f), x4), pp(K3(f), x3));
   K1(r) = fp2_dotp(pp2(K0(f), K1(f)), pp2(K2(f), x5), pp2(K3(f), x4));
-  K2(r) = fp2_dotp(pp2(K0(f), K2(f)), pp(K1(f), K1(f)), pp2(K3(f), x5), pp(K4(f), x4));
+  K2(r) = fp2_dotp(pp2(K0(f), K2(f)), psq(K1(f)), pp2(K3(f), x5), pp(K4(f), x4));
   K3(r) = fp2_dotp(pp2(K0(f), K3(f)), pp2(K1(f), K2(f)), pp2(K4(f), x5));
-  K4(r) = fp2_dotp(pp2(K0(f), K4(f)), pp2(K1(f), K3(f)), pp(K2(f), K2(f)), pp(K5(f), x5));
+  K4(r) = fp2_dotp(pp2(K0(f), K4(f)), pp2(K1(f), K3(f)), psq(K2(f)), pp(K5(f), x5));
   K5(r) = fp2_dotp(pp2(K0(f), K5(f)), pp2(K1(f), K4(f)), pp2(K2(f), K3(f)));
   return r;
 }
@@ -331,11 +346,11 @@
   return r;
 }
 BN_HD void gs_pair(Fp2& za, Fp2& zb, const Fp2& a, const Fp2& b, const Fp2& sub, const Fp2& add, bool xi_on_cross) {
-  Fp2 xb = fp2_mul_xi(b);
-  Fp2 S = fp2_dotp(pp(xb, b), pp(a, a));
-  Fp2 T = xi_on_cross ? fp2_dotp(pp2(a, xb)) : fp2_dotp(pp2(a, b));
-  za = fp2_lincomb_reduce(3, S, -2, sub);
-  zb = fp2_lincomb_reduce(3, T, 2, add);
+  Fp2 xb = fp2_mul_xi<false>(b);
+  Fp2 S = fp2_dotp_r<false>(pp(xb, b), pp(a, a));
+  Fp2 T = xi_on_cross ? fp2_dotp_r<false>(pp2(a, xb)) : fp2_dotp_r<false>(pp2(a, b));
+  za = fp2_lincomb_reduce<false>(3, S, -2, sub);
+  zb = fp2_lincomb_reduce<false>(3, T, 2, add);
 }
 BN_HD Fp12 fp12_cyclo_sqr(const Fp12& x) {
   Fp12 z;
diff --git a/snark-bn254-verifier_amd/csrc/bn254_vm.h b/snark-bn254-verifier_amd/csrc/bn254_vm.h
--- a/snark-bn254-verifier_amd/csrc/bn254_vm.h
+++ b/snark-bn254-verifier_amd/csrc/bn254_vm.h
@@ -31,11 +31,11 @@
 BN_HD void vm_f12_sqr(W& w, int e) {
   Fp2 k0 = vld2(w, e), k1 = vld2(w, e + 2), k2 = vld2(w, e + 4), k3 = vld2(w, e + 6), k4 = vld2(w, e + 8), k5 = vld2(w, e + 10);
   Fp2 x3 = fp2_mul_xi(k3), x4 = fp2_mul_xi(k4), x5 = fp2_mul_xi(k5);
-  vst2(w, e, fp2_dotp(pp(k0, k0), pp2(k1, x5), pp2(k2, x4), pp(k3, x3)));
+  vst2(w, e, fp2_dotp(psq(k0), pp2(k1, x5), pp2(k2, x4), pp(k3, x3)));
   vst2(w, e + 2, fp2_dotp(pp2(k0, k1), pp2(k2, x5), pp2(k3, x4)));
-  vst2(w, e + 4, fp2_dotp(pp2(k0, k2), pp(k1, k1), pp2(k3, x5), pp(k4, x4)));
+  vst2(w, e + 4, fp2_dotp(pp2(k0, k2), psq(k1), pp2(k3, x5), pp(k4, x4)));
   vst2(w, e + 6, fp2_dotp(pp2(k0, k3), pp2(k1, k2), pp2(k4, x5)));
-  vst2(w, e + 8, fp2_dotp(pp2(k0, k4), pp2(k1, k3), pp(k2, k2), pp(k5, x5)));
+  vst2(w, e + 8, fp2_dotp(pp2(k0, k4), pp2(k1, k3), psq(k2), pp(k5, x5)));
   vst2(w, e + 10, fp2_dotp(pp2(k0, k5), pp2(k1, k4), pp2(k2, k3)));
 }
 template <class W>
@@ -121,11 +121,11 @@
   {
     Fp2 k0 = vld2(w, e), k1 = vld2(w, e + 2), k2 = vld2(w, e + 4), k3 = vld2(w, e + 6), k4 = vld2(w, e + 8), k5 = vld2(w, e + 10);
     Fp2 x3 = fp2_mul_xi(k3), x4 = fp2_mul_xi(k4), x5 = fp2_mul_xi(k5);
-    w.park(0, fp2_dotp(pp(k0, k0), pp2(k1, x5), pp2(k2, x4), pp(k3, x3)));
+    w.park(0, fp2_dotp(psq(k0), pp2(k1, x5), pp2(k2, x4), pp(k3, x3)));
     w.park(1, fp2_dotp(pp2(k0, k1), pp2(k2, x5), pp2(k3, x4)));
-    w.park(2, fp2_dotp(pp2(k0, k2), pp(k1, k1), pp2(k3, x5), pp(k4, x4)));
+    w.park(2, fp2_dotp(pp2(k0, k2), psq(k1), pp2(k3, x5), pp(k4, x4)));
     w.park(3, fp2_dotp(pp2(k0, k3), pp2(k1, k2), pp2(k4, x5)));
-    r4 = fp2_dotp(pp2(k0, k4), pp2(k1, k3), pp(k2, k2), pp(k5, x5));
+    r4 = fp2_dotp(pp2(k0, k4), pp2(k1, k3), psq(k2), pp(k5, x5));
     r5 = fp2_dotp(pp2(k0, k5), pp2(k1, k4), pp2(k2, k3));
   }
   G2Line l;
@@ -156,11 +156,11 @@
   if constexpr (DO_SQR) {
     Fp2 k0 = vld2(w, e), k1 = vld2(w, e + 2), k2 = vld2(w, e + 4), k3 = vld2(w, e + 6), k4 = vld2(w, e + 8), k5 = vld2(w, e + 10);
     Fp2 x3 = fp2_mul_xi(k3), x4 = fp2_mul_xi(k4), x5 = fp2_mul_xi(k5);
-    w.park(0, fp2_dotp(pp(k0, k0), pp2(k1, x5), pp2(k2, x4), pp(k3, x3)));
+    w.park(0, fp2_dotp(psq(k0), pp2(k1, x5), pp2(k2, x4), pp(k3, x3)));
     w.park(1, fp2_dotp(pp2(k0, k1), pp2(k2, x5), pp2(k3, x4)));
-    w.park(2, fp2_dotp(pp2(k0, k2), pp(k1, k1), pp2(k3, x5), pp(k4, x4)));
+    w.park(2, fp2_dotp(pp2(k0, k2), psq(k1), pp2(k3, x5), pp(k4, x4)));
     w.park(3, fp2_dotp(pp2(k0, k3), pp2(k1, k2), pp2(k4, x5)));
-    f4 = fp2_dotp(pp2(k0, k4), pp2(k1, k3), pp(k2, k2), pp(k5, x5));
+    f4 = fp2_dotp(pp2(k0, k4), pp2(k1, k3), psq(k2), pp(k5, x5));
     f5 = fp2_dotp(pp2(k0, k5), pp2(k1, k4), pp2(k2, k3));
   }
   G2Line l;
@@ -232,11 +232,11 @@
 template <class W> BN_HD void mf_sqr(W& w, Fp2& f4, Fp2& f5) {
   Fp2 k0 = w.unpark(0), k1 = w.unpark(1), k2 = w.unpark(2), k3 = w.unpark(3), k4 = f4, k5 = f5;
   Fp2 x3 = fp2_mul_xi(k3), x4 = fp2_mul_xi(k4), x5 = fp2_mul_xi(k5);
-  w.park(0, fp2_dotp(pp(k0, k0), pp2(k1, x5), pp2(k2, x4), pp(k3, x3)));
+  w.park(0, fp2_dotp(psq(k0), pp2(k1, x5), pp2(k2, x4), pp(k3, x3)));
   w.park(1, fp2_dotp(pp2(k0, k1), pp2(k2, x5), pp2(k3, x4)));
-  w.park(2, fp2_dotp(pp2(k0, k2), pp(k1, k1), pp2(k3, x5), pp(k4, x4)));
+  w.park(2, fp2_dotp(pp2(k0, k2), psq(k1), pp2(k3, x5), pp(k4, x4)));
   w.park(3, fp2_dotp(pp2(k0, k3), pp2(k1, k2), pp2(k4, x5)));
-  Fp2 n4 = fp2_dotp(pp2(k0, k4), pp2(k1, k3), pp(k2, k2), pp(k5, x5));
+  Fp2 n4 = fp2_dotp(pp2(k0, k4), pp2(k1, k3), psq(k2), pp(k5, x5));
   f5 = fp2_dotp(pp2(k0, k5), pp2(k1, k4), pp2(k2, k3));
   f4 = n4;
 }
```
